# afb2001/path_planner

Measured on AMD Instinct MI355X. Metric: Dubins edges costed/sec on 2048x2048 grid, higher is better.
Workload: dtype f64; 1 GPU; cfg3_2048_10pct_65536_obst16; grid=2048x2048 @0.1m, 10% blocked, samples_per_iter_per_gpu=65536, samples_per_iter_total=65536, dynamic_obstacles=16, obstacle_placement=uniform in the map (SURVEY 8d), seed 3, ribbons=5, heuristic=TspPointRobotNoSplitKRibbons K=2, edges_per_iter_per_gpu=236140

## Files before the change

include/ppgpu.h:

```cpp
#ifndef PATH_PLANNER_AMD_PPGPU_H
#define PATH_PLANNER_AMD_PPGPU_H

#include <stdint.h>

#ifdef __cplusplus
extern "C" {
#endif

#define PPGPU_OK          0
#define PPGPU_EINVAL     (-1)
#define PPGPU_EHIP       (-2)
#define PPGPU_ENODEV     (-3)
#define PPGPU_ESTATE     (-4)
#define PPGPU_ECAPACITY  (-5)
#define PPGPU_ERCCL      (-6)

typedef struct ppgpu_ctx ppgpu_ctx;

enum {
    PPGPU_H_MAX_DISTANCE = 0,
    PPGPU_H_TSP_POINT_ALL = 1,
    PPGPU_H_TSP_POINT_K = 2,
    PPGPU_H_TSP_DUBINS_ALL = 3,
    PPGPU_H_TSP_DUBINS_K = 4
};

enum {
    PPGPU_OBST_NONE = 0,
    PPGPU_OBST_BINARY = 1,
    PPGPU_OBST_GAUSSIAN = 2
};

typedef struct ppgpu_config {
    double max_speed;
    double slow_speed;
    double turning_radius;
    double coverage_turning_radius;
    double time_horizon;
    double time_minimum;
    double collision_checking_increment;
    double start_state_time;
    double ribbon_width;
    double collision_penalty_factor;
    double time_penalty_factor;
    double heuristic_turning_radius;
    int32_t heuristic;
    int32_t tsp_k;
    int32_t branching_factor;
    int32_t reserved;
} ppgpu_config;

typedef struct ppgpu_vertex {
    double x, y, heading, speed, time;
    double g;
    double coverage_completed_time;
    int32_t ribbon_offset;
    int32_t ribbon_count;
} ppgpu_vertex;

#define PPGPU_F_INFEASIBLE   0x01u
#define PPGPU_F_THROWS       0x02u
#define PPGPU_F_RIBBON_OVF   0x04u
#define PPGPU_F_RIBBON_LOST  0x40u
#define PPGPU_F_DUBINS_ERR   0x08u
#define PPGPU_F_GOAL         0x10u
#define PPGPU_F_DONE         0x20u

typedef struct ppgpu_edge_result {
    uint32_t flags;
    uint32_t info;
    double true_cost;
    double collision_penalty;
    double approx_cost;
    double end_x, end_y, end_heading, end_speed, end_time;
    double g, h, f;
    double coverage_completed_time;
    double param[3];
} ppgpu_edge_result;

#define PPGPU_EDGE_COVERAGE 0x1u
#define PPGPU_EDGE_SLOW     0x2u
static inline uint64_t ppgpu_edge_pack(uint32_t vertex, uint32_t target, uint32_t cfg) {
    return ((uint64_t)(cfg & 0xffu) << 56) | ((uint64_t)(vertex & 0xffffffu) << 32) | (uint64_t)target;
}

typedef struct ppgpu_wrapper_edge {
    int32_t vertex;
    int32_t coverage_allowed;
    double qi[3];
    double param[3];
    double rho;
    int32_t type;
    int32_t reserved;
    double speed;
    double start_time;
    double end_time;
} ppgpu_wrapper_edge;


int ppgpu_create(int device, ppgpu_ctx** out);
int ppgpu_destroy(ppgpu_ctx* ctx);
const char* ppgpu_last_error(void);
int ppgpu_set_stream(ppgpu_ctx* ctx, void* hip_stream);
int ppgpu_synchronize(ppgpu_ctx* ctx);
int ppgpu_reserve_samples(ppgpu_ctx* ctx, int64_t max_samples, int32_t max_vertices);
int ppgpu_growth_stats(ppgpu_ctx* ctx, uint64_t* count, double* seconds);
int ppgpu_enable_timing(ppgpu_ctx* ctx, int32_t on);
int ppgpu_last_timing(ppgpu_ctx* ctx, double* ms_solve, double* ms_pose, double* ms_cover, double* ms_heuristic);
int ppgpu_past_timing(ppgpu_ctx* ctx, int32_t back, double* ms_solve, double* ms_pose, double* ms_cover, double* ms_heuristic);
int ppgpu_last_cover_edges(ppgpu_ctx* ctx, int64_t* n_edges);
int ppgpu_last_shared_edges(ppgpu_ctx* ctx, int64_t* n_edges);

int ppgpu_device_alloc(ppgpu_ctx* ctx, uint64_t bytes, void** d_out);
int ppgpu_device_free(ppgpu_ctx* ctx, void* d_ptr);
int ppgpu_device_read(ppgpu_ctx* ctx, void* h_dst, const void* d_src, uint64_t bytes);
int ppgpu_copy_engine_read(ppgpu_ctx* ctx, void* h_pinned_dst, const void* d_src, uint64_t bytes);
int ppgpu_copy_engine_wait(ppgpu_ctx* ctx);


int ppgpu_set_config(ppgpu_ctx* ctx, const ppgpu_config* cfg);

int ppgpu_set_grid(ppgpu_ctx* ctx, const uint8_t* h_cells, int32_t rows, int32_t cols, double resolution);
int ppgpu_get_grid_clearance(ppgpu_ctx* ctx, uint8_t* h_out, int64_t capacity);

int ppgpu_set_obstacles(ppgpu_ctx* ctx, int32_t model, int32_t n, const double* h_obstacles7);

int ppgpu_set_gaussian_obstacles(ppgpu_ctx* ctx, int32_t n, const double* h_obstacles, int32_t covariance_given);

int ppgpu_set_vertices(ppgpu_ctx* ctx, int32_t n, const ppgpu_vertex* h_vertices,
                       int32_t n_ribbons, const double* h_ribbons4);


int ppgpu_sampler_init(ppgpu_ctx* ctx, const double* bounds6, uint64_t seed,
                       int32_t n_ribbons, const double* h_ribbons4);

int ppgpu_sampler_add(ppgpu_ctx* ctx, int64_t n_attempts, int64_t* n_total_out);

int ppgpu_sampler_skip(ppgpu_ctx* ctx, int64_t n_attempts);

int ppgpu_set_samples(ppgpu_ctx* ctx, int64_t n, const double* h_x, const double* h_y, const double* h_heading);
int ppgpu_set_extra_targets(ppgpu_ctx* ctx, int32_t n, const double* h_x, const double* h_y, const double* h_heading,
                            int64_t* first_index);

int ppgpu_get_samples(ppgpu_ctx* ctx, int64_t first, int64_t n, double* h_states5);
int64_t ppgpu_num_samples(ppgpu_ctx* ctx);


int ppgpu_dubins_lengths(ppgpu_ctx* ctx, int32_t v0, int32_t nv, double* d_lengths);

int ppgpu_select_nearest(ppgpu_ctx* ctx, int32_t v0, int32_t nv, int32_t k,
                         int32_t* h_sample_index, double* h_length);

int ppgpu_expand_order(ppgpu_ctx* ctx, int32_t v0, int32_t nv, int32_t k, int32_t* h_sample_index, uint32_t* h_fallbacks);
uint64_t ppgpu_order_fallbacks(ppgpu_ctx* ctx);


int ppgpu_cost_edges_dense(ppgpu_ctx* ctx, int32_t v0, int32_t nv, int64_t s0, int64_t ns,
                           uint32_t cfg_mask, ppgpu_edge_result* d_results,
                           double* d_child_ribbons, int32_t ribbon_stride);

int ppgpu_cost_edges_list(ppgpu_ctx* ctx, int64_t n, const uint64_t* d_edges,
                          ppgpu_edge_result* d_results,
                          double* d_child_ribbons, int32_t ribbon_stride);

int64_t ppgpu_expand_capacity(int32_t nv, int32_t k);
int ppgpu_expand_host(ppgpu_ctx* ctx, int32_t nv, const ppgpu_vertex* h_vertices, int32_t n_ribbons, const double* h_ribbons,
                      const double* h_nearest, int32_t k, int64_t* n_edges, uint64_t* h_edges, ppgpu_edge_result* h_results,
                      double* h_child_ribbons, int32_t ribbon_stride);

int ppgpu_heuristic_host(ppgpu_ctx* ctx, int32_t n, const double* h_poses3, const int32_t* h_ribbon_counts, const double* h_ribbons,
                         double* h_out, uint32_t* h_flags);

#define PPGPU_TSP_TABLE_MAX 16
int ppgpu_set_tsp_table(ppgpu_ctx* ctx, int32_t min_ribbons, int32_t max_ribbons);
int ppgpu_set_dubins_tsp_table(ppgpu_ctx* ctx, int32_t min_ribbons, int32_t max_ribbons);
int ppgpu_tsp_table_stats(ppgpu_ctx* ctx, uint64_t* lists, uint64_t* refused);
int ppgpu_last_tsp_table_timing(ppgpu_ctx* ctx, double* ms);

int ppgpu_cost_edges_host(ppgpu_ctx* ctx, int64_t n, const uint64_t* h_edges,
                          ppgpu_edge_result* h_results,
                          double* h_child_ribbons, int32_t ribbon_stride);

int ppgpu_cost_wrapper_edges_host(ppgpu_ctx* ctx, int64_t n, const ppgpu_wrapper_edge* h_edges,
                                  ppgpu_edge_result* h_results,
                                  double* h_child_ribbons, int32_t ribbon_stride);


#define PPGPU_CHAIN_LEGS        1u
#define PPGPU_CHAIN_INFEASIBLE  2u
#define PPGPU_CHAIN_GOAL        3u
#define PPGPU_CHAIN_THROWS      4u
#define PPGPU_CHAIN_CAPACITY    5u

int ppgpu_cost_plans_host(ppgpu_ctx* ctx, int32_t n_plans, const int32_t* h_leg_offsets, const ppgpu_wrapper_edge* h_legs,
                          ppgpu_edge_result* h_results, double* h_child_ribbons, int32_t ribbon_stride,
                          int32_t* h_legs_costed, uint32_t* h_stop);


#define PPGPU_S_BLOCKED  0x1u
#define PPGPU_S_STRAIGHT 0x2u
typedef struct ppgpu_step_record {
    double x, y, heading, time;
    double collision;
    double penalty_before;
    uint32_t flags, step;
    double reserved;
} ppgpu_step_record;

int ppgpu_trace_edges_list(ppgpu_ctx* ctx, int64_t n, const uint64_t* d_edges, ppgpu_edge_result* d_results,
                           int32_t step_stride, int32_t* d_counts, ppgpu_step_record* d_steps);
int ppgpu_trace_edges_host(ppgpu_ctx* ctx, int64_t n, const uint64_t* h_edges, ppgpu_edge_result* h_results,
                           int32_t step_stride, int32_t* h_counts, ppgpu_step_record* h_steps);
int ppgpu_trace_wrapper_edges_host(ppgpu_ctx* ctx, int64_t n, const ppgpu_wrapper_edge* h_wedges, ppgpu_edge_result* h_results,
                                   int32_t step_stride, int32_t* h_counts, ppgpu_step_record* h_steps);
int ppgpu_last_trace_timing(ppgpu_ctx* ctx, double* ms_trace);


#define PPGPU_C_EVENT   0x1u
#define PPGPU_C_COVER   0x2u
#define PPGPU_C_CHANGED 0x4u
#define PPGPU_C_DONE    0x8u
typedef struct ppgpu_cover_record {
    double to_cover;
    double remaining;
    uint32_t flags, step;
    uint32_t ribbons;
    uint32_t reserved;
} ppgpu_cover_record;

#define PPGPU_CS_LAST_COVER   0x01u
#define PPGPU_CS_LAST_CHANGED 0x02u
#define PPGPU_CS_DONE         0x04u
#define PPGPU_CS_REFUSED      0x08u
#define PPGPU_CS_THROWS       0x10u
typedef struct ppgpu_cover_summary {
    int32_t events, changes;
    int32_t ribbons_final;
    uint32_t flags;
    double coverage_completed_time;
    double remaining_final;
} ppgpu_cover_summary;

int ppgpu_trace_cover_list(ppgpu_ctx* ctx, int64_t n, const uint64_t* d_edges, ppgpu_edge_result* d_results,
                           int32_t step_stride, int32_t* d_counts, ppgpu_cover_record* d_cover,
                           ppgpu_cover_summary* d_summaries, double* d_child_ribbons, int32_t ribbon_stride);
int ppgpu_trace_cover_host(ppgpu_ctx* ctx, int64_t n, const uint64_t* h_edges, ppgpu_edge_result* h_results,
                           int32_t step_stride, int32_t* h_counts, ppgpu_cover_record* h_cover,
                           ppgpu_cover_summary* h_summaries, double* h_child_ribbons, int32_t ribbon_stride);
int ppgpu_trace_cover_wrapper_edges_host(ppgpu_ctx* ctx, int64_t n, const ppgpu_wrapper_edge* h_wedges, ppgpu_edge_result* h_results,
                                         int32_t step_stride, int32_t* h_counts, ppgpu_cover_record* h_cover,
                                         ppgpu_cover_summary* h_summaries, double* h_child_ribbons, int32_t ribbon_stride);
int ppgpu_last_cover_trace_timing(ppgpu_ctx* ctx, double* ms_cover_trace);


typedef struct ppgpu_contact_record {
    double cpa_distance;
    double cpa_time;
    double first_hit_time, last_hit_time;
    double exposure;
    int32_t cpa_step, hit_steps, first_hit_step, last_hit_step;
    double peak;
} ppgpu_contact_record;

int ppgpu_obstacle_count(ppgpu_ctx* ctx, int32_t* n, int32_t* model);
// ... 98 lines not shown
```

path_planner_amd/api.py:

```python
import ctypes as C
import os

import numpy as np

from .types import PpgpuConfig, RESULT_DTYPE, VERTEX_DTYPE

_HERE = os.path.dirname(os.path.abspath(__file__))
LIB_PATH = os.environ.get("PPGPU_LIB_OVERRIDE") or os.path.join(_HERE, "csrc", "libppgpu.so")


class PpgpuError(RuntimeError):
    pass


def _load():
    try:
        import torch
    except Exception:
        pass
    if not os.path.exists(LIB_PATH):
        raise ImportError(
            f"{LIB_PATH} is missing: build it with `python -c 'import __graft_entry__ as g; g.build()'` "
            "(hipcc --offload-arch=gfx950). path_planner_amd has no CPU fallback.")
    lib = C.CDLL(LIB_PATH)
    vp, i32, i64, u32, u64, dbl = C.c_void_p, C.c_int32, C.c_int64, C.c_uint32, C.c_uint64, C.c_double
    sig = {
        "ppgpu_create": (C.c_int, [C.c_int, C.POINTER(vp)]),
        "ppgpu_destroy": (C.c_int, [vp]),
        "ppgpu_last_error": (C.c_char_p, []),
        "ppgpu_set_stream": (C.c_int, [vp, vp]),
        "ppgpu_synchronize": (C.c_int, [vp]),
        "ppgpu_reserve_samples": (C.c_int, [vp, i64, i32]),
        "ppgpu_growth_stats": (C.c_int, [vp, C.POINTER(u64), C.POINTER(dbl)]),
        "ppgpu_device_alloc": (C.c_int, [vp, u64, C.POINTER(vp)]),
        "ppgpu_device_free": (C.c_int, [vp, vp]),
        "ppgpu_device_read": (C.c_int, [vp, vp, vp, u64]),
        "ppgpu_copy_engine_read": (C.c_int, [vp, vp, vp, u64]),
        "ppgpu_copy_engine_wait": (C.c_int, [vp]),
        "ppgpu_heuristic_host": (C.c_int, [vp, i32, vp, vp, vp, vp, vp]),
        "ppgpu_set_tsp_table": (C.c_int, [vp, i32, i32]),
        "ppgpu_set_dubins_tsp_table": (C.c_int, [vp, i32, i32]),
        "ppgpu_tsp_table_stats": (C.c_int, [vp, C.POINTER(u64), C.POINTER(u64)]),
        "ppgpu_last_tsp_table_timing": (C.c_int, [vp, C.POINTER(dbl)]),
        "ppgpu_expand_capacity": (C.c_int64, [i32, i32]),
        "ppgpu_expand_host": (C.c_int, [vp, i32, vp, i32, vp, vp, i32, C.POINTER(C.c_int64), vp, vp, vp, i32]),
        "ppgpu_enable_timing": (C.c_int, [vp, i32]),
        "ppgpu_last_timing": (C.c_int, [vp, C.POINTER(dbl), C.POINTER(dbl), C.POINTER(dbl), C.POINTER(dbl)]),
        "ppgpu_past_timing": (C.c_int, [vp, i32, C.POINTER(dbl), C.POINTER(dbl), C.POINTER(dbl), C.POINTER(dbl)]),
        "ppgpu_last_cover_edges": (C.c_int, [vp, C.POINTER(i64)]),
        "ppgpu_last_shared_edges": (C.c_int, [vp, C.POINTER(i64)]),
        "ppgpu_set_config": (C.c_int, [vp, C.POINTER(PpgpuConfig)]),
        "ppgpu_set_grid": (C.c_int, [vp, vp, i32, i32, dbl]),
        "ppgpu_get_grid_clearance": (C.c_int, [vp, vp, i64]),
        "ppgpu_set_obstacles": (C.c_int, [vp, i32, i32, vp]),
        "ppgpu_set_gaussian_obstacles": (C.c_int, [vp, i32, vp, i32]),
        "ppgpu_set_vertices": (C.c_int, [vp, i32, vp, i32, vp]),
        "ppgpu_sampler_init": (C.c_int, [vp, vp, u64, i32, vp]),
        "ppgpu_sampler_add": (C.c_int, [vp, i64, C.POINTER(i64)]),
        "ppgpu_sampler_skip": (C.c_int, [vp, i64]),
        "ppgpu_set_samples": (C.c_int, [vp, i64, vp, vp, vp]),
        "ppgpu_set_extra_targets": (C.c_int, [vp, i32, vp, vp, vp, C.POINTER(i64)]),
        "ppgpu_get_samples": (C.c_int, [vp, i64, i64, vp]),
        "ppgpu_num_samples": (i64, [vp]),
        "ppgpu_dubins_lengths": (C.c_int, [vp, i32, i32, vp]),
        "ppgpu_select_nearest": (C.c_int, [vp, i32, i32, i32, vp, vp]),
        "ppgpu_expand_order": (C.c_int, [vp, i32, i32, i32, vp, C.POINTER(u32)]),
        "ppgpu_order_fallbacks": (u64, [vp]),
        "ppgpu_cost_edges_dense": (C.c_int, [vp, i32, i32, i64, i64, u32, vp, vp, i32]),
        "ppgpu_cost_edges_list": (C.c_int, [vp, i64, vp, vp, vp, i32]),
        "ppgpu_cost_edges_host": (C.c_int, [vp, i64, vp, vp, vp, i32]),
        "ppgpu_cost_wrapper_edges_host": (C.c_int, [vp, i64, vp, vp, vp, i32]),
        "ppgpu_cost_plans_host": (C.c_int, [vp, i32, vp, vp, vp, vp, i32, vp, vp]),
        "ppgpu_trace_edges_list": (C.c_int, [vp, i64, vp, vp, i32, vp, vp]),
        "ppgpu_trace_edges_host": (C.c_int, [vp, i64, vp, vp, i32, vp, vp]),
        "ppgpu_trace_wrapper_edges_host": (C.c_int, [vp, i64, vp, vp, i32, vp, vp]),
        "ppgpu_last_trace_timing": (C.c_int, [vp, C.POINTER(dbl)]),
        "ppgpu_trace_cover_list": (C.c_int, [vp, i64, vp, vp, i32, vp, vp, vp, vp, i32]),
        "ppgpu_trace_cover_host": (C.c_int, [vp, i64, vp, vp, i32, vp, vp, vp, vp, i32]),
        "ppgpu_trace_cover_wrapper_edges_host": (C.c_int, [vp, i64, vp, vp, i32, vp, vp, vp, vp, i32]),
        "ppgpu_last_cover_trace_timing": (C.c_int, [vp, C.POINTER(dbl)]),
        "ppgpu_obstacle_count": (C.c_int, [vp, C.POINTER(i32), C.POINTER(i32)]),
        "ppgpu_trace_contacts_list": (C.c_int, [vp, i64, vp, vp, vp, vp]),
        "ppgpu_trace_contacts_host": (C.c_int, [vp, i64, vp, vp, vp, vp]),
        "ppgpu_trace_contacts_wrapper_edges_host": (C.c_int, [vp, i64, vp, vp, vp, vp]),
        "ppgpu_last_contact_trace_timing": (C.c_int, [vp, C.POINTER(dbl)]),
        "ppgpu_get_grid_distance": (C.c_int, [vp, vp, i64]),
        "ppgpu_grid_clearance_at": (C.c_int, [vp, i64, vp, vp, vp]),
        "ppgpu_last_grid_distance_timing": (C.c_int, [vp, C.POINTER(dbl)]),
        "ppgpu_trace_clearance_list": (C.c_int, [vp, i64, vp, vp, vp, vp, dbl]),
        "ppgpu_trace_clearance_host": (C.c_int, [vp, i64, vp, vp, vp, vp, dbl]),
        "ppgpu_trace_clearance_wrapper_edges_host": (C.c_int, [vp, i64, vp, vp, vp, vp, dbl]),
        "ppgpu_last_clearance_trace_timing": (C.c_int, [vp, C.POINTER(dbl)]),
        "ppgpu_keepout_limit2": (C.c_int, [dbl, dbl, C.POINTER(u32)]),
        "ppgpu_set_keepout_limit2": (C.c_int, [vp, u32]),
        "ppgpu_get_keepout_limit2": (C.c_int, [vp, C.POINTER(u32)]),
        "ppgpu_get_grid_blocked": (C.c_int, [vp, vp, i64]),
        "ppgpu_last_keepout_timing": (C.c_int, [vp, C.POINTER(dbl)]),
        "ppgpu_get_grid_labels": (C.c_int, [vp, vp, i64]),
        "ppgpu_set_reach_seed": (C.c_int, [vp, dbl, dbl, vp]),
        "ppgpu_get_grid_reach_gap": (C.c_int, [vp, vp, i64]),
        "ppgpu_ribbon_reach_host": (C.c_int, [vp, i32, vp, dbl, vp]),
        "ppgpu_last_reach_timing": (C.c_int, [vp, C.POINTER(dbl), C.POINTER(dbl), C.POINTER(dbl)]),
        "ppgpu_dense_edge_count": (i64, [i32, i64, u32]),
        "ppgpu_best_edge": (C.c_int, [vp, i64, vp, i32, u64, vp]),
        "ppgpu_key_min": (C.c_int, [vp, i32, vp, vp]),
        "ppgpu_allreduce_best": (C.c_int, [vp, vp, vp]),
        "ppgpu_comm_unique_id": (C.c_int, [vp]),
        "ppgpu_comm_init_rank": (C.c_int, [vp, i32, i32, vp]),
        "ppgpu_comm_init_all": (C.c_int, [C.POINTER(vp), i32]),
        "ppgpu_comm_info": (C.c_int, [vp, C.POINTER(i32), C.POINTER(i32)]),
        "ppgpu_comm_destroy": (C.c_int, [vp]),
        "ppgpu_comm_abort": (C.c_int, [vp]),
    }
    for name, (res, args) in sig.items():
        fn = getattr(lib, name)
        fn.restype = res
        fn.argtypes = args
    return lib, list(sig)


LIB, EXPORTS = _load()


def keepout_limit2(res, margin):
    k = C.c_uint32()
    rc = LIB.ppgpu_keepout_limit2(float(res), float(margin), C.byref(k))
    if rc != 0:
        raise PpgpuError(f"ppgpu_keepout_limit2 failed ({rc}): {LIB.ppgpu_last_error().decode()}")
    return k.value


def _ptr(a):
    if a is None:
        return None
    if isinstance(a, np.ndarray):
        assert a.flags["C_CONTIGUOUS"]
        return a.ctypes.data
    return int(a)


class Context:

    def __init__(self, device=0):
        h = C.c_void_p()
        rc = LIB.ppgpu_create(device, C.byref(h))
        if rc != 0:
            raise PpgpuError(f"ppgpu_create: {LIB.ppgpu_last_error().decode()}")
        self._h = h

    def _ck(self, rc, what):
        if rc != 0:
            raise PpgpuError(f"{what} failed ({rc}): {LIB.ppgpu_last_error().decode()}")

    def close(self):
        if self._h:
            LIB.ppgpu_destroy(self._h)
            self._h = None

    def __del__(self):
        try:
            self.close()
        except Exception:
            pass

    def set_stream(self, stream_ptr):
        self._ck(LIB.ppgpu_set_stream(self._h, stream_ptr), "ppgpu_set_stream")

    def enable_timing(self, on=True):
        self._ck(LIB.ppgpu_enable_timing(self._h, 1 if on else 0), "ppgpu_enable_timing")

    def last_timing(self):
        t = [C.c_double() for _ in range(4)]
        self._ck(LIB.ppgpu_last_timing(self._h, *[C.byref(x) for x in t]), "ppgpu_last_timing")
        return tuple(x.value for x in t)

    def past_timing(self, back):
        t = [C.c_double() for _ in range(4)]
        self._ck(LIB.ppgpu_past_timing(self._h, back, *[C.byref(x) for x in t]), "ppgpu_past_timing")
        return tuple(x.value for x in t)

    def last_cover_edges(self):
        n = C.c_int64()
        self._ck(LIB.ppgpu_last_cover_edges(self._h, C.byref(n)), "ppgpu_last_cover_edges")
        return n.value

    def last_shared_edges(self):
        n = C.c_int64()
        self._ck(LIB.ppgpu_last_shared_edges(self._h, C.byref(n)), "ppgpu_last_shared_edges")
        return n.value

    def reserve_samples(self, max_samples, max_vertices=16):
        self._ck(LIB.ppgpu_reserve_samples(self._h, max_samples, max_vertices), "ppgpu_reserve_samples")

    def synchronize(self):
        self._ck(LIB.ppgpu_synchronize(self._h), "ppgpu_synchronize")

    def set_config(self, cfg):
        self.cfg = cfg
        self._ck(LIB.ppgpu_set_config(self._h, C.byref(cfg)), "ppgpu_set_config")

    def set_grid(self, cells, resolution):
        if cells is None:
            self._ck(LIB.ppgpu_set_grid(self._h, None, 0, 0, 0.0), "ppgpu_set_grid")
            return
        cells = np.ascontiguousarray(cells, dtype=np.uint8)
        self._ck(LIB.ppgpu_set_grid(self._h, _ptr(cells), cells.shape[0], cells.shape[1], float(resolution)), "ppgpu_set_grid")

    def get_grid_clearance(self, rows, cols):
        out = np.zeros((rows, cols), dtype=np.uint8)
        self._ck(LIB.ppgpu_get_grid_clearance(self._h, _ptr(out), out.size), "ppgpu_get_grid_clearance")
        return out

    def set_obstacles(self, obst7, model=1):
        if obst7 is None or len(obst7) == 0:
            self._ck(LIB.ppgpu_set_obstacles(self._h, 0, 0, None), "ppgpu_set_obstacles")
            return
        o = np.ascontiguousarray(obst7, dtype=np.float64).reshape(-1, 7)
        self._ck(LIB.ppgpu_set_obstacles(self._h, model, o.shape[0], _ptr(o)), "ppgpu_set_obstacles")

    def set_gaussian_obstacles(self, rows):
        o = np.ascontiguousarray(rows, dtype=np.float64)
        if o.size == 0:
            self._ck(LIB.ppgpu_set_gaussian_obstacles(self._h, 0, None, 0), "ppgpu_set_gaussian_obstacles")
            return
        assert o.ndim == 2 and o.shape[1] in (5, 9)
        self._ck(LIB.ppgpu_set_gaussian_obstacles(self._h, o.shape[0], _ptr(o), 1 if o.shape[1] == 9 else 0), "ppgpu_set_gaussian_obstacles")

    def set_vertices(self, vertices, ribbons4):
        v = np.ascontiguousarray(vertices, dtype=VERTEX_DTYPE)
        r = np.ascontiguousarray(ribbons4, dtype=np.float64).reshape(-1, 4)
        self._ck(LIB.ppgpu_set_vertices(self._h, v.shape[0], _ptr(v), r.shape[0], _ptr(r) if r.shape[0] else None),
                 "ppgpu_set_vertices")

    def sampler_init(self, bounds6, seed, ribbons4=None):
        b = np.ascontiguousarray(bounds6, dtype=np.float64)
        if ribbons4 is None:
            self._ck(LIB.ppgpu_sampler_init(self._h, _ptr(b), int(seed), -1, None), "ppgpu_sampler_init")
        else:
            r = np.ascontiguousarray(ribbons4, dtype=np.float64).reshape(-1, 4)
            self._ck(LIB.ppgpu_sampler_init(self._h, _ptr(b), int(seed), r.shape[0], _ptr(r) if r.shape[0] else None),
                     "ppgpu_sampler_init")

    def sampler_add(self, n_attempts):
        tot = C.c_int64()
        self._ck(LIB.ppgpu_sampler_add(self._h, int(n_attempts), C.byref(tot)), "ppgpu_sampler_add")
        return tot.value

    def copy_engine_read(self, h_pinned_ptr, d_ptr, nbytes):
        self._ck(LIB.ppgpu_copy_engine_read(self._h, int(h_pinned_ptr), int(d_ptr), int(nbytes)), "ppgpu_copy_engine_read")

    def copy_engine_wait(self):
        self._ck(LIB.ppgpu_copy_engine_wait(self._h), "ppgpu_copy_engine_wait")

    def growth_stats(self):
        n, sec = C.c_uint64(), C.c_double()
        self._ck(LIB.ppgpu_growth_stats(self._h, C.byref(n), C.byref(sec)), "ppgpu_growth_stats")
        return int(n.value), float(sec.value)

    def sampler_skip(self, n_attempts):
        self._ck(LIB.ppgpu_sampler_skip(self._h, int(n_attempts)), "ppgpu_sampler_skip")

    def set_samples(self, x, y, heading):
        x = np.ascontiguousarray(x, dtype=np.float64)
        y = np.ascontiguousarray(y, dtype=np.float64)
        h = np.ascontiguousarray(heading, dtype=np.float64)
        self._ck(LIB.ppgpu_set_samples(self._h, x.shape[0], _ptr(x), _ptr(y), _ptr(h)), "ppgpu_set_samples")

    def num_samples(self):
        return LIB.ppgpu_num_samples(self._h)

    def get_samples(self, first=0, n=None):
        if n is None:
            n = self.num_samples() - first
        out = np.zeros((n, 5), dtype=np.float64)
        self._ck(LIB.ppgpu_get_samples(self._h, first, n, _ptr(out)), "ppgpu_get_samples")
        return out

    def dubins_lengths(self, v0, nv, d_lengths):
        self._ck(LIB.ppgpu_dubins_lengths(self._h, v0, nv, _ptr(d_lengths)), "ppgpu_dubins_lengths")

    def set_extra_targets(self, x, y, heading):
        x, y, heading = [np.ascontiguousarray(a, dtype=np.float64) for a in (x, y, heading)]
        first = C.c_int64(0)
        self._ck(LIB.ppgpu_set_extra_targets(self._h, x.shape[0], _ptr(x) if x.shape[0] else None, _ptr(y) if x.shape[0] else None,
                                             _ptr(heading) if x.shape[0] else None, C.byref(first)), "ppgpu_set_extra_targets")
        return int(first.value)

    def select_nearest(self, v0, nv, k):
        idx = np.zeros((nv, 2, k), dtype=np.int32)
        ln = np.zeros((nv, 2, k), dtype=np.float64)
        self._ck(LIB.ppgpu_select_nearest(self._h, v0, nv, k, _ptr(idx), _ptr(ln)), "ppgpu_select_nearest")
        return idx, ln

    def expand_order(self, nv, k):
        idx = np.zeros((nv, 2, k), dtype=np.int32)
        fb = C.c_uint32(0)
        self._ck(LIB.ppgpu_expand_order(self._h, 0, nv, k, _ptr(idx), C.byref(fb)), "ppgpu_expand_order")
        return idx, int(fb.value)

    def order_fallbacks(self):
        return int(LIB.ppgpu_order_fallbacks(self._h))

    def cost_edges_dense(self, v0, nv, s0, ns, cfg_mask, d_results, d_child=None, stride=0):
        self._ck(LIB.ppgpu_cost_edges_dense(self._h, v0, nv, s0, ns, cfg_mask, _ptr(d_results), _ptr(d_child), stride),
                 "ppgpu_cost_edges_dense")

    def cost_edges_list(self, n, d_edges, d_results, d_child=None, stride=0):
        self._ck(LIB.ppgpu_cost_edges_list(self._h, n, _ptr(d_edges), _ptr(d_results), _ptr(d_child), stride),
                 "ppgpu_cost_edges_list")

    def heuristic_host(self, poses3, ribbon_lists):
        ps = np.ascontiguousarray(poses3, dtype=np.float64).reshape(-1, 3)
        counts = np.array([len(r) for r in ribbon_lists], dtype=np.int32)
        flat = np.ascontiguousarray(np.concatenate([np.asarray(r, dtype=np.float64).reshape(-1, 4) for r in ribbon_lists]) if counts.sum() else np.zeros((0, 4)))
        out = np.zeros(len(ps), dtype=np.float64)
        fl = np.zeros(len(ps), dtype=np.uint32)
        self._ck(LIB.ppgpu_heuristic_host(self._h, len(ps), _ptr(ps), _ptr(counts), _ptr(flat) if len(flat) else None, _ptr(out), _ptr(fl)), "ppgpu_heuristic_host")
        return out, fl

    def set_tsp_table(self, min_ribbons, max_ribbons):
        self._ck(LIB.ppgpu_set_tsp_table(self._h, int(min_ribbons), int(max_ribbons)), "ppgpu_set_tsp_table")

    def set_dubins_tsp_table(self, min_ribbons, max_ribbons):
        self._ck(LIB.ppgpu_set_dubins_tsp_table(self._h, int(min_ribbons), int(max_ribbons)), "ppgpu_set_dubins_tsp_table")

    def tsp_table_stats(self):
        lists, refused = C.c_uint64(), C.c_uint64()
        self._ck(LIB.ppgpu_tsp_table_stats(self._h, C.byref(lists), C.byref(refused)), "ppgpu_tsp_table_stats")
        return int(lists.value), int(refused.value)

    def last_tsp_table_timing(self):
        ms = C.c_double()
        self._ck(LIB.ppgpu_last_tsp_table_timing(self._h, C.byref(ms)), "ppgpu_last_tsp_table_timing")
        return float(ms.value)

    def expand_host(self, vertices, ribbons4, nearest3, k, stride=0):
        v = np.ascontiguousarray(vertices, dtype=VERTEX_DTYPE)
        r = np.ascontiguousarray(ribbons4, dtype=np.float64).reshape(-1, 4)
        nz = np.ascontiguousarray(nearest3, dtype=np.float64).reshape(-1, 3)
        cap = int(LIB.ppgpu_expand_capacity(v.shape[0], k))
        e = np.zeros(cap, dtype=np.uint64)
        res = np.zeros(cap, dtype=RESULT_DTYPE)
# ... 250 lines not shown
```

path_planner_amd/csrc/pp_k_common.h:

```cpp
#pragma once
#include "../../include/ppgpu.h"
#include "pp_device.h"

struct __attribute__((aligned(128))) PPLaunchWords {
    unsigned need_big;
    unsigned live_count;
    unsigned hw_count;
    unsigned defer_count[PP_HL_MAX_N + 1];
};
static_assert(sizeof(PPLaunchWords) == 128, "the launch counters share one 128-byte line");

struct PPParams {
    double max_speed, slow_speed, rho, rho_cov, horizon, tmin, inc_d, sst, ribw, cpf, tpf;
    double inv_inc_d;
    int heuristic, tsp_k;
    int fuse_h;
    int quiet_finish;
    int lane_split;
    int defer_h;
    double h_rho;
    PPGrid grid;
    const PPObst* obst; int n_obst; int obst_model;
    const ppgpu_vertex* verts; const double* ribbons; const double* tgrid; int ng; int nverts;
    const double* sx; const double* sy; const double* sh; long long n_samples;
    const unsigned long long* edges; long long n_edges;
    long long total_edges;
    const ppgpu_wrapper_edge* wedges;
    int v0, nv; long long s0, ns; unsigned cfg_mask; int per;
    ppgpu_edge_result* out; double* child; int stride;
    long long e_base, ws_base;
    struct PPEdgeSetup* setup;
    unsigned short* track_hits;
    unsigned long long* track_eq;
    unsigned* track_chunk_hits;
    double* track_pen;
    double* track_chunk_pen;
    struct PPTrackSummary* track_summary;
    unsigned char* track_skip;
    int2* track_far;
    unsigned long long* work;
    PPLaunchWords* words;
    int reset_words;
    unsigned* live_list;
    unsigned* defer_list;
    struct PPCoverState* cover_state;
    unsigned* hw_list;
    int ngp, nch;
    unsigned* share_head;
    unsigned* share_of;
};

#define PP_SETUP_MALFORMED 1u
#define PP_SETUP_COLOCATED 2u
#define PP_SETUP_SHARED 4u
#define PP_SETUP_NO_SWEEP (PP_SETUP_MALFORMED | PP_SETUP_COLOCATED | PP_SETUP_SHARED)
#define PP_SHARE_KEYS 8
#define PP_SHARE_NONE 0xffffffffu
struct PPEdgeSetupBody {
    PPSegBase seg[3];
    double p0, p1, p2, hi1;
    double qx, qy, rho, rho_inv, length;
    double wStart, wEnd, speed;
    double approx;
    unsigned long long omask;
    int type;
    unsigned vi, cbits, sflags;
    double srcH;
};
struct __attribute__((aligned(128))) PPEdgeSetup : PPEdgeSetupBody {};
static_assert(sizeof(PPEdgeSetup) == 256 && sizeof(PPEdgeSetupBody) == 256, "PPEdgeSetup is sized for two 128-byte lines");
template <bool TAB = false>
__device__ __forceinline__ void pp_setup_seg_pose(const PPEdgeSetupBody* S, int i, double tprime, double p0, double p1, int word, double& ux, double& uy, double& uth) {
    const PPSegBase* g = &S->seg[i];
    pp_curve_seg<TAB>(pp_word_seg_type(word, i), (tprime - pp_seg_o1(i, p0)) - pp_seg_o2(i, p1), g->bx, g->by, g->bth, g->sb, g->cb, ux, uy, uth);
}
template <bool TAB = false>
__device__ __forceinline__ void pp_setup_seg_pose(const PPEdgeSetupBody* S, int i, double tprime, double& ux, double& uy, double& uth) {
    pp_setup_seg_pose<TAB>(S, i, tprime, S->p0, S->p1, S->type, ux, uy, uth);
}
#define PP_SETUP_GLOBAL_WORDS 32
#define PP_SETUP_WORDS 32
#define PP_SETUP_LDS_STRIDE 33
static_assert(sizeof(PPEdgeSetup) == 8 * PP_SETUP_GLOBAL_WORDS && sizeof(PPEdgeSetupBody) == 8 * PP_SETUP_WORDS, "the LDS staging of the skip planner copies whole records");

__global__ __launch_bounds__(256) void pp_k_grid_row_clear(const uint32_t* bits, int rows, int cols, int wpr, unsigned char* rowclear) {
    const long long i = (long long)blockIdx.x * 256 + threadIdx.x;
    if (i >= (long long)rows * cols) return;
    const int r = (int)(i / cols), c = (int)(i - (long long)r * cols);
    const uint32_t* row = bits + (size_t)r * wpr;
    int d = 0;
    for (; d < PP_CLEAR_CAP; d++) {
        const int a = c - d, b = c + d;
        if (a < 0 || b >= cols) break;
        if (((row[a >> 5] >> (a & 31)) | (row[b >> 5] >> (b & 31))) & 1u) break;
    }
    rowclear[i] = (unsigned char)d;
}
__global__ __launch_bounds__(256) void pp_k_grid_clear(const unsigned char* rowclear, int rows, int cols, unsigned char* clearance) {
    const long long i = (long long)blockIdx.x * 256 + threadIdx.x;
    if (i >= (long long)rows * cols) return;
    const int r = (int)(i / cols), c = (int)(i - (long long)r * cols);
    int best = rowclear[i];
    for (int dy = 1; dy < best; dy++) {
        const int up = r + dy, dn = r - dy;
        int m = dy;
        if (up < rows && dn >= 0) {
            const int ru = rowclear[(size_t)up * cols + c], rd = rowclear[(size_t)dn * cols + c];
            m = max(dy, min(ru, rd));
        }
        best = min(best, m);
    }
    clearance[i] = (unsigned char)best;
}

#define PP_TG_SEG 2048
__global__ __launch_bounds__(64) void pp_k_time_grid(const ppgpu_vertex* verts, int nverts, double sst, double inc_d, double max_speed,
                                                    int ng, double* tgrid) {
    __shared__ double seg[PP_TG_SEG];
    const int v = blockIdx.x;
    if (v >= nverts) return;
    const int lane = threadIdx.x;
    double timeIncrement = inc_d / max_speed;
    double t = verts[v].time;
    double timeSinceStart = t - sst;
    double timeNudge = fmod(timeSinceStart, timeIncrement);
    t += timeNudge;
    double* row = tgrid + (size_t)v * ng;
    int s = 0;
    for (int tries = 0; s < ng && tries < 8; tries++) {
        const double c = (t + timeIncrement) - t;
        int firstBad = ng;
        for (int k0 = s; k0 < ng; k0 += 64) {
            const int k = k0 + lane;
            const double val = t + (double)(k - s) * c;
            const double nxt = t + (double)(k + 1 - s) * c;
            if (k < ng) row[k] = val;
            const bool bad = (k < ng - 1) && !(val + timeIncrement == nxt);
            const unsigned long long m = __ballot(bad);
            if (m != 0ull) { firstBad = k0 + (int)__builtin_ctzll(m); break; }
        }
        if (firstBad == ng) { s = ng; break; }
        const double tf = t + (double)(firstBad - s) * c;
        t = tf + timeIncrement;
        s = firstBad + 1;
    }
    for (int k0 = s; k0 < ng; k0 += PP_TG_SEG) {
        const int m = (ng - k0) < PP_TG_SEG ? (ng - k0) : PP_TG_SEG;
        if (lane == 0) {
            for (int k = 0; k < m; k++) {
                seg[k] = t;
                t += timeIncrement;
            }
        }
        __syncthreads();
        for (int k = lane; k < m; k += 64) row[k0 + k] = seg[k];
        __syncthreads();
        t = __shfl(t, 0, 64);
    }
}

__device__ __forceinline__ long long pp_edge_position(const PPParams& p, long long w) {
    if (p.wedges || p.edges) return w;
    const long long Q = p.total_edges / p.per;
    const long long r = w / Q;
    return (w - r * Q) * p.per + (p.per - 1 - r);
}

__device__ __forceinline__ void pp_edge_decode(const PPParams& p, long long e, unsigned& vi, unsigned& target, unsigned& cbits) {
    if (p.wedges) {
        vi = (unsigned)p.wedges[e].vertex;
        target = 0;
        cbits = p.wedges[e].coverage_allowed ? PPGPU_EDGE_COVERAGE : 0u;
    } else if (p.edges) {
        unsigned long long d = p.edges[e];
        target = (unsigned)(d & 0xffffffffull);
        vi = (unsigned)((d >> 32) & 0xffffffull);
        cbits = (unsigned)(d >> 56);
    } else {
        long long q = e / p.per;
        int rank = (int)(e - q * p.per);
        long long vv = q / p.ns;
        target = (unsigned)(p.s0 + (q - vv * p.ns));
        vi = (unsigned)(p.v0 + vv);
        unsigned m = p.cfg_mask;
        for (int i = 0; i < rank; i++) m &= m - 1;
        cbits = (unsigned)(__ffs((int)m) - 1);
    }
}

template <int WPB>
__device__ __forceinline__ long long pp_wave_edge(int& wave) {
    wave = __builtin_amdgcn_readfirstlane((int)(threadIdx.x >> 6));
    return (long long)blockIdx.x * WPB + wave;
}
#define PP_NQ 32
#define PP_QSTRIDE 544
#define PP_WORK_WORDS (PP_NQ * PP_QSTRIDE)
struct PPQueue { int q, dry; };
__device__ __forceinline__ PPQueue pp_queue_init() {
    PPQueue s; s.q = (int)(blockIdx.x % PP_NQ); s.dry = 0; return s;
}
__device__ __forceinline__ long long pp_next_edge(const PPParams& p, PPQueue& s, long long n) {
    while (s.dry < PP_NQ) {
        unsigned long long* head = p.work + (size_t)s.q * PP_QSTRIDE;
        unsigned long long k = 0;
        if (pp_lane() == 0) {
            k = (s.dry > 0) ? __hip_atomic_load(head, __ATOMIC_RELAXED, __HIP_MEMORY_SCOPE_AGENT) : 0ull;
            if ((long long)(k * PP_NQ) + s.q < n) k = atomicAdd(head, 1ull);
        }
        const unsigned lo = (unsigned)__builtin_amdgcn_readfirstlane((int)(unsigned)k);
        const unsigned hi = (unsigned)__builtin_amdgcn_readfirstlane((int)(unsigned)(k >> 32));
        const int q = __builtin_amdgcn_readfirstlane(s.q);
        const unsigned long long kk = ((unsigned long long)hi << 32) | lo;
        const long long idx = (long long)(kk * PP_NQ) + q;
        if (idx < n) { s.dry = 0; return idx; }
        s.q = (s.q + 1 == PP_NQ) ? 0 : s.q + 1;
        s.dry++;
    }
    return n;
}
__device__ __forceinline__ void pp_launch_reset(const PPParams& p, long long e) {
    if (!p.reset_words) return;
    if (e < PP_NQ) p.work[(size_t)e * PP_QSTRIDE] = 0ull;
    if (e == 0) { if (p.e_base == 0) *p.words = PPLaunchWords{}; else p.words->live_count = 0u; }
}
```

path_planner_amd/csrc/pp_k_cover.h:

```cpp
#pragma once
__device__ __forceinline__ int pp_event_stride(double D, double inc_d, double inv_inc_d, int ng) {
    int m = 0;
    if (D > inc_d) {
        const double qd = D * inv_inc_d;
        if (qd > (double)(ng + 2)) {
            m = ng + 1;
        } else {
            const int m0 = (int)ceil(qd - 1.0);
            const double r = fma(-(double)m0, inc_d, D);
            const double margin = (double)m0 * D * 5e-16 + 1e-12;
            if (m0 >= 1 && r > margin && r < inc_d - margin) {
                m = m0;
            } else {
                double tc = D;
                while (tc > inc_d && m <= ng) { tc -= inc_d; m++; }
            }
        }
    }
    return m;
}

#define PP_FAR_DONE (-2)
#define PP_FAR_SHARED (-3)
#define PP_FAR_LAST_MASK 0xfffff
#define PP_FAR_SPLIT (1 << 30)
#define PP_FAR_MOVE_END (1 << 29)
#define PP_FAR_PIECE_SHIFT 21
#define PP_REC_STRIDE 17
template <class RP>
__device__ __forceinline__ bool pp_any_tiny_ribbon(RP r, int n, double thr) {
    bool tiny = false;
    for (int i = 0; i < n; i++) tiny |= pp_sq_len(r[4 * i], r[4 * i + 1], r[4 * i + 2], r[4 * i + 3]) < thr;
    return tiny;
}
struct PPBoxScan { bool inBox; int boxCount, boxIdx; double q; };
template <class RP>
__device__ __forceinline__ PPBoxScan pp_box_scan(RP r, int n, double x, double y, double grow) {
    PPBoxScan s = {false, 0, 0, PP_DBL_MAX};
    for (int i = 0; i < n; i++) {
        const double sx = r[4 * i], sy = r[4 * i + 1], ex = r[4 * i + 2], ey = r[4 * i + 3];
        const bool in = pp_in_grown_box(sx, sy, ex, ey, x, y, grow);
        s.inBox |= in; s.boxCount += in ? 1 : 0; s.boxIdx = in ? i : s.boxIdx;
        const double qS = (sx - x) * (sx - x) + (sy - y) * (sy - y);
        const double qE = (ex - x) * (ex - x) + (ey - y) * (ey - y);
        s.q = fmin(s.q, fmin(qE, qS));
    }
    return s;
}
#ifndef PP_APPROACH_MIN_WAVES
#define PP_APPROACH_MIN_WAVES 4
#endif
#ifndef PP_APPROACH_THREADS
#define PP_APPROACH_THREADS 256
#endif
#ifndef PP_LANE_NEAR_MAX
#define PP_LANE_NEAR_MAX 8
#endif
__global__ __launch_bounds__(PP_APPROACH_THREADS, PP_APPROACH_MIN_WAVES) void pp_k_approach_events(PPParams p) {
    __shared__ double s_rec[PP_APPROACH_THREADS * PP_REC_STRIDE];
    const long long e0 = (long long)blockIdx.x * PP_APPROACH_THREADS;
    const long long e = e0 + threadIdx.x;
    const bool valid = e < p.n_edges;
    const PPEdgeSetupBody* S = p.setup + p.ws_base + (valid ? e : 0);
    int2 out; out.x = 0; out.y = 0;
    int splitInfo = 0;
#ifdef PP_DBG_PHASES
    const long long apT0 = (long long)__builtin_readcyclecounter();
    long long apT1 = apT0, apT2 = apT0;
    int apEvents = 0;
#endif
    const unsigned sflags = S->sflags;
    const int dubType = S->type;
    const unsigned viMine = S->vi;
    const unsigned viFirst = (unsigned)__builtin_amdgcn_readfirstlane((int)viMine);
    const bool oneVertex = viFirst < (unsigned)p.nverts && __ballot(valid && viMine != viFirst) == 0ull;
    const double* rpU = p.ribbons + 4 * (size_t)pp_const_i32(&p.verts[oneVertex ? viFirst : 0].ribbon_offset)[0];
    const int nribU = pp_const_i32(&p.verts[oneVertex ? viFirst : 0].ribbon_count)[0];
    if (valid && !(sflags & PP_SETUP_NO_SWEEP) && dubType >= 0) {
        const ppgpu_vertex* V = p.verts + S->vi;
        const int nrib = V->ribbon_count;
        const int limit = p.track_summary[p.ws_base + e].limit;
        if (nrib > 0 && nrib <= PP_WAVE && limit > 0) {
            const double* rp = p.ribbons + 4 * (size_t)V->ribbon_offset;
            const double* tg = p.tgrid + (size_t)S->vi * p.ng;
            const PPLaneCurve cv = pp_lane_curve(S);
            const double endTime0 = fmin(p.horizon + 1e-12 + p.sst, S->wEnd);
            const double w = p.ribw, grow = w + 1e-3, minLength0 = 2 * w;
            const PPLaneRibbons ribs = {rp, nrib, rpU, nribU, oneVertex};
            const bool tiny = pp_with_ribbons(ribs, [&](auto r, int n) { return pp_any_tiny_ribbon(r, n, minLength0 * minLength0 / (2.0 * 2.0)); });
            int k = 0, lastEv = -1;
            bool handOver = tiny;
            int nearBudget = PP_LANE_NEAR_MAX;
            const bool covEdge = (S->cbits & PPGPU_EDGE_COVERAGE) != 0;
#ifdef PP_DBG_PHASES
            apT1 = (long long)__builtin_readcyclecounter();
#endif
            while (!tiny) {
                if (k >= limit) break;
                const double t = tg[k];
                if (!(t < endTime0)) break;
#ifdef PP_DBG_PHASES
                apEvents++;
#endif
                double x, y, uth;
                bool perr = false;
                pp_lane_pose(S, cv, t, x, y, uth, perr);
                if (perr) { handOver = true; break; }
                const PPBoxScan scan = pp_with_ribbons(ribs, [&](auto r, int n) { return pp_box_scan(r, n, x, y, grow); });
                const int boxIdx = scan.boxIdx;
#ifdef PP_DBG_TRACE
                if (pp_edge_position(p, p.e_base + e) == (long long)(PP_DBG_TRACE)) printf("[lane] event %d: inBox %d q %.17g x %.17g y %.17g\n", k, (int)scan.inBox, scan.q, x, y);
#endif
                double D = fmin(PP_DBL_MAX, sqrt(scan.q));
                if (scan.inBox) {
                    if (scan.boxCount == 1 && nearBudget-- > 0) {
                        bool inside, strict;
                        double px, py;
                        const double bsx = rp[4 * boxIdx], bsy = rp[4 * boxIdx + 1], bex = rp[4 * boxIdx + 2], bey = rp[4 * boxIdx + 3];
                        pp_lane_ribbon_contains(bsx, bsy, bex, bey, x, y, w, inside, strict, px, py);
                        const bool coverOn = covEdge || (((p.track_eq[(size_t)(p.ws_base + e) * p.nch + (k >> 6)] >> (k & 63)) & 1ull) != 0ull);
                        if (!(strict && coverOn)) {
                            if (inside) D = 0;
                            lastEv = k;
                            k = k + pp_event_stride(D, p.inc_d, p.inv_inc_d, p.ng) + 1;
                            continue;
                        }
                        const double thr = minLength0 * minLength0 / (2.0 * 2.0);
                        const bool keepF = !(pp_sq_len(bsx, bsy, px, py) < thr), keepR = !(pp_sq_len(px, py, bex, bey) < thr);
                        if (keepF && keepR && p.lane_split && nrib + 1 <= p.stride && nrib + 1 <= PP_WAVE) {
                            double* c = p.child + (size_t)pp_edge_position(p, p.e_base + e) * p.stride * 4;
                            for (int i = 0; i < boxIdx; i++) { c[4 * i] = rp[4 * i]; c[4 * i + 1] = rp[4 * i + 1]; c[4 * i + 2] = rp[4 * i + 2]; c[4 * i + 3] = rp[4 * i + 3]; }
                            c[4 * boxIdx] = bsx; c[4 * boxIdx + 1] = bsy; c[4 * boxIdx + 2] = px; c[4 * boxIdx + 3] = py;
                            c[4 * boxIdx + 4] = px; c[4 * boxIdx + 5] = py; c[4 * boxIdx + 6] = bex; c[4 * boxIdx + 7] = bey;
                            for (int i = boxIdx + 1; i < nrib; i++) { c[4 * i + 4] = rp[4 * i]; c[4 * i + 5] = rp[4 * i + 1]; c[4 * i + 6] = rp[4 * i + 2]; c[4 * i + 7] = rp[4 * i + 3]; }
                            double sn, cs;
                            pp_sincos_bounded(uth, &sn, &cs);
                            const bool towardsEnd = (cs * (bex - bsx) + sn * (bey - bsy)) > 0.0;
                            splitInfo = PP_FAR_SPLIT | (towardsEnd ? 0 : PP_FAR_MOVE_END) | ((towardsEnd ? boxIdx + 1 : boxIdx) << PP_FAR_PIECE_SHIFT);
                            lastEv = k;
                            k = k + 1;
                            handOver = true; break;
                        }
                    }
                    handOver = true; break;
                }
                lastEv = k;
                k = k + pp_event_stride(D, p.inc_d, p.inv_inc_d, p.ng) + 1;
            }
            out.x = k; out.y = (lastEv + 1) | splitInfo;
#ifdef PP_DBG_PHASES
            apT2 = (long long)__builtin_readcyclecounter();
#endif
            if (!handOver && k >= limit && p.quiet_finish &&
                pp_finish_quiet_edge(p, S, cv, V, p.ws_base + e, pp_edge_position(p, p.e_base + e), limit, lastEv, ribs, tg, s_rec + (size_t)threadIdx.x * PP_REC_STRIDE))
                out.x = PP_FAR_DONE;
        }
    }
    asm volatile("" ::: "memory");
    if (valid && (S->sflags & PP_SETUP_SHARED) != 0u) out.x = PP_FAR_SHARED;
    if (valid) p.track_far[p.ws_base + e] = make_int2(max(out.x, PP_FAR_DONE), out.y);
#ifdef PP_DBG_PHASES
    {
        const long long apT3 = (long long)__builtin_readcyclecounter();
        const double wPro = pp_wave_max((double)(apT1 - apT0)), wLoop = pp_wave_max((double)(apT2 - apT1)), wFin = pp_wave_max((double)(apT3 - apT2));
        const double wEv = pp_wave_max((double)apEvents);
        if (valid && out.x == PP_FAR_DONE) {
            double* st = s_rec + (size_t)threadIdx.x * PP_REC_STRIDE;
            st[12] = wPro; st[13] = wLoop * 4294967296.0 + (double)(apT2 - apT1); st[14] = -1.0 - wFin; st[15] = wEv * 1e6 + (double)apEvents;
        }
    }
#endif
    {
        const int lane = threadIdx.x & 63, wbase = (int)threadIdx.x - lane;
        const unsigned long long doneMask = __ballot(valid && out.x == PP_FAR_DONE);
        if (doneMask) {
            pp_wave_lds_fence();
            const long long myEg = valid ? pp_edge_position(p, p.e_base + e) : 0;
            const int g = lane >> 4, slot = lane & 15;
            for (int it = 0; it < 16; it++) {
                const int src = 4 * it + g;
                const long long egs = __shfl(myEg, src, PP_WAVE);
                if ((doneMask >> src) & 1ull) reinterpret_cast<double*>(p.out + egs)[slot] = s_rec[(size_t)(wbase + src) * PP_REC_STRIDE + slot];
            }
        }
    }
    if (p.live_list) {
        __shared__ unsigned s_cnt[PP_APPROACH_THREADS / 64];
        __shared__ unsigned s_base;
        const int lane = threadIdx.x & 63, wave = threadIdx.x >> 6;
        const bool live = valid && out.x >= 0;
        const unsigned long long m = __ballot(live);
        if (lane == 0) s_cnt[wave] = (unsigned)__popcll(m);
        __syncthreads();
        if (threadIdx.x == 0) {
            unsigned tot = 0;
            for (int w = 0; w < PP_APPROACH_THREADS / 64; w++) tot += s_cnt[w];
            s_base = tot ? atomicAdd(&p.words->live_count, tot) : 0u;
        }
        __syncthreads();
        if (live) {
            unsigned at = s_base + (unsigned)__popcll(m & ((1ull << lane) - 1ull));
            for (int w = 0; w < wave; w++) at += s_cnt[w];
            p.live_list[2 * at] = (unsigned)e;
            p.live_list[2 * at + 1] = (unsigned)pp_edge_position(p, p.e_base + e);
        }
    }
}

#ifndef PP_FUSE_HEUR
#define PP_FUSE_HEUR 1
#endif
template <bool GAUSSIAN>
__device__ __forceinline__ void pp_cover_sweep_edge(const PPParams& p, const long long e, const long long eg, double* lds) {
    const int lane = pp_lane();

    if (p.track_far && pp_const_i32(&p.track_far[e].x)[0] == PP_FAR_DONE) return;
    const PPEdgeSetup* S = p.setup + e;
    unsigned flags = 0;
    ppgpu_edge_result* rec = p.out + eg;
    const unsigned sflags = (unsigned)PP_SI32(sflags);
#if !defined(PP_DBG_COUNTS)
    const bool laneFinish = !GAUSSIAN && p.cover_state != nullptr;
#else
    const bool laneFinish = false;
#endif
    if (laneFinish && lane == 0) p.cover_state[e].nrib = -1;
    if (sflags & PP_SETUP_MALFORMED) {
        if (lane == 0) { rec->flags = PPGPU_F_INFEASIBLE | PPGPU_F_THROWS | PPGPU_F_DUBINS_ERR; rec->info = 0; }
        return;
    }
    const unsigned vi = (unsigned)PP_SI32(vi), cbits = (unsigned)PP_SI32(cbits);
    const ppgpu_vertex* V = p.verts + vi;
    const double srcX = pp_sgpr(V->x), srcY = pp_sgpr(V->y), srcT = pp_sgpr(V->time), srcG = pp_sgpr(V->g);
    double cct = pp_sgpr(V->coverage_completed_time);
    int nrib = __builtin_amdgcn_readfirstlane(V->ribbon_count);
    const bool cov = (cbits & PPGPU_EDGE_COVERAGE) != 0;

    PPRibbon rib = {0, 0, 0, 0};
    if (nrib > PP_WAVE) { nrib = PP_WAVE; flags |= PPGPU_F_RIBBON_OVF | PPGPU_F_RIBBON_LOST; }
    if (lane < nrib) {
        const double* rp = p.ribbons + 4 * ((size_t)V->ribbon_offset + lane);
        rib.sx = rp[0]; rib.sy = rp[1]; rib.ex = rp[2]; rib.ey = rp[3];
    }
    const bool startedDone = (nrib == 0);

    const int dubType = PP_SI32(type);
    const double wEnd = PP_SF64(wEnd), wStart = PP_SF64(wStart), speed = PP_SF64(speed);
    const double endTime0 = fmin(p.horizon + 1e-12 + p.sst, wEnd);
    double endTime = endTime0;
    bool infeasible = (srcT >= endTime);
    bool throwsRef = ((sflags & PP_SETUP_COLOCATED) != 0) || (dubType < 0);
    if (dubType < 0) flags |= PPGPU_F_DUBINS_ERR;

    const PPTrackSummary* sum = p.track_summary + e;
    const int limit = pp_const_i32(&sum->limit)[0];
    const int stopKind = pp_const_i32(&sum->blocked)[0];
    const bool blockedAtLimit = stopKind == 1;
    if (pp_const_i32(&sum->dub_err)[0]) flags |= PPGPU_F_DUBINS_ERR;
    const unsigned long long* teq = p.track_eq + (size_t)e * p.nch;
    const double* tg = p.tgrid + (size_t)vi * p.ng;

#ifdef PP_DBG_COUNTS
    int dbgWindows = 0, dbgCorr = 0, dbgQuiet = 0, dbgGeneric = 0, dbgCorrLen = 0, dbgQuietLen = 0, dbgFar = 0, dbgNoChange = 0, dbgInPlace = 0, dbgRestFar = 0;
#define PP_CNT(x) x
#else
#define PP_CNT(x)
#endif
#ifdef PP_DBG_PHASES
    long long phWin = 0, phCont = 0, phGen = 0, phRun = 0, phLoop = 0, phT = 0;
#define PP_PH_START() (phT = (long long)__builtin_readcyclecounter())
#define PP_PH_END(acc) (acc += (long long)__builtin_readcyclecounter() - phT)
#else
#define PP_PH_START()
#define PP_PH_END(acc)
#endif
#ifdef PP_DBG_TRACE
#define PP_TRACE(...) do { if (eg == (long long)(PP_DBG_TRACE) && lane == 0) printf(__VA_ARGS__); } while (0)
#else
#define PP_TRACE(...)
#endif
    int rdt = -1;
    int nextEvent = 0;
    int lastEv = -1;
    int handCont = 0, handPiece = 0, handCount = 0;
    bool handMoveEnd = false;
    if (p.track_far) {
        nextEvent = pp_const_i32(&p.track_far[e].x)[0];
        const int fy = pp_const_i32(&p.track_far[e].y)[0];
        lastEv = (fy & PP_FAR_LAST_MASK) - 1;
        if (fy & PP_FAR_SPLIT) {
            nrib = nrib + 1;
            rib = PPRibbon{0, 0, 0, 0};
            if (lane < nrib) {
                const double* rp = p.child + ((size_t)eg * p.stride + lane) * 4;
                rib.sx = rp[0]; rib.sy = rp[1]; rib.ex = rp[2]; rib.ey = rp[3];
            }
            handCont = 1 | 4; handPiece = (fy >> PP_FAR_PIECE_SHIFT) & 0x3f; handMoveEnd = (fy & PP_FAR_MOVE_END) != 0;
            handCount = nrib;
        }
    }
    const double w = p.ribw;
    const double inc_d = p.inc_d;
    const double runSpan = 64.0 * (p.inc_d / p.max_speed) * speed * (1.0 + 1e-9) + 1e-6;

#ifndef PP_LONG_REACH
#define PP_LONG_REACH 0.05
#endif
#ifndef PP_LONG_MAX_STRIDE
#define PP_LONG_MAX_STRIDE 16
#endif
#define PP_STEP_LEN() ((p.inc_d / p.max_speed) * speed * (1.0 + 1e-9) + 1e-9)
    int longStride = 1;
    {
        const double stepLen = PP_STEP_LEN();
        const double sd = PP_LONG_REACH / stepLen;
        longStride = sd >= (double)PP_LONG_MAX_STRIDE ? PP_LONG_MAX_STRIDE : (sd > 1.0 ? (int)sd : 1);
        if (!((double)longStride * stepLen + 1e-6 < 0.5 * w) || !(((double)longStride * stepLen + 1e-6) / PP_SF64(rho) < 0.5)) longStride = 1;
    }

    if (!throwsRef) {
#ifdef PP_DBG_PHASES
        const long long phLoop0 = (long long)__builtin_readcyclecounter();
#endif
        bool ended = false;
        int cont = handCont, contPiece = handPiece;
        bool contMoveEnd = handMoveEnd;
        while (!ended) {
            if (nextEvent >= limit) break;
            const int base = nextEvent;
            const int stride = ((cont & 4) != 0 && longStride > 1 && base + 2 * longStride < limit) ? longStride : 1;
            PP_TRACE("[wave] window at %d stride %d (limit %d, lastEv %d, nrib %d)\n", base, stride, limit, lastEv, nrib);
            PP_CNT(dbgWindows++);
            PP_PH_START();
            const int k = base + lane * stride;
            const double t = (k < p.ng) ? tg[k] : INFINITY;
            double2 q;
            {
                PP_WINDOW_POSE(S, t, pp_readlane(t, 0), k < limit, q.x, q.y);
                if (k >= limit) { q.x = 0.0; q.y = 0.0; }
            }
            unsigned long long coverMask = ~0ull, coverAny = ~0ull;
            if (!cov) {
                if (stride == 1) {
                    const int c0 = base >> 6, sh = base & 63;
                    const unsigned long long lo = pp_const_u64(teq + c0)[0];
                    const unsigned long long hi = (sh != 0 && c0 + 1 < p.nch) ? pp_const_u64(teq + c0 + 1)[0] : 0ull;
                    coverMask = sh ? ((lo >> sh) | (hi << (64 - sh))) : lo;
                    coverAny = coverMask;
                } else {
                    const int lo = (lane == 0) ? base : (k - stride + 1);
                    const int cnt = (lane == 0) ? 1 : stride;
                    unsigned long long bits = 0ull;
                    if (k < limit) {
                        const int w0 = lo >> 6, sh = lo & 63;
                        bits = teq[w0] >> sh;
                        if (sh + cnt > 64 && w0 + 1 < p.nch) bits |= teq[w0 + 1] << (64 - sh);
                    }
                    const unsigned long long mask = (1ull << cnt) - 1ull;
                    bits &= mask;
                    coverMask = __ballot(bits == mask);
// ... 323 lines not shown
```

path_planner_amd/csrc/pp_k_solve.h:

```cpp
#pragma once
#ifndef PP_CR_SOLVE
#define PP_CR_SOLVE true
#endif
#ifndef PP_SOLVE_MIN_WAVES
#define PP_SOLVE_MIN_WAVES 1
#endif
__device__ __forceinline__ bool pp_edge_shareable(const PPParams& p, const PPCurve& cv, int type, unsigned sflags, unsigned cbits,
                                                  double wStart, double wEnd, double speed) {
    if (type < 0 || (sflags & (PP_SETUP_MALFORMED | PP_SETUP_COLOCATED)) || cbits >= 4u) return false;
    const double bound = p.horizon + 1e-12 + p.sst;
    if (wEnd < bound) return false;
    const double dist = (bound - wStart) * speed;
    if (!(dist <= cv.length)) return false;
    const double tprime = (cv.rho_inv != 0.0) ? dist * cv.rho_inv : dist / cv.rho;
    return tprime < cv.p0;
}
__device__ __forceinline__ unsigned pp_share_key(unsigned vi, unsigned cbits, int type) {
    return vi * PP_SHARE_KEYS + (cbits & 3u) * 2u + (pp_word_seg_type(type, 0) == 0 ? 0u : 1u);
}
__device__ __forceinline__ void pp_share_elect(const PPParams& p, bool member, unsigned key, unsigned pos) {
    bool pend = false;
    if (member) pend = pos < __hip_atomic_load(p.share_head + key, __ATOMIC_RELAXED, __HIP_MEMORY_SCOPE_AGENT);
    unsigned long long m;
    while ((m = __ballot(pend)) != 0ull) {
        const int leader = __ffsll((long long)m) - 1;
        const unsigned k0 = (unsigned)__builtin_amdgcn_readlane((int)key, leader);
        if (pp_lane() == leader) atomicMin(p.share_head + k0, pos);
        if (key == k0) pend = false;
    }
}

template <bool ALL_WORDS>
__device__ __forceinline__ void pp_solve_edges_body(const PPParams& p) {
    const long long e = (long long)blockIdx.x * 256 + threadIdx.x;
    pp_launch_reset(p, e);
    if (e >= p.n_edges) return;
    long long e2 = -1;
    if (!p.wedges && !p.edges) {
        const long long Q = p.total_edges / p.per;
        const int r = (int)((p.e_base + e) / Q);
        unsigned m = p.cfg_mask;
        for (int i = 0; i < p.per - 1 - r; i++) m &= m - 1;
        const unsigned c = (unsigned)(__ffs((int)m) - 1), c2 = c ^ PPGPU_EDGE_SLOW;
        if ((p.cfg_mask >> c2) & 1u) {
            const int r2 = (int)__popc(p.cfg_mask >> (c2 + 1));
            const long long ep = e + (long long)(r2 - r) * Q;
            if (ep >= 0 && ep < p.n_edges) {
                if (!(c & PPGPU_EDGE_SLOW)) return;
                e2 = ep;
            }
        }
    }
    unsigned vi, target, cbits;
    const long long eg = pp_edge_position(p, p.e_base + e);
    pp_edge_decode(p, eg, vi, target, cbits);
    PPCurve cv;
    bool valid = false;
    unsigned sflags = 0;
    double srcT = 0, wSpeed = 1, wStart = 0, wEnd = 0;
    double srcHeading = 0;
    PPDubins dub;
    dub.p0 = dub.p1 = dub.p2 = 0; dub.type = -1;
    if (vi >= (unsigned)p.nverts || (!p.wedges && (long long)target >= p.n_samples)) {
        sflags = PP_SETUP_MALFORMED;
        pp_curve_init<false>(cv, 0, 0, 0, 1.0, dub);
    } else {
        const ppgpu_vertex* V = p.verts + vi;
        const double srcX = V->x, srcY = V->y, srcH = V->heading;
        srcT = V->time;
        srcHeading = srcH;
        valid = true;
        double rho = (cbits & PPGPU_EDGE_COVERAGE) ? p.rho_cov : p.rho;
        if (p.wedges) {
            const ppgpu_wrapper_edge* W = p.wedges + eg;
            dub.p0 = W->param[0]; dub.p1 = W->param[1]; dub.p2 = W->param[2]; dub.type = W->type;
            if (dub.type < 0 || dub.type > 5) dub.type = -1;
            rho = W->rho; wSpeed = W->speed;
            pp_curve_init<PP_CR_SOLVE, PP_CR_SOLVE && !ALL_WORDS>(cv, W->qi[0], W->qi[1], W->qi[2], rho, dub);
            wStart = W->start_time; wEnd = W->end_time;
        } else {
            const double tgtX = p.sx[target], tgtY = p.sy[target], tgtH = p.sh[target];
            if ((srcX == tgtX) && (srcY == tgtY) && (srcH == tgtH)) sflags |= PP_SETUP_COLOCATED;
            if constexpr (ALL_WORDS || !PP_CR_SOLVE) {
                pp_dubins_shortest<PP_CR_SOLVE>(srcX, srcY, pp_yaw(srcH), tgtX, tgtY, pp_yaw(tgtH), rho, dub);
                pp_curve_init<PP_CR_SOLVE>(cv, srcX, srcY, pp_yaw(srcH), rho, dub);
            } else {
                pp_dubins_shortest_ranked(srcX, srcY, pp_yaw(srcH), tgtX, tgtY, pp_yaw(tgtH), rho, dub);
                pp_curve_init<PP_CR_SOLVE, true>(cv, srcX, srcY, pp_yaw(srcH), rho, dub);
            }
        }
        {
            const double bound = fabs(cv.qth) + cv.p0 + (cv.t1 == 1 ? 0.0 : cv.p1) + cv.p2;
            if (!(bound < 9.0e4)) dub.type = -1;
        }
    }
    bool member[2] = {false, false};
    unsigned key[2] = {0u, 0u}, pos[2] = {0u, 0u};
    for (int k = 0; k < (e2 >= 0 ? 2 : 1); k++) {
        PPEdgeSetup* __restrict__ O = p.setup + p.ws_base + (k ? e2 : e);
        struct { double approx, wStart, wEnd, speed; int type; unsigned vi, cbits, sflags; } S;
        S.vi = vi; S.cbits = k ? (cbits ^ PPGPU_EDGE_SLOW) : cbits; S.sflags = sflags; S.type = -1;
        S.approx = S.wStart = S.wEnd = 0; S.speed = 1;
        if (valid) {
            if (p.wedges) {
                S.speed = wSpeed;
                S.wStart = wStart; S.wEnd = wEnd;
                S.approx = (S.wEnd - srcT) * 1.0;
            } else {
                S.speed = (S.cbits & PPGPU_EDGE_SLOW) ? p.slow_speed : p.max_speed;
                S.approx = cv.length / S.speed * 1.0;
                S.wStart = srcT;
                S.wEnd = srcT + cv.length / S.speed;
            }
            S.type = dub.type;
        }
        if (p.share_head) {
            const long long egk = k ? pp_edge_position(p, p.e_base + e2) : eg;
            member[k] = pp_edge_shareable(p, cv, S.type, S.sflags, S.cbits, S.wStart, S.wEnd, S.speed);
            key[k] = member[k] ? pp_share_key(S.vi, S.cbits, S.type) : PP_SHARE_NONE;
            pos[k] = (unsigned)egk;
            p.share_of[egk] = key[k];
        }
        pp_curve_segments(cv, O->seg);
        O->qx = cv.qx; O->qy = cv.qy; O->rho = cv.rho; O->rho_inv = cv.rho_inv; O->length = cv.length;
        O->p0 = cv.p0; O->p1 = cv.p1; O->p2 = cv.p2; O->hi1 = cv.p0 + cv.p1;
        O->approx = S.approx; O->wStart = S.wStart; O->wEnd = S.wEnd; O->speed = S.speed;
        O->type = S.type; O->vi = S.vi; O->cbits = S.cbits; O->sflags = S.sflags;
        O->srcH = srcHeading;
        unsigned long long omask = 0ull;
        if (p.n_obst > PP_WAVE) omask = ~0ull;
        else if (p.n_obst > 0 && S.type >= 0 && !(S.sflags & PP_SETUP_MALFORMED) && p.ng > 0) {
            const double t0 = p.tgrid[(size_t)vi * p.ng];
            const double endTime = fmin(p.horizon + 1e-12 + p.sst, S.wEnd);
            const double chunkTime = 64.0 * (p.inc_d / p.max_speed);
            const double duration = fmax(endTime - t0, 0.0) + chunkTime;
            const double travel = fmin(cv.length, fmax(endTime - S.wStart, 0.0) * S.speed) + 1e-3;
            for (int j = 0; j < p.n_obst; j++) {
                const PPObst& o = p.obst[j];
                const double dt = t0 - o.Time;
                const double X = o.X + o.Speed * dt * o.cosYaw, Y = o.Y + o.Speed * dt * o.sinYaw;
                const double R = o.reach + travel + fabs(o.Speed) * duration + 1e-3;
                const double dx = cv.qx - X, dy = cv.qy - Y;
                if (!(dx * dx + dy * dy > R * R)) omask |= 1ull << j;
            }
        }
        O->omask = omask;
    }
    if (p.share_head) {
        pp_share_elect(p, member[0], key[0], pos[0]);
        if (__ballot(e2 >= 0) != 0ull) pp_share_elect(p, member[1], key[1], pos[1]);
    }
}
__global__ __launch_bounds__(256) void pp_k_share_mark(PPParams p) {
    const long long e = (long long)blockIdx.x * 256 + threadIdx.x;
    if (e >= p.n_edges) return;
    const long long eg = pp_edge_position(p, p.e_base + e);
    const unsigned key = p.share_of[eg];
    if (key == PP_SHARE_NONE) return;
    const unsigned head = p.share_head[key];
    if (head == (unsigned)eg) { p.share_of[eg] = PP_SHARE_NONE; return; }
    p.share_of[eg] = head;
    PPEdgeSetup* S = p.setup + p.ws_base + e;
    S->sflags |= PP_SETUP_SHARED;
    double* r = reinterpret_cast<double*>(p.out + eg);
    const unsigned info = (unsigned)(S->type & 0xff);
    r[0] = __hiloint2double((int)info, 0);
    r[1] = 0.0; r[2] = 0.0; r[3] = S->approx;
    for (int i = 4; i < 13; i++) r[i] = 0.0;
    r[13] = S->p0; r[14] = S->p1; r[15] = S->p2;
}
__global__ __launch_bounds__(256) void pp_k_share_fanout(PPParams p, int copy_child) {
    const long long eg = (long long)blockIdx.x * 16 + (threadIdx.x >> 4);
    const int sub = (int)(threadIdx.x & 15);
    if (eg >= p.n_edges) return;
    const unsigned h = p.share_of[eg];
    if (h == PP_SHARE_NONE) return;
    const unsigned long long* src = reinterpret_cast<const unsigned long long*>(p.out + h);
    unsigned long long* dst = reinterpret_cast<unsigned long long*>(p.out + eg);
    unsigned long long v = src[sub];
    if (sub == 0) v = (v & ~(0xffull << 32)) | (dst[0] & (0xffull << 32));
    if (sub != 3 && sub < 13) dst[sub] = v;
    if (copy_child) {
        const double* cs = p.child + (size_t)h * p.stride * 4;
        double* cd = p.child + (size_t)eg * p.stride * 4;
        for (int i = sub; i < p.stride * 4; i += 16) cd[i] = cs[i];
    }
}
__global__ __launch_bounds__(256, PP_SOLVE_MIN_WAVES) void pp_k_solve_edges(PPParams p) { pp_solve_edges_body<false>(p); }
__global__ __launch_bounds__(256, PP_SOLVE_MIN_WAVES) void pp_k_solve_edges_all_words(PPParams p) { pp_solve_edges_body<true>(p); }
```

path_planner_amd/csrc/pp_k_sweep.h:

```cpp
#pragma once
#ifndef PP_WPB
#define PP_WPB 4
#endif
#ifndef PP_MIN_WAVES
#define PP_MIN_WAVES 4
#endif
#define PP_SF64(field) (pp_const_f64(&S->field)[0])
#define PP_SI32(field) (pp_const_i32(&S->field)[0])

struct PPTrackSummary {
    int limit;
    int blocked;
    int dub_err;
    int pad;
};

#define PP_FINISH_MAX 8
struct PPCoverState {
    double cct, endTime;
    int nrib, lastEv, rdt;
    unsigned flags;
};
struct PPCurveHot { double wStart, speed, length, rho, rho_inv, qx, qy; };
__device__ __forceinline__ PPCurveHot pp_curve_hot(const PPEdgeSetup* S) {
    PPCurveHot h;
    h.wStart = PP_SF64(wStart); h.speed = PP_SF64(speed); h.length = PP_SF64(length); h.rho = PP_SF64(rho); h.rho_inv = PP_SF64(rho_inv);
    h.qx = PP_SF64(qx); h.qy = PP_SF64(qy);
    return h;
}
template <bool TAB = false>
__device__ __forceinline__ void pp_window_pose(const PPEdgeSetup* S, const PPCurveHot& c, int& cur, PPSeg& cs, double t, double tFirst, bool valid,
                                               double& x, double& y, double& uth, bool& dubErr) {
    const double tl = valid ? t : tFirst;
    double dist = (tl - c.wStart) * c.speed;
    if (__ballot((dist < 0) | (dist > c.length)) != 0ull) {
        if (dist < 0 || dist > c.length) dist = dist - 1e-5;
        if (dist < 0 || dist > c.length) { dubErr = true; dist = fmin(fmax(dist, 0.0), c.length); }
    }
    const double tprime = (c.rho_inv != 0.0) ? dist * c.rho_inv : dist / c.rho;
    double ux, uy;
    bool uniformSeg = __ballot(!((tprime >= cs.lo) & (tprime < cs.hi))) == 0ull;
    if (!uniformSeg) {
        const double hi0 = PP_SF64(p0), hi1 = PP_SF64(hi1);
        const int mine = pp_seg_of(tprime, hi0, hi1);
        const int firstSeg = __builtin_amdgcn_readfirstlane(mine);
        const int lastSeg = __builtin_amdgcn_readlane(mine, 63 - __clzll((long long)__ballot(valid)));
        if (__ballot(mine != firstSeg) != 0ull) {
            pp_setup_seg_pose<TAB>(S, mine, tprime, ux, uy, uth);
        } else {
            uniformSeg = true;
            if (cur != firstSeg) { cur = firstSeg; cs = pp_seg_load_uniform(&S->seg[cur], cur, hi0, PP_SF64(p1), hi1, PP_SI32(type)); }
        }
        if (cur != lastSeg && !uniformSeg) { cur = lastSeg; cs = pp_seg_load_uniform(&S->seg[cur], cur, hi0, PP_SF64(p1), hi1, PP_SI32(type)); }
    }
    if (uniformSeg) pp_curve_seg<TAB>(cs.type, (tprime - cs.o1) - cs.o2, cs.bx, cs.by, cs.bth, cs.sb, cs.cb, ux, uy, uth);
    x = ux * c.rho + c.qx;
    y = uy * c.rho + c.qy;
}

#ifndef PP_COVER_SINCOS_TAB
#define PP_COVER_SINCOS_TAB true
#endif
#define PP_WINDOW_POSE(S, t, t0, valid, x, y) do {                                                         \
        const PPEdgeSetup* _S = (S);                                                                       \
        asm volatile("" : "+s"(_S));                                                                       \
        const PPCurveHot _hot = pp_curve_hot(_S);                                                          \
        int _cur = -1;                                                                                     \
        PPSeg _cs = PPSeg{0, 0, 0, 0, 0, INFINITY, -INFINITY, 0, 0, 1};    \
        double _u; bool _e = false;                                                                        \
        pp_window_pose<PP_COVER_SINCOS_TAB>(_S, _hot, _cur, _cs, t, t0, valid, x, y, _u, _e);              \
    } while (0)
template <bool GAUSSIAN>
__device__ __forceinline__ bool pp_chunk_clear_of(const PPObst& o, double x, double y, double tM, double rad, double ht) {
    const double dt = tM - o.Time;
    const double X = o.X + o.Speed * dt * o.cosYaw, Y = o.Y + o.Speed * dt * o.sinYaw;
    const double slack = rad + fabs(o.Speed) * ht + 1e-3;
    const double dx = x - X, dy = y - Y;
    if (GAUSSIAN) {
        const double R = o.reach + slack;
        return dx * dx + dy * dy > R * R;
    }
    const double rx = dx * o.cosYaw - dy * o.sinYaw, ry = dx * o.sinYaw + dy * o.cosYaw;
    return (fabs(rx) > o.halfL + slack) | (fabs(ry) > o.halfW + slack);
}
#define PP_SKIP_ALL 1
#define PP_SKIP_GRID 2
#define PP_SKIP_OBST 4
#define PP_SKIP_HITS 8
#define PP_PLAN_EDGES_MAX 32
__device__ __forceinline__ void pp_plan_unit_pose(const PPEdgeSetupBody* S, double d, double& ux, double& uy) {
    const double rho = S->rho, rho_inv = S->rho_inv;
    const double tp = (rho_inv != 0.0) ? d * rho_inv : d / rho;
    double uth;
    pp_setup_seg_pose(S, pp_seg_of(tp, S->p0, S->hi1), tp, ux, uy, uth);
}
__device__ __forceinline__ void pp_plan_place(const PPEdgeSetupBody* S, double ux, double uy, double& x, double& y) {
    x = ux * S->rho + S->qx; y = uy * S->rho + S->qy;
}
__device__ __forceinline__ void pp_plan_pose(const PPEdgeSetupBody* S, double d, double& x, double& y) {
    double ux, uy;
    pp_plan_unit_pose(S, d, ux, uy);
    pp_plan_place(S, ux, uy, x, y);
}
template <bool GAUSSIAN, typename Ends, typename Each>
__device__ __forceinline__ void pp_plan_chunk(const PPParams& p, const PPEdgeSetupBody* S, const long long e, const int chunk, const double* tg,
                                              const double endTime, const double tF, Ends ends, Each each) {
    const int k0 = chunk * PP_WAVE;
    unsigned char* skipb = p.track_skip + (size_t)e * p.nch + chunk;
    if (!(tF < endTime)) { *skipb = 0; return; }
    const bool whole = k0 + PP_WAVE - 1 < p.ng;
    const bool cov = (S->cbits & PPGPU_EDGE_COVERAGE) != 0;
    const double wStart = S->wStart, speed = S->speed, length = S->length, rho = S->rho, rho_inv = S->rho_inv;
    const double tM = whole ? tg[k0 + PP_WAVE / 2] : tF, tL = whole ? tg[k0 + PP_WAVE - 1] : tF;
    const double tP = (k0 > 0) ? tg[k0 - 1] : 0.0;
    const double dP = (tP - wStart) * speed, dF = (tF - wStart) * speed, dL = (tL - wStart) * speed;
    const bool okGeom = whole && tL < endTime && (dF >= 0.0) && (dL <= length);
    const double hi0 = S->p0, hi1 = S->hi1;
    unsigned long long eqWord = ~0ull;
    double tpP = 0.0;
    int segP = 0;
    bool okHead = true;
    if (!cov) {
        tpP = (rho_inv != 0.0) ? dP * rho_inv : dP / rho;
        const double tpL = (rho_inv != 0.0) ? dL * rho_inv : dL / rho;
        segP = pp_seg_of(tpP, hi0, hi1);
        const int segL = pp_seg_of(tpL, hi0, hi1);
        const bool straight = pp_word_seg_type(S->type, segL) == 1;
        eqWord = straight ? ~0ull : 0ull;
        if (k0 > 0) {
            okHead = (dP >= 0.0) && (segP == segL) && (straight || (tpL - tpP) > 65.0 * 1e-9);
        } else {
            const double tpF = (rho_inv != 0.0) ? dF * rho_inv : dF / rho;
            const int segF = pp_seg_of(tpF, hi0, hi1);
            okHead = (dF >= 0.0) && (segF == segL) && (straight || (tpL - tpF) > 64.0 * 1e-9);
            const PPSegBase* g = &S->seg[segF];
            const int gtype = pp_word_seg_type(S->type, segF);
            const double tt = (tpF - pp_seg_o1(segF, S->p0)) - pp_seg_o2(segF, S->p1);
            const double uth0 = (gtype == 1) ? (0.0 + g->bth) : ((gtype == 0) ? (tt + g->bth) : (-tt + g->bth));
            const bool same0 = pp_heading_from_yaw(pp_mod2pi(uth0)) == S->srcH;
            eqWord = (eqWord & ~1ull) | (same0 ? 1ull : 0ull);
        }
    }
    bool gridClear = false, obstClear = false;
    int nInside = 0;
    bool decided = false;
    if (okGeom) {
        double xF, yF, xE, yE, tE = tL, dE = dL;
        ends(dF, dL, xF, yF, xE, yE, tE, dE);
        const double ht = fmax(tE - tM, tM - tF);
        const double Lc = dE - dF;
        const double dev = ((rho_inv != 0.0) ? Lc * Lc * (0.125 * rho_inv) : Lc * Lc / (8.0 * rho)) * (1.0 + 1e-9) + 1e-3;
        gridClear = true;
        if (p.grid.rows != 0) {
            const int need = (int)((0.25 * Lc + dev) * p.grid.inv_res) + 2;
            for (int h = 0; h < 2; h++) {
                const double f = h ? 0.75 : 0.25;
                const double x = xF + f * (xE - xF), y = yF + f * (yE - yF);
                const double cx = x * p.grid.inv_res, cy = y * p.grid.inv_res;
                const bool inside = (x >= 0.0) & (y >= 0.0) & (cx < (double)p.grid.cols) & (cy < (double)p.grid.rows);
                int clear = 0;
                if (inside) clear = (int)p.grid.clearance[(size_t)(unsigned)cy * p.grid.cols + (unsigned)cx];
                gridClear = gridClear && inside && (need < PP_CLEAR_CAP) && (clear > need);
            }
        }
        decided = true;
        auto against = [&](const PPObst& o) {
            if (GAUSSIAN) {
                if (!pp_chunk_clear_of<true>(o, 0.5 * (xF + xE), 0.5 * (yF + yE), tM, 0.5 * Lc + dev, ht)) decided = false;
                return;
            }
            {
                const double dtM = tM - o.Time;
                const double ddx = 0.5 * (xF + xE) - (o.X + o.Speed * dtM * o.cosYaw), ddy = 0.5 * (yF + yE) - (o.Y + o.Speed * dtM * o.sinYaw);
                const double R = o.reach + 0.5 * Lc + dev + fabs(o.Speed) * ht + 1e-3;
                if (ddx * ddx + ddy * ddy > R * R) return;
            }
            const double dtF = tF - o.Time, dtE = tE - o.Time;
            const double txF = xF - (o.X + o.Speed * dtF * o.cosYaw), tyF = yF - (o.Y + o.Speed * dtF * o.sinYaw);
            const double txE = xE - (o.X + o.Speed * dtE * o.cosYaw), tyE = yE - (o.Y + o.Speed * dtE * o.sinYaw);
            const double rxF = txF * o.cosYaw - tyF * o.sinYaw, ryF = txF * o.sinYaw + tyF * o.cosYaw;
            const double rxE = txE * o.cosYaw - tyE * o.sinYaw, ryE = txE * o.sinYaw + tyE * o.cosYaw;
            const bool out = (fmin(rxF, rxE) > o.halfL + dev) | (fmax(rxF, rxE) < -o.halfL - dev) | (fmin(ryF, ryE) > o.halfW + dev) | (fmax(ryF, ryE) < -o.halfW - dev);
            const bool in = (fmax(fabs(rxF), fabs(rxE)) < o.halfL - dev) & (fmax(fabs(ryF), fabs(ryE)) < o.halfW - dev);
            if (in) nInside++;
            else if (!out) decided = false;
        };
        each(against, decided);
        obstClear = decided && nInside == 0;
    }
    const bool ok = okGeom && okHead && gridClear && decided;
    *skipb = ok ? (unsigned char)(PP_SKIP_ALL | (nInside > 0 ? PP_SKIP_HITS : 0)) : (unsigned char)((gridClear ? PP_SKIP_GRID : 0) | (obstClear ? PP_SKIP_OBST : 0));
    if (ok) {
        p.track_chunk_hits[(size_t)e * p.nch + chunk] = (unsigned)(PP_WAVE * nInside);
        if (!cov) p.track_eq[(size_t)e * p.nch + chunk] = eqWord;
        if (GAUSSIAN) p.track_chunk_pen[(size_t)e * p.nch + chunk] = 0.0;
    } else if (!cov && k0 > 0 && dP >= 0.0 && dP <= length) {
        double ux, uy, uth;
        pp_setup_seg_pose(S, segP, tpP, ux, uy, uth);
        p.track_eq[(size_t)e * p.nch + chunk] = (unsigned long long)__double_as_longlong(pp_heading_from_yaw(pp_mod2pi(uth)));
    }
}
template <bool GAUSSIAN>
__device__ __forceinline__ void pp_plan_skips_chunk(const PPParams& p, const PPEdgeSetupBody* S, const PPObst* OB, const long long e, const int chunk) {
    const bool sane = !(S->sflags & PP_SETUP_NO_SWEEP) && S->type >= 0;
    const double endTime = fmin(p.horizon + 1e-12 + p.sst, S->wEnd);
    const double* tg = p.tgrid + (size_t)(sane ? S->vi : 0) * p.ng;
    const double tF = (sane && chunk * PP_WAVE < p.ng) ? tg[chunk * PP_WAVE] : INFINITY;
    pp_plan_chunk<GAUSSIAN>(p, S, e, chunk, tg, endTime, tF,
        [&](double dF, double dL, double& xF, double& yF, double& xE, double& yE, double&, double&) {
            double uxF, uyF, uxE, uyE;
            pp_plan_unit_pose(S, dF, uxF, uyF);
            pp_plan_unit_pose(S, dL, uxE, uyE);
            pp_plan_place(S, uxF, uyF, xF, yF);
            pp_plan_place(S, uxE, uyE, xE, yE);
        },
        [&](auto& against, const bool& decided) {
            unsigned long long m = S->omask;
            if (p.n_obst > PP_WAVE) m = 0ull;
            while (decided && m) {
                const int j = __ffsll((long long)m) - 1;
                m &= m - 1;
                against(OB[j]);
            }
            if (p.n_obst > PP_WAVE)
                for (int j = 0; j < p.n_obst && decided; j++) against(OB[j]);
        });
}
template <bool OBST_LDS>
__device__ __forceinline__ void pp_plan_stage(const PPParams& p, const long long el0, const int ne, double* s_setup, PPObst* s_obst) {
    const int tid = (int)threadIdx.x;
    const double* src = reinterpret_cast<const double*>(p.setup + p.ws_base + el0);
    for (int i = tid; i < ne * PP_SETUP_GLOBAL_WORDS; i += 256) {
        const int ed = i / PP_SETUP_GLOBAL_WORDS, w = i - ed * PP_SETUP_GLOBAL_WORDS;
        if (w < PP_SETUP_WORDS) s_setup[ed * PP_SETUP_LDS_STRIDE + w] = src[i];
    }
    if (OBST_LDS) {
        const double* os = reinterpret_cast<const double*>(p.obst);
        double* od = reinterpret_cast<double*>(s_obst);
        for (int i = tid; i < p.n_obst * (int)(sizeof(PPObst) / sizeof(double)); i += 256) od[i] = os[i];
    }
}
template <bool GAUSSIAN, bool OBST_LDS>
__device__ __forceinline__ void pp_plan_skips_thread(const PPParams& p, int epw) {
    __shared__ double s_setup[PP_PLAN_EDGES_MAX * PP_SETUP_LDS_STRIDE];
    __shared__ PPObst s_obst[OBST_LDS ? PP_WAVE : 1];
    const int tid = (int)threadIdx.x;
    const long long el0 = (long long)blockIdx.x * epw;
    const int ne = (int)((p.n_edges - el0 < (long long)epw) ? (p.n_edges - el0) : (long long)epw);
    pp_plan_stage<OBST_LDS>(p, el0, ne, s_setup, s_obst);
    __syncthreads();
    const int t = (int)blockIdx.y * 256 + tid;
    if (t >= ne * p.nch) return;
    const int el = (int)((unsigned)t / (unsigned)p.nch);
    const int chunk = t - el * p.nch;
    const PPEdgeSetupBody* S = reinterpret_cast<const PPEdgeSetupBody*>(&s_setup[el * PP_SETUP_LDS_STRIDE]);
    pp_plan_skips_chunk<GAUSSIAN>(p, S, OBST_LDS ? s_obst : p.obst, p.ws_base + el0 + el, chunk);
}
#ifndef PP_PLAN_MIN_WAVES
#define PP_PLAN_MIN_WAVES 8
#endif
__global__ __launch_bounds__(256, PP_PLAN_MIN_WAVES) void pp_k_plan_skips_chunkwise(PPParams p, int epw) { pp_plan_skips_thread<false, true>(p, epw); }
__global__ __launch_bounds__(256) void pp_k_plan_skips_many(PPParams p, int epw) { pp_plan_skips_thread<false, false>(p, epw); }
__global__ __launch_bounds__(256) void pp_k_plan_skips_gaussian_chunkwise(PPParams p, int epw) { pp_plan_skips_thread<true, true>(p, epw); }
__global__ __launch_bounds__(256) void pp_k_plan_skips_gaussian_many(PPParams p, int epw) { pp_plan_skips_thread<true, false>(p, epw); }

#ifndef PP_PLAN_SPAN
#define PP_PLAN_SPAN 4
#endif
static_assert(PP_PLAN_SPAN >= 2 && PP_PLAN_SPAN <= 32 && 256 % PP_PLAN_SPAN == 0, "a span may not straddle a 256-chunk tile of a long edge (and 256 threads clear the span words)");
#define PP_PLAN_SPANS_MAX (256 / PP_PLAN_SPAN + PP_PLAN_EDGES_MAX)
template <bool GAUSSIAN>
__device__ __forceinline__ void pp_plan_skips_spans(const PPParams& p, int epw) {
    constexpr int LOG = __builtin_ctz(PP_PLAN_SPAN);
    __shared__ double s_setup[PP_PLAN_EDGES_MAX * PP_SETUP_LDS_STRIDE];
    __shared__ PPObst s_obst[PP_WAVE];
    __shared__ double s_bx[256], s_by[256];
    __shared__ unsigned long long s_span[PP_PLAN_SPANS_MAX];
    const int tid = (int)threadIdx.x;
    const long long el0 = (long long)blockIdx.x * epw;
    const int ne = (int)((p.n_edges - el0 < (long long)epw) ? (p.n_edges - el0) : (long long)epw);
    pp_plan_stage<true>(p, el0, ne, s_setup, s_obst);
    if (tid < PP_PLAN_SPANS_MAX) s_span[tid] = 0ull;
    __syncthreads();
    const int t = (int)blockIdx.y * 256 + tid;
    const bool live = t < ne * p.nch;
    const int el = live ? (int)((unsigned)t / (unsigned)p.nch) : 0;
    const int chunk = live ? t - el * p.nch : 0;
    const PPEdgeSetupBody* S = reinterpret_cast<const PPEdgeSetupBody*>(&s_setup[el * PP_SETUP_LDS_STRIDE]);
    const int k0 = chunk * PP_WAVE;
    const bool sane = !(S->sflags & PP_SETUP_NO_SWEEP) && S->type >= 0;
    const double endTime = fmin(p.horizon + 1e-12 + p.sst, S->wEnd);
    const double* tg = p.tgrid + (size_t)(sane ? S->vi : 0) * p.ng;
    const double tF = (live && sane && k0 < p.ng) ? tg[k0] : INFINITY;
    const double wStart = S->wStart, speed = S->speed;
    {
        const double dF = (tF - wStart) * speed;
        double x = NAN, y = 0.0;
        if (tF < endTime && dF >= 0.0 && dF <= S->length) pp_plan_pose(S, dF, x, y);
        s_bx[tid] = x; s_by[tid] = y;
    }
    __syncthreads();
    const int sp = live ? el * ((p.nch + PP_PLAN_SPAN - 1) >> LOG) + ((chunk - (int)blockIdx.y * 256) >> LOG) : 0;
    {
        const int r = chunk & (PP_PLAN_SPAN - 1), cA = chunk - r, tidA = tid - r;
        const int nT = (p.nch - cA < PP_PLAN_SPAN) ? p.nch - cA : PP_PLAN_SPAN;
        unsigned long long mine = 0ull;
        for (int q = r; q < PP_PLAN_SPAN; q += nT) mine |= (~0ull / ((1ull << PP_PLAN_SPAN) - 1ull)) << q;
        unsigned long long m = live ? (S->omask & mine) : 0ull;
        unsigned long long keep = m;
        const double xA = s_bx[tidA], yA = s_by[tidA];
        if (m != 0ull && xA == xA) {
            const double tA = tg[cA * PP_WAVE], dA = (tA - wStart) * speed;
            const int cB = cA + PP_PLAN_SPAN, tidB = tidA + PP_PLAN_SPAN;
            const bool inTile = cB < p.nch && tidB < 256;
            const double xB = inTile ? s_bx[tidB] : NAN, yB = inTile ? s_by[tidB] : 0.0;
            double cx, cy, rad, tc, th;
            if (xB == xB) {
                const double tB = tg[cB * PP_WAVE], dB = (tB - wStart) * speed;
                cx = 0.5 * (xA + xB); cy = 0.5 * (yA + yB); rad = 0.5 * (dB - dA); tc = 0.5 * (tA + tB); th = 0.5 * (tB - tA);
            } else {
                const int kE = (cB * PP_WAVE < p.ng) ? cB * PP_WAVE : p.ng - 1;
                const double tE = fmin(tg[kE], endTime), dE = fmin((tE - wStart) * speed, S->length);
                cx = xA; cy = yA; rad = dE - dA; tc = tA; th = tE - tA;
            }
            if (rad >= 0.0 && th >= 0.0) {
                rad = rad * (1.0 + 1e-9) + 1e-3; th = th * (1.0 + 1e-9);
                while (m) {
                    const int j = __ffsll((long long)m) - 1;
                    m &= m - 1;
                    const PPObst& o = s_obst[j];
                    const double dt = tc - o.Time;
                    const double ddx = cx - (o.X + o.Speed * dt * o.cosYaw), ddy = cy - (o.Y + o.Speed * dt * o.sinYaw);
                    const double R = o.reach + rad + fabs(o.Speed) * th + 1e-3;
                    if (ddx * ddx + ddy * ddy > R * R) keep &= ~(1ull << j);
                }
            }
        }
        if (keep != 0ull) atomicOr(&s_span[sp], keep);
    }
    __syncthreads();
    if (!live) return;
    pp_plan_chunk<GAUSSIAN>(p, S, p.ws_base + el0 + el, chunk, tg, endTime, tF,
        [&](double, double dL, double& xF, double& yF, double& xE, double& yE, double& tE, double& dE) {
            xF = s_bx[tid]; yF = s_by[tid];
            xE = NAN; yE = 0.0;
            if (tid + 1 < 256 && chunk + 1 < p.nch) { xE = s_bx[tid + 1]; yE = s_by[tid + 1]; }
            if (xE == xE) {
                tE = tg[chunk * PP_WAVE + PP_WAVE]; dE = (tE - S->wStart) * S->speed;
            } else {
                pp_plan_pose(S, dL, xE, yE);
            }
        },
        [&](auto& against, const bool& decided) {
            unsigned long long m = s_span[sp];
            while (decided && m) {
                const int j = __ffsll((long long)m) - 1;
                m &= m - 1;
                against(s_obst[j]);
            }
        });
}
__global__ __launch_bounds__(256, PP_PLAN_MIN_WAVES) void pp_k_plan_skips(PPParams p, int epw) { pp_plan_skips_spans<false>(p, epw); }
__global__ __launch_bounds__(256, PP_PLAN_MIN_WAVES) void pp_k_plan_skips_gaussian(PPParams p, int epw) { pp_plan_skips_spans<true>(p, epw); }

template <bool GAUSSIAN>
__device__ __forceinline__ void pp_pose_sweep_edge(const PPParams& p, const long long e) {
    const int lane = pp_lane();
    const PPEdgeSetup* S = p.setup + e;
    PPTrackSummary* sum = p.track_summary + e;
    const unsigned char* skipb = p.track_skip ? p.track_skip + (size_t)e * p.nch : nullptr;
    unsigned sbits = (skipb && lane < p.nch) ? (unsigned)skipb[lane] : 0u;
    const bool laneCull = p.n_obst <= PP_WAVE;
    PPObst ol;
    if (laneCull && p.ng > 0 && p.n_obst > 0) {
        const PPObst* o = p.obst + (lane < p.n_obst ? lane : p.n_obst - 1);
        ol.X = o->X; ol.Y = o->Y; ol.cosYaw = o->cosYaw; ol.sinYaw = o->sinYaw; ol.Speed = o->Speed; ol.Time = o->Time; ol.reach = o->reach;
    }
    const unsigned sflags = (unsigned)PP_SI32(sflags);
    const int dubType = PP_SI32(type);
    const unsigned vi = (unsigned)PP_SI32(vi);
    const unsigned cbitsW = (unsigned)PP_SI32(cbits);
    const double srcH = PP_SF64(srcH);
    const PPCurveHot hot = pp_curve_hot(S);
    const double wEnd = PP_SF64(wEnd), wStart = hot.wStart, speed = hot.speed;
    const unsigned long long omask = pp_const_u64(&S->omask)[0];
    int cur = 0;
    PPSeg cs = pp_seg_load_uniform(&S->seg[0], 0, PP_SF64(p0), PP_SF64(p1), PP_SF64(hi1), dubType);
    asm volatile("" :: "s"(sflags), "s"(dubType), "s"(vi), "s"(cbitsW), "s"(srcH), "s"(hot.wStart), "s"(hot.speed), "s"(hot.length), "s"(hot.rho),
                 "s"(hot.rho_inv), "s"(hot.qx), "s"(hot.qy), "s"(wEnd), "s"(omask), "s"(cs.bx), "s"(cs.by), "s"(cs.bth), "s"(cs.sb), "s"(cs.cb),
                 "s"(cs.hi));
    const bool cov = (cbitsW & PPGPU_EDGE_COVERAGE) != 0;
    if ((sflags & PP_SETUP_NO_SWEEP) || dubType < 0) {
        if (lane == 0) { sum->limit = 0; sum->blocked = 0; sum->dub_err = 0; sum->pad = 0; }
        return;
    }
    const double endTime = fmin(p.horizon + 1e-12 + p.sst, wEnd);
    const double* tg = p.tgrid + (size_t)vi * p.ng;
    if (p.wedges && p.ng > 0) {
        const double t0 = pp_const_f64(tg)[0];
        if (t0 < endTime && t0 < wStart) {
            if (lane == 0) { sum->limit = 0; sum->blocked = 2; sum->dub_err = 0; sum->pad = 0; }
            return;
        }
    }
    unsigned short* thits = p.track_hits + (size_t)e * p.ngp;
    unsigned long long* teq = p.track_eq + (size_t)e * p.nch;
    unsigned* tch = p.track_chunk_hits + (size_t)e * p.nch;
    const bool gaussian = GAUSSIAN;
    const double chunkTime = 64.0 * (p.inc_d / p.max_speed);
    const double chunkSpan = 64.0 * (p.inc_d / p.max_speed) * speed;
    double carryHeading = srcH;
    int anyErr = 0;
    int limit = 0, blocked = 0;
    const bool anyObstacle = (p.n_obst > 0 && p.ng > 0) ? (omask != 0ull) : false;
    const double* carry = reinterpret_cast<const double*>(p.track_eq + (size_t)e * p.nch);
    int g0 = -PP_WAVE;
    unsigned long long skips = 0ull, todo = 0ull, gclear = 0ull, oclear = 0ull;
    bool lastSkipped = false;
    int ci;
    double t, carryW;
    bool after;
    auto next_chunk = [&]() {
        while (todo == 0ull) {
            lastSkipped = (g0 >= 0) && ((skips >> 63) & 1ull) != 0ull;
            g0 += PP_WAVE;
            if (g0 > 0) sbits = (skipb && g0 + lane < p.nch) ? (unsigned)skipb[g0 + lane] : 0u;
            skips = __ballot((sbits & PP_SKIP_ALL) != 0u);
            gclear = __ballot((sbits & PP_SKIP_GRID) != 0u);
            oclear = anyObstacle ? __ballot((sbits & PP_SKIP_OBST) != 0u) : ~0ull;
            todo = ~skips;
        }
        ci = __ffsll((long long)todo) - 1;
        todo &= todo - 1ull;
        after = ci > 0 ? (((skips >> (ci - 1)) & 1ull) != 0ull) : lastSkipped;
        const int k = (g0 + ci) * PP_WAVE + lane;
        t = (k < p.ng) ? tg[k] : INFINITY;
        carryW = 0.0;
        if (!cov && after && g0 + ci < p.nch) carryW = pp_const_f64(carry + (g0 + ci))[0];
    };
    next_chunk();
    __shared__ double s_cull[PP_WPB * 5 * PP_WAVE];
    double* cullL = s_cull + (size_t)__builtin_amdgcn_readfirstlane((int)(threadIdx.x >> 6)) * (5 * PP_WAVE) + lane;
    double cullT0 = 0;
    if (anyObstacle && laneCull) {
        const double t0 = pp_const_f64(tg)[0];
        cullT0 = t0;
        double oX0 = 0, oY0 = 0, oVx = 0, oVy = 0, oR2 = -1.0;
        if (lane < p.n_obst) {
            const PPObst& o = ol;
            const double dt = t0 - o.Time;
            oX0 = o.X + o.Speed * dt * o.cosYaw; oY0 = o.Y + o.Speed * dt * o.sinYaw;
            oVx = o.Speed * o.cosYaw; oVy = o.Speed * o.sinYaw;
            const double Rc = o.reach + chunkSpan + fabs(o.Speed) * chunkTime + 2e-3;
            oR2 = Rc * Rc;
        }
        cullL[0 * PP_WAVE] = oX0; cullL[1 * PP_WAVE] = oY0; cullL[2 * PP_WAVE] = oVx; cullL[3 * PP_WAVE] = oVy; cullL[4 * PP_WAVE] = oR2;
        pp_wave_lds_fence();
    }
    for (;;) {
        const double tFirst = pp_readlane(t, 0);
        const bool live = tFirst < endTime;
        double x, y, heading;
        bool dubErr = false;
        PPCellRef cell;
        uint32_t word;
        unsigned long long near = 0ull;
        if (live) {
            const bool gridClear = ((gclear >> ci) & 1ull) != 0ull, obstClear = ((oclear >> ci) & 1ull) != 0ull;
            const bool valid = t < endTime;
            double uth;
            pp_window_pose(S, hot, cur, cs, t, tFirst, valid, x, y, uth, dubErr);
            heading = cov ? 0.0 : pp_heading_from_yaw(pp_mod2pi(uth));
            if (!gridClear && p.grid.rows != 0) {
                cell = pp_blocked_cell(p.grid, x, y);
                word = p.grid.bits[cell.word];
            }
            if (!obstClear && laneCull) {
                const double dtc = tFirst - cullT0;
                const double oX0 = cullL[0 * PP_WAVE], oY0 = cullL[1 * PP_WAVE], oVx = cullL[2 * PP_WAVE], oVy = cullL[3 * PP_WAVE], oR2 = cullL[4 * PP_WAVE];
                const double ddx = pp_readlane(x, 0) - (oX0 + oVx * dtc), ddy = pp_readlane(y, 0) - (oY0 + oVy * dtc);
                near = __ballot(!(ddx * ddx + ddy * ddy > oR2));
            }
        }
        const int base = (g0 + ci) * PP_WAVE;
        const int k = base + lane;
        {
#ifdef PP_DBG_TRACE
            if (pp_edge_position(p, p.e_base + (e - p.ws_base)) == (long long)(PP_DBG_TRACE) && lane == 0 && base < 400)
                printf("[pose] chunk at %d: sampled after skip %d (eq word %llx)\n", base, (int)after, (unsigned long long)teq[base >> 6]);
#endif
            if (!live) { limit = base; break; }
            if (!cov && after) carryHeading = carryW;
            const bool obstClear = ((oclear >> ci) & 1ull) != 0ull;
            const bool valid = t < endTime;
            const bool gridTested = !(((gclear >> ci) & 1ull) != 0ull) && p.grid.rows != 0;
            const bool blk = gridTested ? (valid & pp_blocked_test(cell, word)) : false;
            int hits = 0;
            double dens = 0;
            if (obstClear) {
            } else if (laneCull) {
                unsigned long long m = near;
                while (m) {
                    const int j = __ffsll((long long)m) - 1;
                    m &= m - 1;
                    if (!gaussian) { if (valid) hits += pp_obstacle_hit(pp_obst_load_uniform(p.obst + j), x, y, t); }
                    else dens += pp_obstacle_pdf(reinterpret_cast<const PPGauss*>(p.obst)[j], x, y, t);
                }
                if (gaussian) { if (dens < 1e-5) dens = 0; if (!valid) dens = 0; }
            } else {
                if (!gaussian)
                    hits = pp_obstacle_hits_chunk(p.obst, p.n_obst, x, y, t, valid, pp_readlane(x, 0), pp_readlane(y, 0), tFirst, chunkSpan, chunkTime);
                else
                    dens = pp_obstacle_density_chunk(reinterpret_cast<const PPGauss*>(p.obst), p.n_obst, x, y, t, valid, pp_readlane(x, 0),
                                                     pp_readlane(y, 0), tFirst, chunkSpan, chunkTime);
            }
            unsigned long long eqMask = ~0ull;
            if (!cov) {
                double prevHeading = __shfl_up(heading, 1, PP_WAVE);
                if (lane == 0) prevHeading = carryHeading;
                eqMask = __ballot(prevHeading == heading);
#ifdef PP_DBG_TRACE
                if (pp_edge_position(p, p.e_base + (e - p.ws_base)) == (long long)(PP_DBG_TRACE) && lane == 0 && base < 400)
                    printf("[pose] chunk at %d sampled: carry %.17g heading0 %.17g heading1 %.17g eq %llx\n", base, prevHeading, heading, pp_readlane(heading, 1), (unsigned long long)eqMask);
#endif
                carryHeading = pp_readlane(heading, 63);
            }
            if (__ballot(dubErr) != 0ull) anyErr = 1;

            const unsigned long long bm = __ballot(blk);
            const int fb = bm ? (__ffsll((long long)bm) - 1) : PP_WAVE;
            const int nvalid = __popcll(__ballot(valid));
            const int nlim = fb < nvalid ? fb : nvalid;

            int chunkHits = 0;
            if (__ballot(hits != 0) != 0ull) {
                chunkHits = pp_wave_sum_i(lane < nlim ? hits : 0);
                thits[k] = (unsigned short)(hits > 65535 ? 65535 : hits);
            }
            if (gaussian) {
                double chunkPen = 0;
                if (__ballot(dens != 0.0) != 0ull) {
                    chunkPen = pp_wave_sum_d(lane < nlim ? dens * p.cpf : 0.0);
                    p.track_pen[(size_t)e * p.ngp + k] = dens;
                }
                if (lane == 0) p.track_chunk_pen[(size_t)e * p.nch + (base >> 6)] = chunkPen;
            }
            if (lane == 0) {
                tch[base >> 6] = (unsigned)chunkHits;
                if (!cov) teq[base >> 6] = eqMask;
            }

            if (fb < nvalid) { limit = base + fb; blocked = 1; break; }
            if (nvalid < PP_WAVE) { limit = base + nvalid; break; }
            limit = base + PP_WAVE;
        }
        next_chunk();
    }
    if (lane == 0) { sum->limit = limit; sum->blocked = blocked; sum->dub_err = anyErr; sum->pad = 0; }
}

#ifndef PP_POSE_MIN_WAVES
#define PP_POSE_MIN_WAVES 6
#endif
__global__ __launch_bounds__(PP_WPB * 64, PP_POSE_MIN_WAVES) void pp_k_pose_sweep(PPParams p) {
    int wave;
    const long long idx = pp_wave_edge<PP_WPB>(wave);
    if (idx < p.n_edges) pp_pose_sweep_edge<false>(p, p.ws_base + idx);
}
__global__ __launch_bounds__(PP_WPB * 64, 4) void pp_k_pose_sweep_gaussian(PPParams p) {
    int wave;
    const long long idx = pp_wave_edge<PP_WPB>(wave);
    if (idx < p.n_edges) pp_pose_sweep_edge<true>(p, p.ws_base + idx);
}
```

path_planner_amd/csrc/ppgpu.hip:

```cpp
#include <hip/hip_runtime.h>

#include <algorithm>
#include <cfloat>
#include <cmath>
#include <cstdio>
#include <cstdlib>
#include <cstring>
#include <memory>
#include <mutex>
#include <string>
#include <vector>

#include "../../include/ppgpu.h"
#include "pp_kernels.h"
#include "pp_sampler.h"

static thread_local std::string g_err = "";
static int fail(int code, const std::string& msg) { g_err = msg; return code; }

#define HIP_TRY(call)                                                                              \
    do {                                                                                           \
        hipError_t _e = (call);                                                                    \
        if (_e != hipSuccess)                                                                      \
            return fail(PPGPU_EHIP, std::string(#call) + ": " + hipGetErrorString(_e));            \
    } while (0)

#ifndef PP_PREPASS_MIN_EDGES
#define PP_PREPASS_MIN_EDGES 8192
#endif
#ifndef PP_SLICE_BYTES
#define PP_SLICE_BYTES (32ull << 30)
#endif
#include <atomic>
#include <chrono>
static std::atomic<unsigned long long> g_growth_count{0}, g_growth_ns{0};
struct GrowthTimer {
    std::chrono::steady_clock::time_point t0 = std::chrono::steady_clock::now();
    ~GrowthTimer() {
        g_growth_count.fetch_add(1, std::memory_order_relaxed);
        g_growth_ns.fetch_add((unsigned long long)std::chrono::duration_cast<std::chrono::nanoseconds>(std::chrono::steady_clock::now() - t0).count(), std::memory_order_relaxed);
    }
};
template <typename T>
struct DevBuf {
    T* p = nullptr;
    size_t cap = 0;
    DevBuf() = default;
    DevBuf(const DevBuf&) = delete;
    DevBuf& operator=(const DevBuf&) = delete;
    ~DevBuf() { if (p) (void)hipFree(p); }
    int reserve(size_t n, bool keep, hipStream_t s) {
        if (n <= cap) return PPGPU_OK;
        GrowthTimer growth;
        size_t ncap = cap ? cap : 64;
        while (ncap < n) ncap *= 2;
        T* np = nullptr;
        HIP_TRY(hipMalloc((void**)&np, ncap * sizeof(T)));
        hipError_t e = hipSuccess;
        if (keep && p && cap) {
            e = hipMemcpyAsync(np, p, cap * sizeof(T), hipMemcpyDeviceToDevice, s);
            if (e == hipSuccess) e = hipStreamSynchronize(s);
        }
        if (e == hipSuccess && p) e = hipFree(p);
        if (e != hipSuccess) {
            (void)hipFree(np);
            return fail(PPGPU_EHIP, std::string("DevBuf::reserve: ") + hipGetErrorString(e));
        }
        p = np; cap = ncap;
        return PPGPU_OK;
    }
};

struct ExpandWork {
    DevBuf<double> lengths;
    DevBuf<double> probe_min, groupmin, bound, key, len;
    DevBuf<int> near_idx, near_count, groupcnt, count, val, idx;
    DevBuf<unsigned> fallbacks;
    static long long list_cap(long long ns) {
        long long cap = 64;
        while (cap < ns && cap < 65536) cap <<= 1;
        return cap;
    }
    static size_t groups_row(long long ns) { return (size_t)((ns + 255) / 256) * (256 / PP_NEAR_GROUP); }
    int reserve(size_t nv, long long ns, int k, hipStream_t st) {
        const size_t lists = nv * 2 * (size_t)list_cap(ns), groups = nv * groups_row(ns);
        int rc;
        if ((rc = lengths.reserve(nv * (size_t)ns * 2, false, st)) || (rc = probe_min.reserve(nv * 2 * PP_PROBE_GROUPS, false, st)) ||
            (rc = near_idx.reserve(nv * (size_t)ns, false, st)) || (rc = near_count.reserve(nv, false, st)) ||
            (rc = groupmin.reserve(groups * 2, false, st)) || (rc = groupcnt.reserve(groups, false, st)) ||
            (rc = bound.reserve(nv * 2, false, st)) || (rc = count.reserve(nv * 2, false, st)) ||
            (rc = key.reserve(lists, false, st)) || (rc = val.reserve(lists, false, st)) || (rc = len.reserve(lists, false, st)) ||
            (rc = idx.reserve(nv * 2 * (size_t)k, false, st)) || (rc = fallbacks.reserve(1, false, st)))
            return rc;
        return PPGPU_OK;
    }
};

#define PP_TIMING_RING 8
struct TraceTimer {
    hipEvent_t ev[2] = {nullptr, nullptr};
    double ms_earlier = 0;
    bool timed = false;
};
enum { EV_BEGIN, EV_SOLVED, EV_POSED, EV_COVERED, EV_END, EV_APPROACHED, EV_COUNT };
struct ppgpu_ctx {
    int device = 0;
    hipStream_t own_stream = nullptr, stream = nullptr;
    hipStream_t side_stream = nullptr;
    hipEvent_t ev_fork = nullptr, ev_join = nullptr;
    bool have_cfg = false;
    ppgpu_config cfg{};
    DevBuf<uint32_t> grid;
    DevBuf<unsigned char> grid_clear, grid_rowclear;
    int rows = 0, cols = 0, wpr = 0;
    double res = 0;
    DevBuf<uint16_t> grid_dist;
    bool grid_dist_built = false;
    uint32_t keepout_limit2 = 0;
    DevBuf<uint32_t> grid_keepout;
    DevBuf<uint32_t> reach_labels;
    bool reach_labels_built = false;
    DevBuf<unsigned long long> reach_words;
    unsigned long long reach_free = 0, reach_components = 0, reach_cells = 0;
    bool reach_have_seed = false;
    double reach_seed_x = 0, reach_seed_y = 0;
    uint32_t reach_seed_label = PPGPU_REACH_NONE;
    bool reach_seed_fresh = false;
    DevBuf<uint32_t> reach_bits;
    DevBuf<uint16_t> reach_gap;
    bool reach_set_built = false;
    uint32_t reach_set_label = PPGPU_REACH_NONE;
    DevBuf<double> reach_ribbons;
    DevBuf<ppgpu_ribbon_reach_record> reach_records;
    TraceTimer t_reach_labels, t_reach_gap, t_reach_ribbons;
    DevBuf<PPObst> obst;
    int n_obst = 0;
    int obst_model = PPGPU_OBST_NONE;
    DevBuf<ppgpu_vertex> verts;
    DevBuf<double> ribbons, tgrid;
    int nverts = 0, nribbons = 0, ng = 0;
    DevBuf<double> sx, sy, sh;
    long long n_samples = 0;
    long long n_extra = 0;
    PPSamplerState sampler{};
    DevBuf<double> samp_ribbons;
    DevBuf<unsigned long long> samp_pos;
    int samp_group = -1;
    unsigned long long* pinned_counts = nullptr;
    std::vector<double> samp_ribbons_host;
    DevBuf<unsigned char> s_bytes;
    DevBuf<unsigned long long> s_u64;
    DevBuf<unsigned> s_u32a, s_u32b;
    DevBuf<double> s_cand;
    DevBuf<unsigned long long> tmp_edges, partial;
    DevBuf<ppgpu_wrapper_edge> tmp_wedges;
    DevBuf<ppgpu_edge_result> tmp_results;
    DevBuf<double> tmp_child, tmp_lengths, tmp_len_out, int_child;
    DevBuf<unsigned char> tmp_trace;
    DevBuf<ppgpu_cover_summary> tmp_summaries;
    DevBuf<double> tmp_cover_child;
    DevBuf<int> tmp_counts;
    TraceTimer t_steps, t_cover, t_contacts, t_clearance;
    TraceTimer t_tsp;
    TraceTimer t_dist;
    TraceTimer t_keepout;
    bool quiet_finish = true;
    bool solve_all_words = false;
    bool lane_split = true;
    bool lane_finish = true;
    bool plan_spans = true;
    bool lane_heuristic = true;
    long long prepass_min_edges = PP_PREPASS_MIN_EDGES;
    bool share_sweeps = true;
    size_t slice_bytes = PP_SLICE_BYTES;
    DevBuf<PPEdgeSetup> setup;
    DevBuf<unsigned short> track_hits;
    DevBuf<unsigned long long> track_eq;
    DevBuf<unsigned> track_chunk_hits;
    DevBuf<PPTrackSummary> track_summary;
    DevBuf<int2> track_far;
    DevBuf<unsigned char> track_skip;
    DevBuf<PPLaunchWords> words;
    DevBuf<unsigned> defer_list, live_list, hw_list;
    DevBuf<unsigned> share_head, share_of;
    bool last_launch_shared = false;
    DevBuf<PPCoverState> cover_state;
    DevBuf<unsigned long long> work;
    int n_cu = 0;
    int resident[2] = {0, 0};
    DevBuf<double> track_pen, track_chunk_pen;
    bool timing = false;
    hipEvent_t ev_ring[PP_TIMING_RING][EV_COUNT] = {};
    double ms_ring[PP_TIMING_RING][4] = {};
    int ev_slot = 0;
    long long last_launch_edges = 0;
    bool last_launch_packed = false;
    long long live_earlier_slices = 0;
    long long ev_launches = 0;
    int max_vertex_ribbons = 0;
    DevBuf<int> tmp_idx;
    ExpandWork expand;
    unsigned long long order_fallbacks = 0;
    DevBuf<unsigned char> dstage_in, dstage_out;
    void* stage_in = nullptr; size_t stage_in_cap = 0;
    void* stage_out = nullptr; size_t stage_out_cap = 0;
    DevBuf<unsigned long long> gather;
    void* comm = nullptr;
    unsigned long long hsa_gpu = 0, hsa_cpu = 0, hsa_signal = 0;
    bool copy_pending = false;
    int tsp_table_min = 0, tsp_table_max = 0;
    int tsp_dubins_min = 0, tsp_dubins_max = 0;
    int tsp_table_cap = 0;
    DevBuf<unsigned char> tsp_slots;
    DevBuf<unsigned> tsp_list;
    DevBuf<double> tsp_T;
    DevBuf<unsigned long long> tsp_words;

    __attribute__((visibility("hidden"))) ~ppgpu_ctx() {
        for (void* pinned : {(void*)pinned_counts, stage_in, stage_out}) if (pinned) (void)hipHostFree(pinned);
        for (auto& set : ev_ring) for (hipEvent_t e : set) if (e) (void)hipEventDestroy(e);
        for (hipEvent_t e : {t_steps.ev[0], t_steps.ev[1], t_cover.ev[0], t_cover.ev[1], t_contacts.ev[0], t_contacts.ev[1], t_clearance.ev[0], t_clearance.ev[1], t_tsp.ev[0], t_tsp.ev[1], t_dist.ev[0], t_dist.ev[1], t_keepout.ev[0], t_keepout.ev[1],
                             t_reach_labels.ev[0], t_reach_labels.ev[1], t_reach_gap.ev[0], t_reach_gap.ev[1], t_reach_ribbons.ev[0], t_reach_ribbons.ev[1], ev_fork, ev_join}) if (e) (void)hipEventDestroy(e);
        for (hipStream_t s : {side_stream, own_stream}) if (s) (void)hipStreamDestroy(s);
    }
};

static int require_cfg(ppgpu_ctx* c) {
    if (!c) return fail(PPGPU_EINVAL, "null context");
    if (!c->have_cfg) return fail(PPGPU_ESTATE, "ppgpu_set_config must be called first");
    return PPGPU_OK;
}

static int require_vertices(ppgpu_ctx* c) {
    int rc = require_cfg(c);
    if (rc) return rc;
    if (c->nverts <= 0) return fail(PPGPU_ESTATE, "ppgpu_set_vertices must be called (after ppgpu_set_config)");
    return PPGPU_OK;
}

static int require_world(ppgpu_ctx* c) {
    int rc = require_vertices(c);
    if (rc) return rc;
    if (c->n_samples + c->n_extra <= 0) return fail(PPGPU_ESTATE, "no targets: call ppgpu_sampler_add, ppgpu_set_samples or ppgpu_set_extra_targets");
    return PPGPU_OK;
}

static int check_open_vertices(const ppgpu_ctx* c, const char* who, int n, const ppgpu_vertex* hv, int n_ribbons, int* max_ribbons) {
    *max_ribbons = 0;
    for (int i = 0; i < n; i++) {
        if (hv[i].ribbon_count < 0 || hv[i].ribbon_offset < 0 || hv[i].ribbon_offset + hv[i].ribbon_count > n_ribbons)
            return fail(PPGPU_EINVAL, std::string(who) + ": ribbon range outside the pool");
        if (hv[i].ribbon_count > PP_WAVE) return fail(PPGPU_ECAPACITY, std::string(who) + ": more than 64 ribbons on one vertex");
        if (hv[i].time < c->cfg.start_state_time) return fail(PPGPU_EINVAL, std::string(who) + ": vertex time before start_state_time");
        if (hv[i].ribbon_count > *max_ribbons) *max_ribbons = hv[i].ribbon_count;
    }
    return PPGPU_OK;
}

static int check_wrapper_edges(const ppgpu_ctx* c, const char* who, int64_t n, const ppgpu_wrapper_edge* w) {
    for (int64_t i = 0; i < n; i++) {
        if (!(w[i].rho > 0) || !(w[i].speed > 0)) return fail(PPGPU_EINVAL, std::string(who) + ": rho and speed must be positive");
        if (w[i].vertex < 0 || w[i].vertex >= c->nverts) return fail(PPGPU_EINVAL, std::string(who) + ": vertex out of range");
    }
    return PPGPU_OK;
}

namespace { struct CtxDelete { void operator()(ppgpu_ctx* c) const { delete c; } }; }
static void ppgpu_copy_engine_release(ppgpu_ctx* c);
extern "C" int ppgpu_copy_engine_wait(ppgpu_ctx* c);

extern "C" {

const char* ppgpu_last_error(void) { return g_err.c_str(); }

int ppgpu_create(int device, ppgpu_ctx** out) {
    if (!out) return fail(PPGPU_EINVAL, "out is null");
    *out = nullptr;
    int n = 0;
    if (hipGetDeviceCount(&n) != hipSuccess || n <= 0) return fail(PPGPU_ENODEV, "no HIP device visible");
    if (device < 0 || device >= n) return fail(PPGPU_ENODEV, "device index out of range");
    HIP_TRY(hipSetDevice(device));
    hipDeviceProp_t prop;
    HIP_TRY(hipGetDeviceProperties(&prop, device));
    if (std::strncmp(prop.gcnArchName, "gfx950", 6) != 0)
        return fail(PPGPU_ENODEV, std::string("device is ") + prop.gcnArchName + ", this library carries gfx950 code only");
    std::unique_ptr<ppgpu_ctx, CtxDelete> c(new ppgpu_ctx());
    c->device = device;
    c->n_cu = prop.multiProcessorCount;
    HIP_TRY(hipStreamCreateWithFlags(&c->own_stream, hipStreamNonBlocking));
    c->stream = c->own_stream;
    HIP_TRY(hipStreamCreateWithFlags(&c->side_stream, hipStreamNonBlocking));
    HIP_TRY(hipEventCreateWithFlags(&c->ev_fork, hipEventDisableTiming));
    HIP_TRY(hipEventCreateWithFlags(&c->ev_join, hipEventDisableTiming));
    HIP_TRY(hipHostMalloc((void**)&c->pinned_counts, 64, hipHostMallocDefault));
    if (const char* pm = std::getenv("PPGPU_PREPASS_MIN_EDGES")) c->prepass_min_edges = std::atoll(pm);
    if (const char* lh = std::getenv("PPGPU_LANE_HEURISTIC")) c->lane_heuristic = std::atoi(lh) != 0;
    if (const char* qf = std::getenv("PPGPU_QUIET_FINISH")) c->quiet_finish = std::atoi(qf) != 0;
    if (const char* lf = std::getenv("PPGPU_LANE_FINISH")) c->lane_finish = std::atoi(lf) != 0;
    if (const char* ls = std::getenv("PPGPU_LANE_SPLIT")) c->lane_split = std::atoi(ls) != 0;
    if (const char* aw = std::getenv("PPGPU_SOLVE_ALL_WORDS")) c->solve_all_words = std::atoi(aw) != 0;
    if (const char* ps = std::getenv("PPGPU_PLAN_SPANS")) c->plan_spans = std::atoi(ps) != 0;
    if (const char* ss = std::getenv("PPGPU_SHARE_SWEEPS")) c->share_sweeps = std::atoi(ss) != 0;
    if (const char* sb = std::getenv("PPGPU_SLICE_BYTES")) {
        const long long v = std::atoll(sb);
        if (v > 0) c->slice_bytes = (size_t)v;
    }
    *out = c.release();
    return PPGPU_OK;
}

int ppgpu_destroy(ppgpu_ctx* c) {
    if (!c) return PPGPU_OK;
    (void)hipSetDevice(c->device);
    (void)hipStreamSynchronize(c->stream);
    if (c->comm) (void)ppgpu_comm_destroy(c);
    if (c->copy_pending) (void)ppgpu_copy_engine_wait(c);
    ppgpu_copy_engine_release(c);
    delete c;
    return PPGPU_OK;
}

int ppgpu_set_stream(ppgpu_ctx* c, void* s) {
    if (!c) return fail(PPGPU_EINVAL, "null context");
    c->stream = s ? (hipStream_t)s : c->own_stream;
    return PPGPU_OK;
}

int ppgpu_enable_timing(ppgpu_ctx* c, int32_t on) {
    if (!c) return fail(PPGPU_EINVAL, "null context");
    HIP_TRY(hipSetDevice(c->device));
    if (on && !c->ev_ring[0][0])
        for (int r = 0; r < PP_TIMING_RING; r++) for (int i = 0; i < EV_COUNT; i++) HIP_TRY(hipEventCreate(&c->ev_ring[r][i]));
    for (TraceTimer* tm : {&c->t_steps, &c->t_cover, &c->t_contacts, &c->t_clearance, &c->t_tsp, &c->t_dist}) {
        if (on && !tm->ev[0])
            for (int i = 0; i < 2; i++) HIP_TRY(hipEventCreate(&tm->ev[i]));
        tm->timed = false;
    }
    c->t_keepout.timed = false;
    c->t_reach_labels.timed = c->t_reach_gap.timed = c->t_reach_ribbons.timed = false;
    c->timing = on != 0;
    c->ev_launches = 0;
    return PPGPU_OK;
}

static int slice_durations(hipEvent_t* ev, float ms[4]) {
    HIP_TRY(hipEventElapsedTime(&ms[0], ev[EV_BEGIN], ev[EV_SOLVED]));
    HIP_TRY(hipEventElapsedTime(&ms[1], ev[EV_SOLVED], ev[EV_POSED]));
    HIP_TRY(hipEventElapsedTime(&ms[2], ev[EV_APPROACHED], ev[EV_COVERED]));
    HIP_TRY(hipEventElapsedTime(&ms[3], ev[EV_POSED], ev[EV_APPROACHED]));
    return PPGPU_OK;
}

int ppgpu_past_timing(ppgpu_ctx* c, int32_t back, double* ms_solve, double* ms_pose, double* ms_cover, double* ms_heuristic) {
    if (!c || !ms_solve || !ms_pose || !ms_cover || !ms_heuristic) return fail(PPGPU_EINVAL, "null argument");
    if (!c->timing || c->ev_launches == 0) return fail(PPGPU_ESTATE, "no timed costing launch (ppgpu_enable_timing, then cost edges)");
    if (back < 0 || back >= PP_TIMING_RING || back >= c->ev_launches) return fail(PPGPU_EINVAL, "past_timing: that launch is no longer (or not yet) in the ring");
    HIP_TRY(hipSetDevice(c->device));
    const int slot = (c->ev_slot - back + PP_TIMING_RING) % PP_TIMING_RING;
    hipEvent_t* ev = c->ev_ring[slot];
    HIP_TRY(hipEventSynchronize(ev[EV_END]));
    float t[4] = {0, 0, 0, 0}, tail = 0;
    int rc = slice_durations(ev, t);
    if (rc) return rc;
    HIP_TRY(hipEventElapsedTime(&tail, ev[EV_COVERED], ev[EV_END]));
    *ms_solve = t[0] + c->ms_ring[slot][0]; *ms_pose = t[1] + c->ms_ring[slot][1]; *ms_cover = t[2] + c->ms_ring[slot][2];
    *ms_heuristic = tail + t[3] + c->ms_ring[slot][3];
    return PPGPU_OK;
}
int ppgpu_last_timing(ppgpu_ctx* c, double* ms_solve, double* ms_pose, double* ms_cover, double* ms_heuristic) {
    return ppgpu_past_timing(c, 0, ms_solve, ms_pose, ms_cover, ms_heuristic);
}

int ppgpu_last_cover_edges(ppgpu_ctx* c, int64_t* n_edges) {
    if (!c || !n_edges) return fail(PPGPU_EINVAL, "null argument");
    HIP_TRY(hipSetDevice(c->device));
    *n_edges = c->last_launch_edges;
    if (c->last_launch_packed) {
        unsigned live = 0;
        HIP_TRY(hipStreamSynchronize(c->stream));
        HIP_TRY(hipMemcpy(&live, &c->words.p->live_count, sizeof(unsigned), hipMemcpyDeviceToHost));
        *n_edges = (int64_t)live + c->live_earlier_slices;
    }
    return PPGPU_OK;
}

int ppgpu_last_shared_edges(ppgpu_ctx* c, int64_t* n_edges) {
    if (!c || !n_edges) return fail(PPGPU_EINVAL, "null argument");
    HIP_TRY(hipSetDevice(c->device));
    *n_edges = 0;
    if (!c->last_launch_shared || c->last_launch_edges <= 0) return PPGPU_OK;
    std::vector<unsigned> of((size_t)c->last_launch_edges);
    HIP_TRY(hipStreamSynchronize(c->stream));
    HIP_TRY(hipMemcpy(of.data(), c->share_of.p, of.size() * sizeof(unsigned), hipMemcpyDeviceToHost));
    int64_t n = 0;
    for (unsigned h : of) n += (h != PP_SHARE_NONE);
    *n_edges = n;
    return PPGPU_OK;
}

int ppgpu_reserve_samples(ppgpu_ctx* c, int64_t max_samples, int32_t max_vertices) {
    if (!c) return fail(PPGPU_EINVAL, "null context");
    if (max_samples <= 0 || max_vertices <= 0) return fail(PPGPU_EINVAL, "reserve_samples: sizes must be positive");
    HIP_TRY(hipSetDevice(c->device));
    hipStream_t st = c->stream;
    const size_t ns = (size_t)max_samples, nv = (size_t)max_vertices;
    const size_t nq = 6 * (size_t)524288 + 8;
    int rc;
    if ((rc = c->sx.reserve(ns + nv, true, st)) || (rc = c->sy.reserve(ns + nv, true, st)) || (rc = c->sh.reserve(ns + nv, true, st)) ||
        (rc = c->s_cand.reserve((size_t)524288 * 3, false, st)) || (rc = c->s_bytes.reserve(nq + 64, false, st)) || (rc = c->s_u32a.reserve(nq + 64, false, st)) ||
        (rc = c->expand.reserve(nv, max_samples, 0, st)))
        return rc;
    return PPGPU_OK;
}

int ppgpu_growth_stats(ppgpu_ctx* c, uint64_t* count, double* seconds) {
    if (!c) return fail(PPGPU_EINVAL, "null context");
    if (count) *count = g_growth_count.load(std::memory_order_relaxed);
    if (seconds) *seconds = 1e-9 * (double)g_growth_ns.load(std::memory_order_relaxed);
    return PPGPU_OK;
}

static int set_table_range(ppgpu_ctx* c, int32_t min_ribbons, int32_t max_ribbons, int& range_min, int& range_max, bool dubins) {
    if (!c) return fail(PPGPU_EINVAL, "null context");
    if (min_ribbons < 0 || max_ribbons < 0 || max_ribbons > PP_TSP_TABLE_MAX || (max_ribbons > 0 && min_ribbons > max_ribbons))
        return fail(PPGPU_EINVAL, "set_tsp_table: 0 <= min_ribbons <= max_ribbons <= 16 (max_ribbons = 0: off)");
    HIP_TRY(hipSetDevice(c->device));
    HIP_TRY(hipStreamSynchronize(c->stream));
    if (max_ribbons > 0) {
        int rc = c->tsp_words.p ? PPGPU_OK : c->tsp_words.reserve(4, false, c->stream);
        if (rc) return rc;
        if (c->tsp_table_cap == 0) HIP_TRY(hipMemsetAsync(c->tsp_words.p, 0, 4 * sizeof(unsigned long long), c->stream));
        const int cap = max_ribbons > c->tsp_table_cap ? max_ribbons : c->tsp_table_cap;
        size_t slots = (size_t)PP_TSP_TABLE_BYTES / pp_tt_slot_bytes(cap);
        if (slots > PP_TT_GRID) slots = PP_TT_GRID;
        if (slots < 1) return fail(PPGPU_ECAPACITY, "set_tsp_table: PP_TSP_TABLE_BYTES holds no slot");
        if (cap != c->tsp_table_cap) {
            if (c->tsp_slots.p) { HIP_TRY(hipFree(c->tsp_slots.p)); c->tsp_slots.p = nullptr; c->tsp_slots.cap = 0; }
            GrowthTimer growth;
            HIP_TRY(hipMalloc((void**)&c->tsp_slots.p, slots * pp_tt_slot_bytes(cap)));
            c->tsp_slots.cap = slots * pp_tt_slot_bytes(cap);
            c->tsp_table_cap = cap;
        }
        if ((rc = c->tsp_list.reserve(1u << 20, false, c->stream))) return rc;
        if (dubins && (rc = c->tsp_T.reserve((size_t)PP_TT_TCAP * PP_TT_TSTRIDE, false, c->stream))) return rc;
        HIP_TRY(hipStreamSynchronize(c->stream));
    }
    range_min = min_ribbons; range_max = max_ribbons;
    return PPGPU_OK;
}

int ppgpu_set_tsp_table(ppgpu_ctx* c, int32_t min_ribbons, int32_t max_ribbons) {
    return c ? set_table_range(c, min_ribbons, max_ribbons, c->tsp_table_min, c->tsp_table_max, false) : fail(PPGPU_EINVAL, "null context");
}

int ppgpu_set_dubins_tsp_table(ppgpu_ctx* c, int32_t min_ribbons, int32_t max_ribbons) {
    return c ? set_table_range(c, min_ribbons, max_ribbons, c->tsp_dubins_min, c->tsp_dubins_max, true) : fail(PPGPU_EINVAL, "null context");
}

int ppgpu_tsp_table_stats(ppgpu_ctx* c, uint64_t* lists, uint64_t* refused) {
    if (!c || !lists || !refused) return fail(PPGPU_EINVAL, "null argument");
    unsigned long long w[2] = {0, 0};
    if (c->tsp_words.p) {
        HIP_TRY(hipSetDevice(c->device));
        HIP_TRY(hipMemcpyAsync(w, c->tsp_words.p, sizeof(w), hipMemcpyDeviceToHost, c->stream));
        HIP_TRY(hipStreamSynchronize(c->stream));
    }
    *lists = w[0]; *refused = w[1];
    return PPGPU_OK;
}

int ppgpu_synchronize(ppgpu_ctx* c) {
    if (!c) return fail(PPGPU_EINVAL, "null context");
    HIP_TRY(hipStreamSynchronize(c->stream));
    return PPGPU_OK;
}

int ppgpu_device_alloc(ppgpu_ctx* c, uint64_t bytes, void** d_out) {
    if (!c || !d_out || bytes == 0) return fail(PPGPU_EINVAL, "device_alloc: bad arguments");
    HIP_TRY(hipSetDevice(c->device));
    HIP_TRY(hipMalloc(d_out, (size_t)bytes));
    return PPGPU_OK;
}
int ppgpu_device_free(ppgpu_ctx* c, void* d_ptr) {
    if (!c) return fail(PPGPU_EINVAL, "null context");
    if (!d_ptr) return PPGPU_OK;
    HIP_TRY(hipSetDevice(c->device));
    HIP_TRY(hipStreamSynchronize(c->stream));
    HIP_TRY(hipFree(d_ptr));
    return PPGPU_OK;
}
int ppgpu_device_read(ppgpu_ctx* c, void* h_dst, const void* d_src, uint64_t bytes) {
    if (!c || !h_dst || !d_src) return fail(PPGPU_EINVAL, "device_read: null argument");
    HIP_TRY(hipSetDevice(c->device));
    HIP_TRY(hipMemcpyAsync(h_dst, d_src, (size_t)bytes, hipMemcpyDeviceToHost, c->stream));
    HIP_TRY(hipStreamSynchronize(c->stream));
    return PPGPU_OK;
}

int ppgpu_set_config(ppgpu_ctx* c, const ppgpu_config* cfg) {
    if (!c || !cfg) return fail(PPGPU_EINVAL, "null argument");
    if (!(cfg->max_speed > 0) || !(cfg->collision_checking_increment > 0) || !(cfg->turning_radius > 0) ||
        !(cfg->coverage_turning_radius > 0) || !(cfg->time_horizon > 0))
        return fail(PPGPU_EINVAL, "config: speeds, radii, increment and horizon must be positive");
    if (cfg->heuristic < PPGPU_H_MAX_DISTANCE || cfg->heuristic > PPGPU_H_TSP_DUBINS_K)
        return fail(PPGPU_EINVAL, "config: unknown heuristic");
    if ((cfg->heuristic == PPGPU_H_TSP_DUBINS_ALL || cfg->heuristic == PPGPU_H_TSP_DUBINS_K) && !(cfg->heuristic_turning_radius > 0))
        return fail(PPGPU_EINVAL, "config: the Dubins-TSP heuristics need heuristic_turning_radius > 0 "
                                  "(RibbonManager throws \"Cannot compute ribbon dubins distance with unset turning radius\")");
    double steps = cfg->time_horizon / (cfg->collision_checking_increment / cfg->max_speed);
    if (!(steps < 60000.0)) return fail(PPGPU_ECAPACITY, "config: more than 60000 collision-check steps per edge");
    c->cfg = *cfg;
    c->have_cfg = true;
    c->ng = (int)steps + 8;
    c->nverts = 0;
    return PPGPU_OK;
}

static const uint32_t* grid_bits(const ppgpu_ctx* c) { return c->keepout_limit2 ? c->grid_keepout.p : c->grid.p; }
static void launch_grid_clear(ppgpu_ctx* c, const uint32_t* bits, int rows, int cols, int wpr) {
    const long long ncell = (long long)rows * cols;
    hipLaunchKernelGGL(pp_k_grid_row_clear, dim3((unsigned)((ncell + 255) / 256)), dim3(256), 0, c->stream, bits, rows, cols, wpr, c->grid_rowclear.p);
    hipLaunchKernelGGL(pp_k_grid_clear, dim3((unsigned)((ncell + 255) / 256)), dim3(256), 0, c->stream, c->grid_rowclear.p, rows, cols, c->grid_clear.p);
}
static int apply_keepout(ppgpu_ctx* c);

int ppgpu_set_grid(ppgpu_ctx* c, const uint8_t* cells, int32_t rows, int32_t cols, double res) {
    if (!c) return fail(PPGPU_EINVAL, "null context");
    HIP_TRY(hipSetDevice(c->device));
    c->grid_dist_built = false;
    c->reach_labels_built = false;
    if (rows == 0) { c->rows = c->cols = c->wpr = 0; c->res = 0; return PPGPU_OK; }
    if (!cells || rows < 0 || cols <= 0 || !(res > 0)) return fail(PPGPU_EINVAL, "grid: bad shape or resolution");
    int wpr = (cols + 31) / 32;
    std::vector<uint32_t> bits((size_t)rows * wpr, 0u);
    for (int r = 0; r < rows; r++) {
        const uint8_t* row = cells + (size_t)r * cols;
        uint32_t* brow = bits.data() + (size_t)r * wpr;
        for (int x = 0; x < cols; x++)
            if (row[x]) brow[x >> 5] |= 1u << (x & 31);
    }
    int rc = c->grid.reserve(bits.size(), false, c->stream);
    if (rc) return rc;
    HIP_TRY(hipMemcpyAsync(c->grid.p, bits.data(), bits.size() * sizeof(uint32_t), hipMemcpyHostToDevice, c->stream));
    if ((rc = c->grid_clear.reserve((size_t)rows * cols, false, c->stream)) || (rc = c->grid_rowclear.reserve((size_t)rows * cols, false, c->stream)))
        return rc;
    if (c->keepout_limit2) {
        c->rows = rows; c->cols = cols; c->wpr = wpr; c->res = res;
        return apply_keepout(c);
    }
// ... 515 lines not shown
    HIP_TRY(hipMemcpyAsync(y.data(), c->sy.p + first, (size_t)n * sizeof(double), hipMemcpyDeviceToHost, c->stream));
    HIP_TRY(hipMemcpyAsync(h.data(), c->sh.p + first, (size_t)n * sizeof(double), hipMemcpyDeviceToHost, c->stream));
    HIP_TRY(hipStreamSynchronize(c->stream));
    for (int64_t i = 0; i < n; i++) {
        out5[5 * i] = x[(size_t)i]; out5[5 * i + 1] = y[(size_t)i]; out5[5 * i + 2] = h[(size_t)i];
        out5[5 * i + 3] = c->cfg.max_speed;
        out5[5 * i + 4] = 0;
    }
    return PPGPU_OK;
}

int64_t ppgpu_num_samples(ppgpu_ctx* c) { return c ? c->n_samples : 0; }

int ppgpu_sampler_init(ppgpu_ctx* c, const double* b6, uint64_t seed, int32_t n_ribbons, const double* hr) {
    int rc = require_cfg(c);
    if (rc) return rc;
    HIP_TRY(hipSetDevice(c->device));
    if (!b6) return fail(PPGPU_EINVAL, "sampler: bounds are null");
    if (n_ribbons > 0 && !hr) return fail(PPGPU_EINVAL, "sampler: ribbons are null");
    if (n_ribbons > 1024) return fail(PPGPU_ECAPACITY, "sampler: more than 1024 ribbons");
    PPSamplerState& s = c->sampler;
    for (int i = 0; i < 6; i++) s.b[i] = b6[i];
    unsigned long long x = seed % 2147483647ull;
    s.seed = (unsigned)(x == 0 ? 1 : x);
    s.on_ribbons = n_ribbons >= 0 ? 1 : 0;
    s.n_ribbons = n_ribbons > 0 ? n_ribbons : 0;
    const int kPosGroups = 1024;
    if (!c->samp_pos.p) c->samp_group = -1;
    if ((rc = c->samp_pos.reserve((size_t)8 * kPosGroups, false, c->stream))) return rc;
    c->samp_group = (c->samp_group + 1) % kPosGroups;
    if (c->samp_group == 0)
        HIP_TRY(hipMemsetAsync(c->samp_pos.p, 0, (size_t)8 * kPosGroups * sizeof(unsigned long long), c->stream));
    s.d_pos = c->samp_pos.p + (size_t)8 * c->samp_group;
    s.initialised = 1;
    if (n_ribbons > 0) {
        const size_t nd = (size_t)n_ribbons * 4;
        if (c->samp_ribbons_host.size() != nd || std::memcmp(c->samp_ribbons_host.data(), hr, nd * sizeof(double)) != 0) {
            if ((rc = c->samp_ribbons.reserve(nd, false, c->stream))) return rc;
            c->samp_ribbons_host.clear();
            HIP_TRY(hipMemcpyAsync(c->samp_ribbons.p, hr, nd * sizeof(double), hipMemcpyHostToDevice, c->stream));
            HIP_TRY(hipStreamSynchronize(c->stream));
            c->samp_ribbons_host.assign(hr, hr + nd);
        }
    }
    c->n_samples = 0;
    c->n_extra = 0;
    return PPGPU_OK;
}

static int sampler_chain(ppgpu_ctx* c, long long n, long long& nq, int& nblk_q, unsigned long long** d_end, bool skip = false) {
    PPSamplerState& s = c->sampler;
    hipStream_t st = c->stream;
    int rc;
    nq = s.on_ribbons ? (6 * n + 8) : n;
    nblk_q = (int)((nq + PP_SCAN_TILE - 1) / PP_SCAN_TILE);
    if (nblk_q > PP_SCAN_TILE) return fail(PPGPU_ECAPACITY, "sampler: batch too large for the two-level scan (max ~690k samples per call)");
    if ((rc = c->s_bytes.reserve((size_t)nq + 64 + (size_t)n + 64, false, st))) return rc;
    if ((rc = c->s_u64.reserve((size_t)nblk_q + 64, false, st))) return rc;
    if ((rc = c->s_u32a.reserve((size_t)nq + 64, false, st))) return rc;
    {
        const size_t nblk_n = (size_t)((n + 255) / 256);
        if ((rc = c->s_u32b.reserve(((size_t)nblk_q > nblk_n ? (size_t)nblk_q : nblk_n) + 64, false, st))) return rc;
    }
    *d_end = c->s_u64.p + nblk_q + 8;
    if (!s.on_ribbons) { HIP_TRY(hipMemsetAsync(c->s_u64.p + nblk_q + 8, 0, 16 * sizeof(unsigned long long), st)); return PPGPU_OK; }
    unsigned char* proj = c->s_bytes.p;
    unsigned* tilefn = reinterpret_cast<unsigned*>(c->s_u64.p);
    hipLaunchKernelGGL(pp_k_proj_reduce, dim3(nblk_q), dim3(256), 0, st, s.seed, s.d_pos, nq, proj, tilefn, c->s_u64.p + nblk_q + 8);
    hipLaunchKernelGGL(pp_k_chain_apply_count, dim3(nblk_q), dim3(256), 0, st, proj, nq, tilefn, c->s_u32b.p);
    hipLaunchKernelGGL(pp_k_chain_positions_scan, dim3(nblk_q), dim3(256), 0, st, proj, nq, c->s_u32b.p, n, c->s_u32a.p, *d_end,
                       skip ? const_cast<unsigned long long*>(s.d_pos) : (unsigned long long*)nullptr);
    HIP_TRY(hipGetLastError());
    return PPGPU_OK;
}

int ppgpu_sampler_skip(ppgpu_ctx* c, int64_t n_attempts) {
    int rc = require_cfg(c);
    if (rc) return rc;
    HIP_TRY(hipSetDevice(c->device));
    if (!c->sampler.initialised) return fail(PPGPU_ESTATE, "ppgpu_sampler_init must be called first");
    if (n_attempts < 0) return fail(PPGPU_EINVAL, "sampler: negative count");
    PPSamplerState& s = c->sampler;
    long long left = n_attempts;
    while (left > 0) {
        long long n = left < 524288 ? left : 524288;
        long long nq = 0; int nblk_q = 0; unsigned long long* d_end = nullptr;
        if (s.on_ribbons) {
            if ((rc = sampler_chain(c, n, nq, nblk_q, &d_end, true))) return rc;
        } else {
            hipLaunchKernelGGL(pp_k_sampler_advance, dim3(1), dim3(1), 0, c->stream, const_cast<unsigned long long*>(s.d_pos), d_end, (const unsigned long long*)nullptr,
                               4ull * (unsigned long long)n, 0);
            HIP_TRY(hipGetLastError());
        }
        left -= n;
    }
    return PPGPU_OK;
}

int ppgpu_sampler_add(ppgpu_ctx* c, int64_t n_attempts, int64_t* n_total_out) {
    int rc = require_cfg(c);
    if (rc) return rc;
    HIP_TRY(hipSetDevice(c->device));
    if (!c->sampler.initialised) return fail(PPGPU_ESTATE, "ppgpu_sampler_init must be called first");
    if (n_attempts < 0) return fail(PPGPU_EINVAL, "sampler: negative count");
    if (n_attempts == 0) { if (n_total_out) *n_total_out = c->n_samples; return PPGPU_OK; }
    if (n_attempts > 524288) return fail(PPGPU_ECAPACITY, "sampler: at most 524288 attempts per call");
    const long long n = n_attempts;
    PPSamplerState& s = c->sampler;
    hipStream_t st = c->stream;
    size_t need_samples = (size_t)(c->n_samples + n);
    if ((rc = c->sx.reserve(need_samples, true, st)) || (rc = c->sy.reserve(need_samples, true, st)) ||
        (rc = c->sh.reserve(need_samples, true, st)))
        return rc;
    if ((rc = c->s_cand.reserve((size_t)n * 3, false, st))) return rc;
    long long nq; int nblk_q; unsigned long long* d_end;
    if ((rc = sampler_chain(c, n, nq, nblk_q, &d_end))) return rc;
    const int nblk_n = (int)((n + 255) / 256);
    unsigned char* proj = c->s_bytes.p;
    unsigned* qpos = c->s_u32a.p;
    unsigned* blk32 = c->s_u32b.p;
    PPGrid g{grid_bits(c), c->rows, c->cols, c->wpr, c->res, c->res > 0 ? 1.0 / c->res : 0.0, nullptr};
    unsigned char* keep = c->s_bytes.p + (size_t)nq + 64;
    hipLaunchKernelGGL(pp_k_generate_keep, dim3((unsigned)nblk_n), dim3(256), 0, st, s, s.on_ribbons ? qpos : nullptr, s.on_ribbons ? proj : nullptr,
                       c->samp_ribbons.p, n, c->s_cand.p, g, keep, blk32);
    unsigned long long* d_total = d_end + 8;
    hipLaunchKernelGGL(pp_k_compact_scan, dim3((unsigned)nblk_n), dim3(256), 0, st, keep, n, blk32, c->s_cand.p, c->sx.p, c->sy.p,
                       c->sh.p, c->n_samples, d_total);
    HIP_TRY(hipGetLastError());
    hipLaunchKernelGGL(pp_k_sampler_advance, dim3(1), dim3(1), 0, st, const_cast<unsigned long long*>(s.d_pos), d_end, d_total, 4ull * (unsigned long long)n, s.on_ribbons);
    HIP_TRY(hipGetLastError());
    volatile unsigned long long* h2 = c->pinned_counts;
    h2[0] = 0; h2[1] = 0; h2[2] = 0;
    HIP_TRY(hipMemcpyAsync((void*)&h2[0], s.d_pos + 1, 3 * sizeof(unsigned long long), hipMemcpyDeviceToHost, st));
    HIP_TRY(hipStreamSynchronize(st));
    if (h2[0] != 0) return fail(PPGPU_EHIP, "sampler: chain scan did not reach the end of the batch (this call or a ppgpu_sampler_skip before it)");
    c->n_samples += (long long)h2[1];
    c->n_extra = 0;
    if (n_total_out) *n_total_out = c->n_samples;
    return PPGPU_OK;
}

static void fill_params(ppgpu_ctx* c, PPParams& p) {
    const ppgpu_config& g = c->cfg;
    p.max_speed = g.max_speed;
    p.slow_speed = g.slow_speed <= 0 ? g.max_speed : g.slow_speed;
    p.rho = g.turning_radius; p.rho_cov = g.coverage_turning_radius;
    p.horizon = g.time_horizon; p.tmin = g.time_minimum; p.inc_d = g.collision_checking_increment;
    p.sst = g.start_state_time; p.ribw = g.ribbon_width;
    p.inv_inc_d = 1.0 / p.inc_d;
    p.cpf = g.collision_penalty_factor; p.tpf = g.time_penalty_factor;
    p.heuristic = g.heuristic; p.tsp_k = g.tsp_k; p.h_rho = g.heuristic_turning_radius;
    p.fuse_h = 0;
    p.lane_split = 0; p.defer_h = 0; p.defer_list = nullptr; p.quiet_finish = 0; p.live_list = nullptr; p.cover_state = nullptr; p.hw_list = nullptr; p.words = nullptr; p.reset_words = 0;
    p.share_head = nullptr; p.share_of = nullptr;
    p.grid = PPGrid{grid_bits(c), c->rows, c->cols, c->wpr, c->res, c->res > 0 ? 1.0 / c->res : 0.0, c->rows > 0 ? c->grid_clear.p : nullptr};
    p.obst = c->obst.p; p.n_obst = c->n_obst; p.obst_model = c->obst_model;
    p.verts = c->verts.p; p.ribbons = c->ribbons.p; p.tgrid = c->tgrid.p; p.ng = c->ng; p.nverts = c->nverts;
    p.sx = c->sx.p; p.sy = c->sy.p; p.sh = c->sh.p; p.n_samples = c->n_samples + c->n_extra;
}

int ppgpu_dubins_lengths(ppgpu_ctx* c, int32_t v0, int32_t nv, double* d_lengths) {
    int rc = require_world(c);
    if (rc) return rc;
    HIP_TRY(hipSetDevice(c->device));
    if (v0 < 0 || nv <= 0 || v0 + nv > c->nverts || !d_lengths) return fail(PPGPU_EINVAL, "dubins_lengths: vertex range");
    if (nv > 65535) return fail(PPGPU_ECAPACITY, "dubins_lengths: at most 65535 vertices per call");
    const long long ns = c->n_samples;
    if (ns <= 0) return fail(PPGPU_ESTATE, "dubins_lengths: the sample store is empty");
    hipLaunchKernelGGL(pp_k_dubins_lengths, dim3((unsigned)((ns + 255) / 256), (unsigned)nv), dim3(256), 0, c->stream, c->verts.p,
                       v0, c->sx.p, c->sy.p, c->sh.p, ns, c->cfg.turning_radius, c->cfg.coverage_turning_radius,
                       c->cfg.collision_checking_increment, d_lengths);
    HIP_TRY(hipGetLastError());
    return PPGPU_OK;
}

int ppgpu_select_nearest(ppgpu_ctx* c, int32_t v0, int32_t nv, int32_t k, int32_t* h_idx, double* h_len) {
    int rc = require_world(c);
    if (rc) return rc;
    HIP_TRY(hipSetDevice(c->device));
    if (k <= 0 || !h_idx || !h_len) return fail(PPGPU_EINVAL, "select_nearest: bad arguments");
    const long long ns = c->n_samples;
    if ((rc = c->expand.lengths.reserve((size_t)nv * ns * 2, false, c->stream))) return rc;
    if ((rc = ppgpu_dubins_lengths(c, v0, nv, c->expand.lengths.p))) return rc;
    size_t nout = (size_t)nv * 2 * k;
    if ((rc = c->tmp_idx.reserve(nout, false, c->stream)) || (rc = c->tmp_len_out.reserve(nout, false, c->stream))) return rc;
    hipLaunchKernelGGL(pp_k_select_nearest, dim3((unsigned)(nv * 2)), dim3(256), 0, c->stream, c->expand.lengths.p, ns, k,
                       c->tmp_idx.p, c->tmp_len_out.p);
    HIP_TRY(hipGetLastError());
    HIP_TRY(hipMemcpyAsync(h_idx, c->tmp_idx.p, nout * sizeof(int), hipMemcpyDeviceToHost, c->stream));
    HIP_TRY(hipMemcpyAsync(h_len, c->tmp_len_out.p, nout * sizeof(double), hipMemcpyDeviceToHost, c->stream));
    HIP_TRY(hipStreamSynchronize(c->stream));
    return PPGPU_OK;
}

struct ExpandLoops { int two_speeds, two_radii; };
static ExpandLoops expand_loops(const ppgpu_config& g) {
    const double slow = g.slow_speed <= 0 ? g.max_speed : g.slow_speed;
    return {slow != g.max_speed ? 1 : 0, g.coverage_turning_radius != g.turning_radius ? 1 : 0};
}

static int launch_expand_order(ppgpu_ctx* c, int nv, int k, bool zero_fallbacks = true) {
    const long long ns = c->n_samples;
    ExpandWork& w = c->expand;
    hipStream_t st = c->stream;
    int rc;
    if ((rc = w.reserve((size_t)nv, ns, k, st))) return rc;
    if (zero_fallbacks) HIP_TRY(hipMemsetAsync(w.fallbacks.p, 0, sizeof(unsigned), st));
    const ppgpu_config& g = c->cfg;
    PPExpandArgs a{};
    a.verts = c->verts.p; a.sx = c->sx.p; a.sy = c->sy.p; a.sh = c->sh.p; a.ns = ns;
    a.k = k; a.two_radii = expand_loops(g).two_radii;
    a.rho = g.turning_radius; a.rho_cov = g.coverage_turning_radius; a.inc_d = g.collision_checking_increment;
    a.max_speed = g.max_speed; a.tpf = g.time_penalty_factor;
    a.probe_min = w.probe_min.p; a.near_idx = w.near_idx.p; a.near_count = w.near_count.p; a.lengths = w.lengths.p;
    a.groupmin = w.groupmin.p; a.groupcnt = w.groupcnt.p; a.groups_row = (int)ExpandWork::groups_row(ns);
    a.bound = w.bound.p; a.cand_count = w.count.p;
    a.g_key = w.key.p; a.g_val = w.val.p; a.g_len = w.len.p; a.g_cap = ExpandWork::list_cap(ns);
    a.out_idx = w.idx.p; a.fallbacks = w.fallbacks.p;
    const dim3 per_sample((unsigned)((ns + 255) / 256), (unsigned)nv), per_list((unsigned)(nv * 2));
    hipLaunchKernelGGL(pp_k_expand_probe, dim3((unsigned)(PP_PROBE / 256), (unsigned)nv), dim3(256), 0, st, a);
    hipLaunchKernelGGL(pp_k_expand_near, dim3((unsigned)((ns + 256 * PP_NEAR_PER - 1) / (256 * PP_NEAR_PER)), (unsigned)nv), dim3(256), 0, st, a);
    hipLaunchKernelGGL(pp_k_near_lengths, per_sample, dim3(256), 0, st, a);
    hipLaunchKernelGGL(pp_k_expand_bound, per_list, dim3(256), 0, st, a);
    hipLaunchKernelGGL(pp_k_expand_candidates, per_sample, dim3(256), 0, st, a);
    hipLaunchKernelGGL(pp_k_expand_order, per_list, dim3(256), 0, st, a);
    HIP_TRY(hipGetLastError());
    return PPGPU_OK;
}

int ppgpu_expand_order(ppgpu_ctx* c, int32_t v0, int32_t nv, int32_t k, int32_t* h_idx, uint32_t* h_fallbacks) {
    int rc = require_world(c);
    if (rc) return rc;
    HIP_TRY(hipSetDevice(c->device));
    if (k <= 0 || !h_idx || v0 != 0 || nv <= 0 || nv > c->nverts) return fail(PPGPU_EINVAL, "expand_order: bad arguments (v0 must be 0)");
    if (nv > 65535) return fail(PPGPU_ECAPACITY, "expand_order: at most 65535 vertices per call");
    if (c->n_samples <= 0) return fail(PPGPU_ESTATE, "expand_order: the sample store is empty");
    const size_t nout = (size_t)nv * 2 * k;
    if ((rc = launch_expand_order(c, nv, k))) return rc;
    unsigned fb = 0;
    HIP_TRY(hipMemcpyAsync(h_idx, c->expand.idx.p, nout * sizeof(int), hipMemcpyDeviceToHost, c->stream));
    HIP_TRY(hipMemcpyAsync(&fb, c->expand.fallbacks.p, sizeof(unsigned), hipMemcpyDeviceToHost, c->stream));
    HIP_TRY(hipStreamSynchronize(c->stream));
    c->order_fallbacks += fb;
    if (h_fallbacks) *h_fallbacks = fb;
    return PPGPU_OK;
}

uint64_t ppgpu_order_fallbacks(ppgpu_ctx* c) { return c ? c->order_fallbacks : 0; }

int64_t ppgpu_dense_edge_count(int32_t nv, int64_t ns, uint32_t cfg_mask) {
    return (int64_t)nv * ns * (int64_t)__builtin_popcount(cfg_mask & 0xFu);
}

static unsigned resident_grid(ppgpu_ctx* c, bool gaussian, long long n_edges) {
    int& resident = c->resident[gaussian ? 1 : 0];
    if (resident == 0) {
        const void* kernel = gaussian ? (const void*)pp_k_cover_sweep_gaussian : (const void*)pp_k_cover_sweep;
        int per_cu = 0;
        if (hipOccupancyMaxActiveBlocksPerMultiprocessor(&per_cu, kernel, PP_WPB * 64, 0) != hipSuccess || per_cu <= 0) per_cu = 2;
        resident = per_cu * (c->n_cu > 0 ? c->n_cu : 256);
    }
    const long long need = (n_edges + PP_WPB - 1) / PP_WPB;
    return (unsigned)(need < resident ? need : resident);
}

static PPParams list_params(ppgpu_ctx* c, long long n, const unsigned long long* d_edges, const ppgpu_wrapper_edge* d_wedges,
                            ppgpu_edge_result* d_out, double* d_child, int stride) {
    PPParams p;
    fill_params(c, p);
    p.edges = d_edges; p.wedges = d_wedges;
    p.v0 = 0; p.nv = 0; p.s0 = 0; p.ns = 1; p.cfg_mask = 0; p.per = 1;
    p.n_edges = n;
    p.out = d_out; p.child = d_child; p.stride = stride;
    return p;
}

struct CostLaunch {
    PPParams p;
    bool gaussian;
    bool prepasses;
    bool skip_chunks;
    bool packed;
    bool lane_finish;
    bool fuse_h;
    bool defer_h;
    bool quiet_finish, lane_split;
    bool forked;
    bool share;
    bool share_child;
    int nch, ngp;
    long long slice;
};

static void cost_modes(const ppgpu_ctx* c, CostLaunch& m) {
    const PPParams& p = m.p;
    const long long total = p.n_edges;
    m.gaussian = p.n_obst > 0 && p.obst_model == PPGPU_OBST_GAUSSIAN;
    m.nch = (p.ng + PP_WAVE - 1) / PP_WAVE;
    if (m.nch < 1) m.nch = 1;
    m.ngp = m.nch * PP_WAVE;
    const size_t per_edge = sizeof(PPEdgeSetup) + (size_t)m.ngp * sizeof(unsigned short) +
                            (size_t)m.nch * (sizeof(unsigned long long) + sizeof(unsigned)) + sizeof(PPTrackSummary) +
                            (m.gaussian ? (size_t)(m.ngp + m.nch) * sizeof(double) : 0);
    m.slice = (long long)(c->slice_bytes / per_edge);
    if (m.slice < PP_WPB) m.slice = PP_WPB;
    if (m.slice > total) m.slice = total;
    m.prepasses = total >= c->prepass_min_edges;
    m.skip_chunks = m.prepasses && !p.wedges && (c->rows == 0 || c->grid_clear.p) && p.ng >= PP_WAVE;
    const bool dubinsH = p.heuristic == PPGPU_H_TSP_DUBINS_ALL || p.heuristic == PPGPU_H_TSP_DUBINS_K;
    m.fuse_h = PP_FUSE_HEUR && !dubinsH && !m.gaussian;
    m.defer_h = m.fuse_h && m.prepasses && c->lane_heuristic && total < (1ll << 32) &&
                (p.heuristic == PPGPU_H_TSP_POINT_ALL || p.heuristic == PPGPU_H_TSP_POINT_K);
    m.quiet_finish = m.prepasses && c->quiet_finish;
    m.lane_split = m.prepasses && c->lane_split && !m.gaussian;
    m.packed = m.prepasses && total < (1ll << 32);
#if defined(PP_DBG_COUNTS)
    const bool laneFinishBuilt = false;
#else
    const bool laneFinishBuilt = true;
#endif
    m.lane_finish = laneFinishBuilt && m.packed && c->lane_finish && !m.gaussian;
    m.forked = m.lane_finish && m.fuse_h && p.heuristic != PPGPU_H_MAX_DISTANCE;
    m.share = m.prepasses && m.packed && !p.wedges && c->share_sweeps && (long long)p.nverts * PP_SHARE_KEYS < (1ll << 32);
    m.share_child = m.share && p.child != nullptr;
}

static int cost_workspace(ppgpu_ctx* c, CostLaunch& m) {
    PPParams& p = m.p;
    const size_t total = (size_t)p.n_edges, ws = (size_t)m.slice;
    hipStream_t st = c->stream;
    int rc;
    if (!p.child) {
        int stride = c->max_vertex_ribbons + 8;
        if (stride > PP_WAVE) stride = PP_WAVE;
        if ((rc = c->int_child.reserve(total * stride * 4, false, st))) return rc;
        p.child = c->int_child.p;
        p.stride = stride;
    }
    p.nch = m.nch; p.ngp = m.ngp;
    if ((rc = c->setup.reserve(ws, false, st)) || (rc = c->track_hits.reserve(ws * p.ngp, false, st)) ||
        (rc = c->track_eq.reserve(ws * p.nch, false, st)) || (rc = c->track_chunk_hits.reserve(ws * p.nch, false, st)) ||
        (rc = c->track_summary.reserve(ws, false, st)) || (rc = c->track_far.reserve(ws, false, st)) ||
        (rc = c->track_skip.reserve(ws * p.nch, false, st)))
        return rc;
    if (m.gaussian && ((rc = c->track_pen.reserve(ws * p.ngp, false, st)) || (rc = c->track_chunk_pen.reserve(ws * p.nch, false, st))))
        return rc;
    if ((rc = c->words.reserve(1, false, st)) || (rc = c->work.reserve(PP_WORK_WORDS, false, st))) return rc;
    p.setup = c->setup.p; p.track_hits = c->track_hits.p; p.track_eq = c->track_eq.p;
    p.track_chunk_hits = c->track_chunk_hits.p; p.track_summary = c->track_summary.p;
    p.track_far = m.prepasses ? c->track_far.p : nullptr;
    p.track_skip = m.skip_chunks ? c->track_skip.p : nullptr;
    p.track_pen = c->track_pen.p; p.track_chunk_pen = c->track_chunk_pen.p;
    p.words = c->words.p; p.reset_words = 1;
    p.work = c->work.p;
    p.fuse_h = m.fuse_h; p.defer_h = m.defer_h; p.quiet_finish = m.quiet_finish; p.lane_split = m.lane_split;
    if (m.packed) {
        if ((rc = c->live_list.reserve(ws * 2, false, st))) return rc;
        p.live_list = c->live_list.p;
    }
    if (m.lane_finish) {
        if ((rc = c->cover_state.reserve(ws, false, st)) || (rc = c->hw_list.reserve(total, false, st))) return rc;
        p.cover_state = c->cover_state.p; p.hw_list = c->hw_list.p;
    }
    if (m.defer_h) {
        if ((rc = c->defer_list.reserve(total * PP_HL_MAX_N, false, st))) return rc;
        p.defer_list = c->defer_list.p;
    }
    if (m.share) {
        if ((rc = c->share_head.reserve((size_t)p.nverts * PP_SHARE_KEYS, false, st)) || (rc = c->share_of.reserve(total, false, st))) return rc;
        p.share_head = c->share_head.p; p.share_of = c->share_of.p;
    }
    return PPGPU_OK;
}

static int bank_slice_timing(ppgpu_ctx* c, bool packed) {
    hipEvent_t* ev = c->ev_ring[c->ev_slot];
    HIP_TRY(hipEventSynchronize(ev[EV_COVERED]));
    float ms[4] = {0, 0, 0, 0};
    int rc = slice_durations(ev, ms);
    if (rc) return rc;
    for (int i = 0; i < 4; i++) c->ms_ring[c->ev_slot][i] += ms[i];
    if (packed) { unsigned live = 0; HIP_TRY(hipMemcpy(&live, &c->words.p->live_count, sizeof(unsigned), hipMemcpyDeviceToHost)); c->live_earlier_slices += live; }
    return PPGPU_OK;
}

static int cost_slice(ppgpu_ctx* c, const CostLaunch& m) {
    const PPParams& p = m.p;
    hipStream_t st = c->stream;
    hipEvent_t* ev = c->ev_ring[c->ev_slot];
    if (c->timing) HIP_TRY(hipEventRecord(ev[EV_BEGIN], st));
    hipLaunchKernelGGL(c->solve_all_words ? pp_k_solve_edges_all_words : pp_k_solve_edges, dim3((unsigned)((p.n_edges + 255) / 256)), dim3(256), 0, st, p);
    if (m.share) hipLaunchKernelGGL(pp_k_share_mark, dim3((unsigned)((p.n_edges + 255) / 256)), dim3(256), 0, st, p);
    if (c->timing) HIP_TRY(hipEventRecord(ev[EV_SOLVED], st));
    if (m.skip_chunks) {
        int epw = 256 / p.nch;
        if (epw < 1) epw = 1;
        if (epw > PP_PLAN_EDGES_MAX) epw = PP_PLAN_EDGES_MAX;
        const unsigned blocks = (unsigned)((p.n_edges + epw - 1) / epw);
        const bool many = p.n_obst > PP_WAVE;
        void (*planner)(PPParams, int) = m.gaussian ? (many ? pp_k_plan_skips_gaussian_many : (c->plan_spans ? pp_k_plan_skips_gaussian : pp_k_plan_skips_gaussian_chunkwise))
                                                    : (many ? pp_k_plan_skips_many : (c->plan_spans ? pp_k_plan_skips : pp_k_plan_skips_chunkwise));
        hipLaunchKernelGGL(planner, dim3(blocks, (unsigned)((epw * p.nch + 255) / 256)), dim3(256), 0, st, p, epw);
    }
    hipLaunchKernelGGL(m.gaussian ? pp_k_pose_sweep_gaussian : pp_k_pose_sweep, dim3((unsigned)((p.n_edges + PP_WPB - 1) / PP_WPB)), dim3(PP_WPB * 64), 0, st, p);
    if (c->timing) HIP_TRY(hipEventRecord(ev[EV_POSED], st));
    if (m.prepasses) hipLaunchKernelGGL(pp_k_approach_events, dim3((unsigned)((p.n_edges + PP_APPROACH_THREADS - 1) / PP_APPROACH_THREADS)), dim3(PP_APPROACH_THREADS), 0, st, p);
    if (c->timing) HIP_TRY(hipEventRecord(ev[EV_APPROACHED], st));
    hipLaunchKernelGGL(m.gaussian ? pp_k_cover_sweep_gaussian : pp_k_cover_sweep, dim3(resident_grid(c, m.gaussian, p.n_edges)), dim3(PP_WPB * 64), 0, st, p);
    if (m.lane_finish)
        hipLaunchKernelGGL(pp_k_cover_finish, dim3((unsigned)((p.n_edges + PP_FINISH_THREADS - 1) / PP_FINISH_THREADS)), dim3(PP_FINISH_THREADS), 0, st, p);
    if (c->timing) HIP_TRY(hipEventRecord(ev[EV_COVERED], st));
    return PPGPU_OK;
}

static int tsp_table_pass(ppgpu_ctx* c, const PPParams& p) {
    const bool point = p.heuristic == PPGPU_H_TSP_POINT_ALL || p.heuristic == PPGPU_H_TSP_POINT_K;
    const bool dubins = p.heuristic == PPGPU_H_TSP_DUBINS_ALL || p.heuristic == PPGPU_H_TSP_DUBINS_K;
    if (!point && !dubins) return PPGPU_OK;
    const int range_min = dubins ? c->tsp_dubins_min : c->tsp_table_min, range_max = dubins ? c->tsp_dubins_max : c->tsp_table_max;
    if (range_max <= 0 || !p.child || p.stride <= 0 || p.n_edges <= 0) return PPGPU_OK;
    hipStream_t st = c->stream;
    PPTspTableArgs q;
    q.out = p.out; q.child = p.child; q.stride = p.stride; q.n_edges = p.n_edges;
    q.heuristic = p.heuristic; q.tsp_k = p.tsp_k; q.ribw = p.ribw; q.max_speed = p.max_speed; q.tpf = p.tpf; q.h_rho = p.h_rho;
    q.min_ribbons = range_min; q.max_ribbons = range_max;
    q.list = c->tsp_list.p; q.list_cap = (unsigned)c->tsp_list.cap; q.count = (unsigned*)(c->tsp_words.p + 2); q.stats = c->tsp_words.p;
    q.slots = c->tsp_slots.p; q.bytes = c->tsp_slots.cap;
    q.T = dubins ? c->tsp_T.p : nullptr;
    if (dubins && q.list_cap > PP_TT_TCAP) q.list_cap = PP_TT_TCAP;
    if (c->timing) HIP_TRY(hipEventRecord(c->t_tsp.ev[0], st));
    HIP_TRY(hipMemsetAsync(c->tsp_words.p + 2, 0, sizeof(unsigned long long), st));
    hipLaunchKernelGGL(pp_k_tsp_table_list, dim3((unsigned)((p.n_edges + 255) / 256)), dim3(256), 0, st, q);
    const long long grid = p.n_edges < PP_TT_GRID ? p.n_edges : PP_TT_GRID;
    if (dubins) hipLaunchKernelGGL(pp_k_tsp_table_dubins_T, dim3((unsigned)grid), dim3(256), 0, st, q);
    hipLaunchKernelGGL(dubins ? pp_k_tsp_table_dubins : pp_k_tsp_table, dim3((unsigned)grid), dim3(PP_TT_THREADS), 0, st, q);
    if (c->timing) { HIP_TRY(hipEventRecord(c->t_tsp.ev[1], st)); c->t_tsp.ms_earlier = 0; c->t_tsp.timed = true; }
    return PPGPU_OK;
}

static int cost_heuristic_tail(ppgpu_ctx* c, const CostLaunch& m) {
    const PPParams& p = m.p;
    const long long total = p.n_edges;
    hipStream_t st = c->stream;
    const dim3 per_wave((unsigned)((total + PP_H_WPB - 1) / PP_H_WPB));
    if (p.heuristic == PPGPU_H_TSP_DUBINS_ALL || p.heuristic == PPGPU_H_TSP_DUBINS_K)
        hipLaunchKernelGGL(pp_k_heuristic_dubins, per_wave, dim3(PP_H_WPB * 64), 0, st, p);
    else if (!m.fuse_h)
        hipLaunchKernelGGL(pp_k_heuristic, per_wave, dim3(PP_H_WPB * 64), 0, st, p);
    if (m.forked) {
        HIP_TRY(hipEventRecord(c->ev_fork, st));
        HIP_TRY(hipStreamWaitEvent(c->side_stream, c->ev_fork, 0));
        hipLaunchKernelGGL(pp_k_heuristic_listed, per_wave, dim3(PP_H_WPB * 64), 0, c->side_stream, p);
        HIP_TRY(hipEventRecord(c->ev_join, c->side_stream));
    }
    if (m.defer_h) {
        hipLaunchKernelGGL(pp_k_deferred_list, dim3((unsigned)((total + 256 * PP_DL_PER - 1) / (256 * PP_DL_PER))), dim3(256), 0, st, p);
        hipLaunchKernelGGL(pp_k_heuristic_lanes, dim3((unsigned)((total * PP_HL_SPLIT + PP_HL_THREADS - 1) / PP_HL_THREADS) + PP_HL_MAX_N), dim3(PP_HL_THREADS), 0, st, p);
    }
    if (p.heuristic == PPGPU_H_TSP_POINT_K)
        hipLaunchKernelGGL(pp_k_heuristic_big, dim3((unsigned)(total < PP_BIG_GRID ? total : PP_BIG_GRID)), dim3(PP_BIG_WPB * 64), 0, st, p);
    if (m.forked) HIP_TRY(hipStreamWaitEvent(st, c->ev_join, 0));
    int rc = tsp_table_pass(c, p);
    if (rc) return rc;
    if (m.share) hipLaunchKernelGGL(pp_k_share_fanout, dim3((unsigned)((total + 15) / 16)), dim3(256), 0, st, p, m.share_child ? 1 : 0);
    return PPGPU_OK;
}

static int launch_cost(ppgpu_ctx* c, const PPParams& asked, CostLaunch* done = nullptr) {
    CostLaunch local;
    CostLaunch& m = done ? *done : local;
    m.p = asked;
    PPParams& p = m.p;
    const long long total = p.n_edges;
    if (total <= 0) return PPGPU_OK;
    p.total_edges = total;
    if ((total + PP_WPB - 1) / PP_WPB > 0x3fffffffll) return fail(PPGPU_ECAPACITY, "cost_edges: too many edges for one launch");
    cost_modes(c, m);
    int rc = cost_workspace(c, m);
    if (rc) return rc;
    if (c->timing) c->ev_slot = (int)(c->ev_launches % PP_TIMING_RING);
    for (double& ms : c->ms_ring[c->ev_slot]) ms = 0;
    c->live_earlier_slices = 0;
    c->last_launch_shared = false;
    if (m.share) HIP_TRY(hipMemsetAsync(p.share_head, 0xff, (size_t)p.nverts * PP_SHARE_KEYS * sizeof(unsigned), c->stream));
    for (long long e0 = 0; e0 < total; e0 += m.slice) {
        p.e_base = e0; p.ws_base = 0; p.n_edges = (total - e0 < m.slice) ? (total - e0) : m.slice;
        if (c->timing && e0 > 0 && (rc = bank_slice_timing(c, m.packed))) return rc;
        if ((rc = cost_slice(c, m))) return rc;
    }
    p.e_base = 0;
    p.n_edges = total;
    if ((rc = cost_heuristic_tail(c, m))) return rc;
    c->last_launch_edges = total; c->last_launch_packed = m.packed; c->last_launch_shared = m.share;
    if (c->timing) { HIP_TRY(hipEventRecord(c->ev_ring[c->ev_slot][EV_END], c->stream)); c->ev_launches++; }
    HIP_TRY(hipGetLastError());
    return PPGPU_OK;
}

int ppgpu_cost_edges_dense(ppgpu_ctx* c, int32_t v0, int32_t nv, int64_t s0, int64_t ns, uint32_t cfg_mask,
                           ppgpu_edge_result* d_results, double* d_child, int32_t stride) {
    int rc = require_world(c);
    if (rc) return rc;
    HIP_TRY(hipSetDevice(c->device));
    cfg_mask &= 0xFu;
    if (v0 < 0 || nv <= 0 || v0 + nv > c->nverts) return fail(PPGPU_EINVAL, "cost_edges_dense: vertex range");
    if (s0 < 0 || ns <= 0 || s0 + ns > c->n_samples) return fail(PPGPU_EINVAL, "cost_edges_dense: sample range");
    if (!cfg_mask || !d_results) return fail(PPGPU_EINVAL, "cost_edges_dense: empty configuration mask or null results");
    if (d_child && stride <= 0) return fail(PPGPU_EINVAL, "cost_edges_dense: ribbon_stride must be positive");
    PPParams p;
    fill_params(c, p);
    p.edges = nullptr; p.wedges = nullptr;
    p.v0 = v0; p.nv = nv; p.s0 = s0; p.ns = ns; p.cfg_mask = cfg_mask; p.per = __builtin_popcount(cfg_mask);
    p.n_edges = (long long)nv * ns * p.per;
    p.out = d_results; p.child = d_child; p.stride = stride;
    return launch_cost(c, p);
}

int ppgpu_cost_edges_list(ppgpu_ctx* c, int64_t n, const uint64_t* d_edges, ppgpu_edge_result* d_results, double* d_child,
                          int32_t stride) {
    int rc = require_world(c);
    if (rc) return rc;
    HIP_TRY(hipSetDevice(c->device));
    if (n < 0 || (n > 0 && (!d_edges || !d_results))) return fail(PPGPU_EINVAL, "cost_edges_list: bad arguments");
    if (d_child && stride <= 0) return fail(PPGPU_EINVAL, "cost_edges_list: ribbon_stride must be positive");
    return launch_cost(c, list_params(c, n, (const unsigned long long*)d_edges, nullptr, d_results, d_child, stride));
}

enum TraceKind { TRACE_STEPS, TRACE_COVER, TRACE_CONTACTS, TRACE_CLEARANCE };
struct TraceRequest {
    TraceKind kind;
    int32_t stride;
    int32_t* counts;
    void* records;
    size_t rec_bytes;
    ppgpu_cover_summary* summaries;
    double* child;
    int32_t ribbon_stride;
    uint32_t limit2;
};
static TraceRequest steps_request(int32_t stride, int32_t* counts, ppgpu_step_record* steps) {
    return TraceRequest{TRACE_STEPS, stride, counts, steps, sizeof(ppgpu_step_record), nullptr, nullptr, 0, 0};
}
static TraceRequest cover_request(int32_t stride, int32_t* counts, ppgpu_cover_record* cover, ppgpu_cover_summary* summaries, double* child, int32_t ribbon_stride) {
    return TraceRequest{TRACE_COVER, stride, counts, cover, sizeof(ppgpu_cover_record), summaries, child, ribbon_stride, 0};
}
static TraceRequest contacts_request(int32_t* counts, ppgpu_contact_record* contacts) {
    return TraceRequest{TRACE_CONTACTS, 0, counts, contacts, sizeof(ppgpu_contact_record), nullptr, nullptr, 0, 0};
}
static TraceRequest clearance_request(int32_t* counts, ppgpu_clearance_record* clearance, uint32_t limit2) {
    return TraceRequest{TRACE_CLEARANCE, 1, counts, clearance, sizeof(ppgpu_clearance_record), nullptr, nullptr, 0, limit2};
}
static int clearance_limit2(const ppgpu_ctx* c, const char* who, double margin, uint32_t* limit2) {
    *limit2 = 0;
    if (c->rows == 0 || !(margin > 0)) return PPGPU_OK;
    if (ppgpu_keepout_limit2(c->res, margin, limit2)) return fail(PPGPU_EINVAL, std::string(who) + ": margin above 255 cells");
    return PPGPU_OK;
}

static int trace_request_args(const ppgpu_ctx* c, const char* who, bool device, int64_t n, const void* edges, const void* results, const TraceRequest& r) {
    static const char* const records_name[] = {"d_steps", "d_cover", "d_contacts", "d_clearance"};
    const bool cover = r.kind == TRACE_COVER, contacts = r.kind == TRACE_CONTACTS;
    if (n < 0 || (n > 0 && (!edges || !r.counts || ((!contacts || c->n_obst > 0) && !r.records)))) return fail(PPGPU_EINVAL, std::string(who) + ": bad arguments");
    if (!contacts && (r.stride <= 0 || r.stride > 65535)) return fail(PPGPU_EINVAL, std::string(who) + ": step_stride must be in 1 .. 65535");
    if (device) {
        if (n > 0 && (!results || (cover && !r.summaries))) return fail(PPGPU_EINVAL, std::string(who) + (cover ? ": null results or summaries" : ": null results"));
    } else if (cover && n > 0 && !r.summaries) {
        return fail(PPGPU_EINVAL, std::string(who) + ": null summaries");
    }
    if (cover && r.child && r.ribbon_stride <= 0) return fail(PPGPU_EINVAL, std::string(who) + ": ribbon_stride must be positive");
    if (device && ((unsigned long long)r.records & 15ull) != 0ull)
        return fail(PPGPU_EINVAL, std::string(who) + ": " + records_name[r.kind] + " must be 16-byte aligned");
    return PPGPU_OK;
}

static void trace_kernel(ppgpu_ctx* c, const CostLaunch& L, const PPParams& q, const TraceRequest& r, void* dst, long long rec_base) {
    const dim3 grid((unsigned)((q.n_edges + PP_TRACE_WPB - 1) / PP_TRACE_WPB)), block(PP_TRACE_WPB * 64);
    switch (r.kind) {
    case TRACE_STEPS:
        hipLaunchKernelGGL(L.gaussian ? pp_k_trace_steps_gaussian : pp_k_trace_steps, grid, block, 0, c->stream, q, (ppgpu_step_record*)dst, rec_base, r.stride, r.counts);
        break;
    case TRACE_COVER:
        hipLaunchKernelGGL(pp_k_trace_cover, grid, block, 0, c->stream, q, (ppgpu_cover_record*)dst, rec_base, r.stride, r.counts, r.summaries, r.child,
                           r.child ? r.ribbon_stride : 0);
        break;
    case TRACE_CONTACTS:
        hipLaunchKernelGGL(L.gaussian ? pp_k_trace_contacts_gaussian : pp_k_trace_contacts, grid, block, 0, c->stream, q, (ppgpu_contact_record*)dst, rec_base, r.counts);
        break;
    case TRACE_CLEARANCE:
        hipLaunchKernelGGL(pp_k_trace_clearance, grid, block, 0, c->stream, q, c->grid_dist.p, r.limit2, (ppgpu_clearance_record*)dst, rec_base, r.counts);
        break;
    }
}

static int trace_passes(ppgpu_ctx* c, const CostLaunch& L, const TraceRequest& r, TraceTimer& tm, int stride, unsigned char* recs, bool host) {
    const PPParams& p = L.p;
    const long long total = p.n_edges;
    const bool reuse = L.slice >= total;
    const size_t edge_bytes = (size_t)stride * r.rec_bytes;
    long long pass = reuse ? total : L.slice;
    if (host) {
        long long cap = (long long)(c->slice_bytes / edge_bytes);
        if (cap < 1) cap = 1;
        if (pass > cap) pass = cap;
        int rc = c->tmp_trace.reserve((size_t)pass * edge_bytes, false, c->stream);
        if (rc) return rc;
    }
    tm.ms_earlier = 0;
    tm.timed = false;
    for (long long e0 = 0; e0 < total; e0 += pass) {
        PPParams q = p;
        q.e_base = e0; q.n_edges = (total - e0 < pass) ? (total - e0) : pass;
        q.ws_base = reuse ? e0 : 0;
        if (!reuse) {
            q.reset_words = 0;
            q.share_head = nullptr;
            hipLaunchKernelGGL(c->solve_all_words ? pp_k_solve_edges_all_words : pp_k_solve_edges, dim3((unsigned)((q.n_edges + 255) / 256)), dim3(256), 0, c->stream, q);
        }
        unsigned char* dst = host ? c->tmp_trace.p : recs;
        const size_t bytes = (size_t)q.n_edges * edge_bytes;
        if (host) HIP_TRY(hipMemcpyAsync(dst, recs + (size_t)e0 * edge_bytes, bytes, hipMemcpyHostToDevice, c->stream));
        if (c->timing && tm.timed) {
            float ms = 0;
            HIP_TRY(hipEventSynchronize(tm.ev[1]));
            HIP_TRY(hipEventElapsedTime(&ms, tm.ev[0], tm.ev[1]));
            tm.ms_earlier += ms;
        }
        if (c->timing) HIP_TRY(hipEventRecord(tm.ev[0], c->stream));
        trace_kernel(c, L, q, r, dst, host ? e0 : 0ll);
        if (c->timing) { HIP_TRY(hipEventRecord(tm.ev[1], c->stream)); tm.timed = true; }
        HIP_TRY(hipGetLastError());
        if (host) {
            HIP_TRY(hipMemcpyAsync(recs + (size_t)e0 * edge_bytes, dst, bytes, hipMemcpyDeviceToHost, c->stream));
            HIP_TRY(hipStreamSynchronize(c->stream));
        }
    }
    return PPGPU_OK;
}

static int trace_timing(ppgpu_ctx* c, TraceTimer& tm, double* ms_out) {
    if (!c || !ms_out) return fail(PPGPU_EINVAL, "null argument");
    if (!c->timing || !tm.timed) return fail(PPGPU_ESTATE, "no timed trace launch (ppgpu_enable_timing, then trace edges)");
    HIP_TRY(hipSetDevice(c->device));
    float ms = 0;
    HIP_TRY(hipEventSynchronize(tm.ev[1]));
    HIP_TRY(hipEventElapsedTime(&ms, tm.ev[0], tm.ev[1]));
    *ms_out = ms + tm.ms_earlier;
// ... 710 lines not shown
```

Baseline: 181.9 million edges/s.

## Compact swept edges into a list so plan, pose and approach kernels skip shared edges

The share-mark kernel now compacts every edge that actually needs a sweep into a device list with a block-level ballot/prefix and one 64-bit atomic. The plan-skips, pose-sweep and approach-events kernels read edge indices from that list and exit early past its count, instead of working on every edge and skipping shared or malformed ones. Edges left off the list have their track summary zeroed, and an optional approach list adds the unshared ones straight to the live list. The cost is an extra indirection and gathered, uncoalesced setup loads, plus a larger mark kernel with atomics. Grids are still sized for all edges, so the surplus blocks launch and exit.

```diff
diff --git a/include/ppgpu.h b/include/ppgpu.h
--- a/include/ppgpu.h
+++ b/include/ppgpu.h
@@ -110,6 +110,8 @@
 int ppgpu_past_timing(ppgpu_ctx* ctx, int32_t back, double* ms_solve, double* ms_pose, double* ms_cover, double* ms_heuristic);
 int ppgpu_last_cover_edges(ppgpu_ctx* ctx, int64_t* n_edges);
 int ppgpu_last_shared_edges(ppgpu_ctx* ctx, int64_t* n_edges);
+int ppgpu_last_swept_edges(ppgpu_ctx* ctx, int64_t* n_edges);
+int ppgpu_last_slices(ppgpu_ctx* ctx, int64_t* n_slices, int64_t* last_slice_edges);
 
 int ppgpu_device_alloc(ppgpu_ctx* ctx, uint64_t bytes, void** d_out);
 int ppgpu_device_free(ppgpu_ctx* ctx, void* d_ptr);
diff --git a/path_planner_amd/api.py b/path_planner_amd/api.py
--- a/path_planner_amd/api.py
+++ b/path_planner_amd/api.py
@@ -49,6 +49,8 @@
         "ppgpu_past_timing": (C.c_int, [vp, i32, C.POINTER(dbl), C.POINTER(dbl), C.POINTER(dbl), C.POINTER(dbl)]),
         "ppgpu_last_cover_edges": (C.c_int, [vp, C.POINTER(i64)]),
         "ppgpu_last_shared_edges": (C.c_int, [vp, C.POINTER(i64)]),
+        "ppgpu_last_swept_edges": (C.c_int, [vp, C.POINTER(i64)]),
+        "ppgpu_last_slices": (C.c_int, [vp, C.POINTER(i64), C.POINTER(i64)]),
         "ppgpu_set_config": (C.c_int, [vp, C.POINTER(PpgpuConfig)]),
         "ppgpu_set_grid": (C.c_int, [vp, vp, i32, i32, dbl]),
         "ppgpu_get_grid_clearance": (C.c_int, [vp, vp, i64]),
@@ -112,7 +114,10 @@
         "ppgpu_comm_destroy": (C.c_int, [vp]),
         "ppgpu_comm_abort": (C.c_int, [vp]),
     }
+    optional = {"ppgpu_last_swept_edges", "ppgpu_last_slices"}
     for name, (res, args) in sig.items():
+        if name in optional and not hasattr(lib, name):
+            continue
         fn = getattr(lib, name)
         fn.restype = res
         fn.argtypes = args
@@ -188,6 +193,16 @@
         n = C.c_int64()
         self._ck(LIB.ppgpu_last_shared_edges(self._h, C.byref(n)), "ppgpu_last_shared_edges")
         return n.value
+
+    def last_swept_edges(self):
+        n = C.c_int64()
+        self._ck(LIB.ppgpu_last_swept_edges(self._h, C.byref(n)), "ppgpu_last_swept_edges")
+        return n.value
+
+    def last_slices(self):
+        n, last = C.c_int64(), C.c_int64()
+        self._ck(LIB.ppgpu_last_slices(self._h, C.byref(n), C.byref(last)), "ppgpu_last_slices")
+        return n.value, last.value
 
     def reserve_samples(self, max_samples, max_vertices=16):
         self._ck(LIB.ppgpu_reserve_samples(self._h, max_samples, max_vertices), "ppgpu_reserve_samples")
diff --git a/path_planner_amd/csrc/pp_k_common.h b/path_planner_amd/csrc/pp_k_common.h
--- a/path_planner_amd/csrc/pp_k_common.h
+++ b/path_planner_amd/csrc/pp_k_common.h
@@ -7,8 +7,13 @@
     unsigned live_count;
     unsigned hw_count;
     unsigned defer_count[PP_HL_MAX_N + 1];
+    unsigned sweep_count;
+    unsigned swept_total;
 };
 static_assert(sizeof(PPLaunchWords) == 128, "the launch counters share one 128-byte line");
+static_assert(offsetof(PPLaunchWords, sweep_count) % 8 == 0 && offsetof(PPLaunchWords, swept_total) == offsetof(PPLaunchWords, sweep_count) + 4,
+              "pp_k_mark_sweeps adds to sweep_count (low half) and swept_total (high half) with one 64-bit atomic");
+__device__ __forceinline__ unsigned long long* pp_sweep_counters(PPLaunchWords* w) { return reinterpret_cast<unsigned long long*>(&w->sweep_count); }
 
 struct PPParams {
     double max_speed, slow_speed, rho, rho_cov, horizon, tmin, inc_d, sst, ribw, cpf, tpf;
@@ -48,6 +53,8 @@
     int ngp, nch;
     unsigned* share_head;
     unsigned* share_of;
+    int approach_list;
+    unsigned* sweep_list;
 };
 
 #define PP_SETUP_MALFORMED 1u
@@ -56,6 +63,8 @@
 #define PP_SETUP_NO_SWEEP (PP_SETUP_MALFORMED | PP_SETUP_COLOCATED | PP_SETUP_SHARED)
 #define PP_SHARE_KEYS 8
 #define PP_SHARE_NONE 0xffffffffu
+#define PP_FAR_DONE (-2)
+#define PP_SHARE_UNSWEPT 0xfffffffeu
 struct PPEdgeSetupBody {
     PPSegBase seg[3];
     double p0, p1, p2, hi1;
@@ -222,5 +231,9 @@
 __device__ __forceinline__ void pp_launch_reset(const PPParams& p, long long e) {
     if (!p.reset_words) return;
     if (e < PP_NQ) p.work[(size_t)e * PP_QSTRIDE] = 0ull;
-    if (e == 0) { if (p.e_base == 0) *p.words = PPLaunchWords{}; else p.words->live_count = 0u; }
-}
+    if (p.e_base == 0) {
+        if (e < (long long)(sizeof(PPLaunchWords) / sizeof(unsigned))) reinterpret_cast<unsigned*>(p.words)[e] = 0u;
+    } else if (e == 0) {
+        p.words->live_count = 0u; p.words->sweep_count = 0u;
+    }
+}
diff --git a/path_planner_amd/csrc/pp_k_cover.h b/path_planner_amd/csrc/pp_k_cover.h
--- a/path_planner_amd/csrc/pp_k_cover.h
+++ b/path_planner_amd/csrc/pp_k_cover.h
@@ -20,7 +20,6 @@
     return m;
 }
 
-#define PP_FAR_DONE (-2)
 #define PP_FAR_SHARED (-3)
 #define PP_FAR_LAST_MASK 0xfffff
 #define PP_FAR_SPLIT (1 << 30)
@@ -56,11 +55,20 @@
 #ifndef PP_LANE_NEAR_MAX
 #define PP_LANE_NEAR_MAX 8
 #endif
-__global__ __launch_bounds__(PP_APPROACH_THREADS, PP_APPROACH_MIN_WAVES) void pp_k_approach_events(PPParams p) {
+template <bool LISTED>
+__device__ __forceinline__ void pp_approach_events_body(const PPParams& p) {
     __shared__ double s_rec[PP_APPROACH_THREADS * PP_REC_STRIDE];
     const long long e0 = (long long)blockIdx.x * PP_APPROACH_THREADS;
-    const long long e = e0 + threadIdx.x;
-    const bool valid = e < p.n_edges;
+    long long eIdx = e0 + threadIdx.x;
+    bool inRange = eIdx < p.n_edges;
+    if (LISTED) {
+        const long long count = (long long)(unsigned)pp_const_i32(&p.words->sweep_count)[0];
+        if (e0 >= count) return;
+        inRange = eIdx < count;
+        eIdx = inRange ? (long long)p.sweep_list[eIdx] : 0;
+    }
+    const long long e = eIdx;
+    const bool valid = inRange;
     const PPEdgeSetupBody* S = p.setup + p.ws_base + (valid ? e : 0);
     int2 out; out.x = 0; out.y = 0;
     int splitInfo = 0;
@@ -206,6 +214,9 @@
         }
     }
 }
+
+__global__ __launch_bounds__(PP_APPROACH_THREADS, PP_APPROACH_MIN_WAVES) void pp_k_approach_events(PPParams p) { pp_approach_events_body<true>(p); }
+__global__ __launch_bounds__(PP_APPROACH_THREADS, PP_APPROACH_MIN_WAVES) void pp_k_approach_events_direct(PPParams p) { pp_approach_events_body<false>(p); }
 
 #ifndef PP_FUSE_HEUR
 #define PP_FUSE_HEUR 1
diff --git a/path_planner_amd/csrc/pp_k_solve.h b/path_planner_amd/csrc/pp_k_solve.h
--- a/path_planner_amd/csrc/pp_k_solve.h
+++ b/path_planner_amd/csrc/pp_k_solve.h
@@ -94,8 +94,8 @@
             if (!(bound < 9.0e4)) dub.type = -1;
         }
     }
-    bool member[2] = {false, false};
-    unsigned key[2] = {0u, 0u}, pos[2] = {0u, 0u};
+    bool member0 = false, member1 = false;
+    unsigned key0 = 0u, key1 = 0u, pos0 = 0u, pos1 = 0u;
     for (int k = 0; k < (e2 >= 0 ? 2 : 1); k++) {
         PPEdgeSetup* __restrict__ O = p.setup + p.ws_base + (k ? e2 : e);
         struct { double approx, wStart, wEnd, speed; int type; unsigned vi, cbits, sflags; } S;
@@ -116,10 +116,11 @@
         }
         if (p.share_head) {
             const long long egk = k ? pp_edge_position(p, p.e_base + e2) : eg;
-            member[k] = pp_edge_shareable(p, cv, S.type, S.sflags, S.cbits, S.wStart, S.wEnd, S.speed);
-            key[k] = member[k] ? pp_share_key(S.vi, S.cbits, S.type) : PP_SHARE_NONE;
-            pos[k] = (unsigned)egk;
-            p.share_of[egk] = key[k];
+            const bool member = pp_edge_shareable(p, cv, S.type, S.sflags, S.cbits, S.wStart, S.wEnd, S.speed);
+            const bool unswept = S.type < 0 || (S.sflags & (PP_SETUP_MALFORMED | PP_SETUP_COLOCATED)) != 0u;
+            const unsigned key = member ? pp_share_key(S.vi, S.cbits, S.type) : PP_SHARE_NONE;
+            if (k) { member1 = member; key1 = key; pos1 = (unsigned)egk; } else { member0 = member; key0 = key; pos0 = (unsigned)egk; }
+            p.share_of[egk] = unswept ? PP_SHARE_UNSWEPT : key;
         }
         pp_curve_segments(cv, O->seg);
         O->qx = cv.qx; O->qy = cv.qy; O->rho = cv.rho; O->rho_inv = cv.rho_inv; O->length = cv.length;
@@ -147,27 +148,67 @@
         O->omask = omask;
     }
     if (p.share_head) {
-        pp_share_elect(p, member[0], key[0], pos[0]);
-        if (__ballot(e2 >= 0) != 0ull) pp_share_elect(p, member[1], key[1], pos[1]);
-    }
-}
-__global__ __launch_bounds__(256) void pp_k_share_mark(PPParams p) {
-    const long long e = (long long)blockIdx.x * 256 + threadIdx.x;
-    if (e >= p.n_edges) return;
-    const long long eg = pp_edge_position(p, p.e_base + e);
-    const unsigned key = p.share_of[eg];
-    if (key == PP_SHARE_NONE) return;
-    const unsigned head = p.share_head[key];
-    if (head == (unsigned)eg) { p.share_of[eg] = PP_SHARE_NONE; return; }
-    p.share_of[eg] = head;
-    PPEdgeSetup* S = p.setup + p.ws_base + e;
-    S->sflags |= PP_SETUP_SHARED;
-    double* r = reinterpret_cast<double*>(p.out + eg);
-    const unsigned info = (unsigned)(S->type & 0xff);
-    r[0] = __hiloint2double((int)info, 0);
-    r[1] = 0.0; r[2] = 0.0; r[3] = S->approx;
-    for (int i = 4; i < 13; i++) r[i] = 0.0;
-    r[13] = S->p0; r[14] = S->p1; r[15] = S->p2;
+        pp_share_elect(p, member0, key0, pos0);
+        if (__ballot(e2 >= 0) != 0ull) pp_share_elect(p, member1, key1, pos1);
+    }
+}
+#define PP_MARK_THREADS 1024
+#define PP_MARK_THREADS_PLAIN 256
+__global__ __launch_bounds__(PP_MARK_THREADS) void pp_k_mark_sweeps(PPParams p) {
+    const long long e = (long long)blockIdx.x * blockDim.x + threadIdx.x;
+    const bool valid = e < p.n_edges;
+    const long long eg = valid ? pp_edge_position(p, p.e_base + e) : 0;
+    const unsigned key = valid ? p.share_of[eg] : PP_SHARE_UNSWEPT;
+    unsigned head = PP_SHARE_NONE;
+    if (key != PP_SHARE_UNSWEPT && key != PP_SHARE_NONE) {
+        head = p.share_head[key];
+        if (head == (unsigned)eg) head = PP_SHARE_NONE;
+    }
+    const bool swept = key != PP_SHARE_UNSWEPT && head == PP_SHARE_NONE;
+    unsigned at = 0u;
+    if (p.sweep_list) {
+        __shared__ unsigned s_cnt[PP_MARK_THREADS / 64];
+        __shared__ unsigned s_base;
+        const int lane = threadIdx.x & 63, wave = threadIdx.x >> 6;
+        const unsigned long long m = __ballot(swept);
+        if (lane == 0) s_cnt[wave] = (unsigned)__popcll(m);
+        __syncthreads();
+        if (threadIdx.x == 0) {
+            unsigned tot = 0;
+            for (int w = 0; w < (int)(blockDim.x >> 6); w++) tot += s_cnt[w];
+            s_base = tot ? (unsigned)atomicAdd(pp_sweep_counters(p.words), ((unsigned long long)tot << 32) | tot) : 0u;
+        }
+        __syncthreads();
+        at = s_base + (unsigned)__popcll(m & ((1ull << lane) - 1ull));
+        for (int w = 0; w < wave; w++) at += s_cnt[w];
+    }
+    if (!valid) return;
+    if (key != PP_SHARE_NONE) p.share_of[eg] = head;
+    if (head != PP_SHARE_NONE) {
+        PPEdgeSetup* S = p.setup + p.ws_base + e;
+        S->sflags |= PP_SETUP_SHARED;
+        double* r = reinterpret_cast<double*>(p.out + eg);
+        const unsigned info = (unsigned)(S->type & 0xff);
+        r[0] = __hiloint2double((int)info, 0);
+        r[1] = 0.0; r[2] = 0.0; r[3] = S->approx;
+        for (int i = 4; i < 13; i++) r[i] = 0.0;
+        r[13] = S->p0; r[14] = S->p1; r[15] = S->p2;
+    }
+    if (!p.sweep_list) return;
+    if (swept) p.sweep_list[at] = (unsigned)e;
+    else {
+        reinterpret_cast<int4*>(p.track_summary)[p.ws_base + e] = make_int4(0, 0, 0, 0);
+        if (p.approach_list) {
+            if (head != PP_SHARE_NONE) {
+                p.track_far[p.ws_base + e] = make_int2(PP_FAR_DONE, 0);
+            } else {
+                p.track_far[p.ws_base + e] = make_int2(0, 0);
+                const unsigned li = atomicAdd(&p.words->live_count, 1u);
+                p.live_list[2 * (size_t)li] = (unsigned)e;
+                p.live_list[2 * (size_t)li + 1] = (unsigned)eg;
+            }
+        }
+    }
 }
 __global__ __launch_bounds__(256) void pp_k_share_fanout(PPParams p, int copy_child) {
     const long long eg = (long long)blockIdx.x * 16 + (threadIdx.x >> 4);
diff --git a/path_planner_amd/csrc/pp_k_sweep.h b/path_planner_amd/csrc/pp_k_sweep.h
--- a/path_planner_amd/csrc/pp_k_sweep.h
+++ b/path_planner_amd/csrc/pp_k_sweep.h
@@ -14,6 +14,7 @@
     int dub_err;
     int pad;
 };
+static_assert(sizeof(PPTrackSummary) == sizeof(int4), "pp_k_mark_sweeps zeroes the summary of an edge off the sweep list with one 16-byte store");
 
 #define PP_FINISH_MAX 8
 struct PPCoverState {
@@ -226,13 +227,27 @@
                 for (int j = 0; j < p.n_obst && decided; j++) against(OB[j]);
         });
 }
-template <bool OBST_LDS>
-__device__ __forceinline__ void pp_plan_stage(const PPParams& p, const long long el0, const int ne, double* s_setup, PPObst* s_obst) {
+template <bool LISTED>
+__device__ __forceinline__ long long pp_plan_count(const PPParams& p) {
+    return LISTED ? (long long)(unsigned)pp_const_i32(&p.words->sweep_count)[0] : p.n_edges;
+}
+template <bool OBST_LDS, bool LISTED>
+__device__ __forceinline__ void pp_plan_stage(const PPParams& p, const long long el0, const int ne, double* s_setup, PPObst* s_obst, unsigned* s_slot) {
     const int tid = (int)threadIdx.x;
-    const double* src = reinterpret_cast<const double*>(p.setup + p.ws_base + el0);
-    for (int i = tid; i < ne * PP_SETUP_GLOBAL_WORDS; i += 256) {
-        const int ed = i / PP_SETUP_GLOBAL_WORDS, w = i - ed * PP_SETUP_GLOBAL_WORDS;
-        if (w < PP_SETUP_WORDS) s_setup[ed * PP_SETUP_LDS_STRIDE + w] = src[i];
+    if (LISTED) {
+        if (tid < ne) s_slot[tid] = p.sweep_list[el0 + tid];
+        __syncthreads();
+        for (int i = tid; i < ne * PP_SETUP_GLOBAL_WORDS; i += 256) {
+            const int ed = i / PP_SETUP_GLOBAL_WORDS, w = i - ed * PP_SETUP_GLOBAL_WORDS;
+            const double* src = reinterpret_cast<const double*>(p.setup + p.ws_base + (long long)s_slot[ed]);
+            if (w < PP_SETUP_WORDS) s_setup[ed * PP_SETUP_LDS_STRIDE + w] = src[w];
+        }
+    } else {
+        const double* src = reinterpret_cast<const double*>(p.setup + p.ws_base + el0);
+        for (int i = tid; i < ne * PP_SETUP_GLOBAL_WORDS; i += 256) {
+            const int ed = i / PP_SETUP_GLOBAL_WORDS, w = i - ed * PP_SETUP_GLOBAL_WORDS;
+            if (w < PP_SETUP_WORDS) s_setup[ed * PP_SETUP_LDS_STRIDE + w] = src[i];
+        }
     }
     if (OBST_LDS) {
         const double* os = reinterpret_cast<const double*>(p.obst);
@@ -240,46 +255,54 @@
         for (int i = tid; i < p.n_obst * (int)(sizeof(PPObst) / sizeof(double)); i += 256) od[i] = os[i];
     }
 }
-template <bool GAUSSIAN, bool OBST_LDS>
+template <bool GAUSSIAN, bool OBST_LDS, bool LISTED>
 __device__ __forceinline__ void pp_plan_skips_thread(const PPParams& p, int epw) {
     __shared__ double s_setup[PP_PLAN_EDGES_MAX * PP_SETUP_LDS_STRIDE];
     __shared__ PPObst s_obst[OBST_LDS ? PP_WAVE : 1];
+    __shared__ unsigned s_slot[LISTED ? PP_PLAN_EDGES_MAX : 1];
     const int tid = (int)threadIdx.x;
-    const long long el0 = (long long)blockIdx.x * epw;
-    const int ne = (int)((p.n_edges - el0 < (long long)epw) ? (p.n_edges - el0) : (long long)epw);
-    pp_plan_stage<OBST_LDS>(p, el0, ne, s_setup, s_obst);
+    const long long el0 = (long long)blockIdx.x * epw, n = pp_plan_count<LISTED>(p);
+    if (LISTED && el0 >= n) return;
+    const int ne = (int)((n - el0 < (long long)epw) ? (n - el0) : (long long)epw);
+    pp_plan_stage<OBST_LDS, LISTED>(p, el0, ne, s_setup, s_obst, s_slot);
     __syncthreads();
     const int t = (int)blockIdx.y * 256 + tid;
     if (t >= ne * p.nch) return;
     const int el = (int)((unsigned)t / (unsigned)p.nch);
     const int chunk = t - el * p.nch;
     const PPEdgeSetupBody* S = reinterpret_cast<const PPEdgeSetupBody*>(&s_setup[el * PP_SETUP_LDS_STRIDE]);
-    pp_plan_skips_chunk<GAUSSIAN>(p, S, OBST_LDS ? s_obst : p.obst, p.ws_base + el0 + el, chunk);
+    pp_plan_skips_chunk<GAUSSIAN>(p, S, OBST_LDS ? s_obst : p.obst, p.ws_base + (LISTED ? (long long)s_slot[el] : el0 + el), chunk);
 }
 #ifndef PP_PLAN_MIN_WAVES
 #define PP_PLAN_MIN_WAVES 8
 #endif
-__global__ __launch_bounds__(256, PP_PLAN_MIN_WAVES) void pp_k_plan_skips_chunkwise(PPParams p, int epw) { pp_plan_skips_thread<false, true>(p, epw); }
-__global__ __launch_bounds__(256) void pp_k_plan_skips_many(PPParams p, int epw) { pp_plan_skips_thread<false, false>(p, epw); }
-__global__ __launch_bounds__(256) void pp_k_plan_skips_gaussian_chunkwise(PPParams p, int epw) { pp_plan_skips_thread<true, true>(p, epw); }
-__global__ __launch_bounds__(256) void pp_k_plan_skips_gaussian_many(PPParams p, int epw) { pp_plan_skips_thread<true, false>(p, epw); }
+__global__ __launch_bounds__(256, PP_PLAN_MIN_WAVES) void pp_k_plan_skips_chunkwise(PPParams p, int epw) { pp_plan_skips_thread<false, true, true>(p, epw); }
+__global__ __launch_bounds__(256) void pp_k_plan_skips_many(PPParams p, int epw) { pp_plan_skips_thread<false, false, true>(p, epw); }
+__global__ __launch_bounds__(256) void pp_k_plan_skips_gaussian_chunkwise(PPParams p, int epw) { pp_plan_skips_thread<true, true, true>(p, epw); }
+__global__ __launch_bounds__(256) void pp_k_plan_skips_gaussian_many(PPParams p, int epw) { pp_plan_skips_thread<true, false, true>(p, epw); }
+__global__ __launch_bounds__(256, PP_PLAN_MIN_WAVES) void pp_k_plan_skips_chunkwise_direct(PPParams p, int epw) { pp_plan_skips_thread<false, true, false>(p, epw); }
+__global__ __launch_bounds__(256) void pp_k_plan_skips_many_direct(PPParams p, int epw) { pp_plan_skips_thread<false, false, false>(p, epw); }
+__global__ __launch_bounds__(256) void pp_k_plan_skips_gaussian_chunkwise_direct(PPParams p, int epw) { pp_plan_skips_thread<true, true, false>(p, epw); }
+__global__ __launch_bounds__(256) void pp_k_plan_skips_gaussian_many_direct(PPParams p, int epw) { pp_plan_skips_thread<true, false, false>(p, epw); }
 
 #ifndef PP_PLAN_SPAN
 #define PP_PLAN_SPAN 4
 #endif
 static_assert(PP_PLAN_SPAN >= 2 && PP_PLAN_SPAN <= 32 && 256 % PP_PLAN_SPAN == 0, "a span may not straddle a 256-chunk tile of a long edge (and 256 threads clear the span words)");
 #define PP_PLAN_SPANS_MAX (256 / PP_PLAN_SPAN + PP_PLAN_EDGES_MAX)
-template <bool GAUSSIAN>
+template <bool GAUSSIAN, bool LISTED>
 __device__ __forceinline__ void pp_plan_skips_spans(const PPParams& p, int epw) {
     constexpr int LOG = __builtin_ctz(PP_PLAN_SPAN);
     __shared__ double s_setup[PP_PLAN_EDGES_MAX * PP_SETUP_LDS_STRIDE];
     __shared__ PPObst s_obst[PP_WAVE];
     __shared__ double s_bx[256], s_by[256];
     __shared__ unsigned long long s_span[PP_PLAN_SPANS_MAX];
+    __shared__ unsigned s_slot[LISTED ? PP_PLAN_EDGES_MAX : 1];
     const int tid = (int)threadIdx.x;
-    const long long el0 = (long long)blockIdx.x * epw;
-    const int ne = (int)((p.n_edges - el0 < (long long)epw) ? (p.n_edges - el0) : (long long)epw);
-    pp_plan_stage<true>(p, el0, ne, s_setup, s_obst);
+    const long long el0 = (long long)blockIdx.x * epw, n = pp_plan_count<LISTED>(p);
+    if (LISTED && el0 >= n) return;
+    const int ne = (int)((n - el0 < (long long)epw) ? (n - el0) : (long long)epw);
+    pp_plan_stage<true, LISTED>(p, el0, ne, s_setup, s_obst, s_slot);
     if (tid < PP_PLAN_SPANS_MAX) s_span[tid] = 0ull;
     __syncthreads();
     const int t = (int)blockIdx.y * 256 + tid;
@@ -340,7 +363,7 @@
     }
     __syncthreads();
     if (!live) return;
-    pp_plan_chunk<GAUSSIAN>(p, S, p.ws_base + el0 + el, chunk, tg, endTime, tF,
+    pp_plan_chunk<GAUSSIAN>(p, S, p.ws_base + (LISTED ? (long long)s_slot[el] : el0 + el), chunk, tg, endTime, tF,
         [&](double, double dL, double& xF, double& yF, double& xE, double& yE, double& tE, double& dE) {
             xF = s_bx[tid]; yF = s_by[tid];
             xE = NAN; yE = 0.0;
@@ -360,8 +383,10 @@
             }
         });
 }
-__global__ __launch_bounds__(256, PP_PLAN_MIN_WAVES) void pp_k_plan_skips(PPParams p, int epw) { pp_plan_skips_spans<false>(p, epw); }
-__global__ __launch_bounds__(256, PP_PLAN_MIN_WAVES) void pp_k_plan_skips_gaussian(PPParams p, int epw) { pp_plan_skips_spans<true>(p, epw); }
+__global__ __launch_bounds__(256, PP_PLAN_MIN_WAVES) void pp_k_plan_skips(PPParams p, int epw) { pp_plan_skips_spans<false, true>(p, epw); }
+__global__ __launch_bounds__(256, PP_PLAN_MIN_WAVES) void pp_k_plan_skips_gaussian(PPParams p, int epw) { pp_plan_skips_spans<true, true>(p, epw); }
+__global__ __launch_bounds__(256, PP_PLAN_MIN_WAVES) void pp_k_plan_skips_direct(PPParams p, int epw) { pp_plan_skips_spans<false, false>(p, epw); }
+__global__ __launch_bounds__(256, PP_PLAN_MIN_WAVES) void pp_k_plan_skips_gaussian_direct(PPParams p, int epw) { pp_plan_skips_spans<true, false>(p, epw); }
 
 template <bool GAUSSIAN>
 __device__ __forceinline__ void pp_pose_sweep_edge(const PPParams& p, const long long e) {
@@ -562,12 +587,32 @@
 #ifndef PP_POSE_MIN_WAVES
 #define PP_POSE_MIN_WAVES 6
 #endif
+__device__ __forceinline__ void pp_pose_sweep_listed(const PPParams& p, bool& mine, long long& idx) {
+    const unsigned count = (unsigned)pp_const_i32(&p.words->sweep_count)[0];
+    const unsigned entry = (unsigned)pp_const_i32(p.sweep_list + idx)[0];
+    mine = idx < (long long)count;
+    idx = (long long)entry;
+}
 __global__ __launch_bounds__(PP_WPB * 64, PP_POSE_MIN_WAVES) void pp_k_pose_sweep(PPParams p) {
+    int wave;
+    long long idx = pp_wave_edge<PP_WPB>(wave);
+    bool mine;
+    pp_pose_sweep_listed(p, mine, idx);
+    if (mine) pp_pose_sweep_edge<false>(p, p.ws_base + idx);
+}
+__global__ __launch_bounds__(PP_WPB * 64, 4) void pp_k_pose_sweep_gaussian(PPParams p) {
+    int wave;
+    long long idx = pp_wave_edge<PP_WPB>(wave);
+    bool mine;
+    pp_pose_sweep_listed(p, mine, idx);
+    if (mine) pp_pose_sweep_edge<true>(p, p.ws_base + idx);
+}
+__global__ __launch_bounds__(PP_WPB * 64, PP_POSE_MIN_WAVES) void pp_k_pose_sweep_direct(PPParams p) {
     int wave;
     const long long idx = pp_wave_edge<PP_WPB>(wave);
     if (idx < p.n_edges) pp_pose_sweep_edge<false>(p, p.ws_base + idx);
 }
-__global__ __launch_bounds__(PP_WPB * 64, 4) void pp_k_pose_sweep_gaussian(PPParams p) {
+__global__ __launch_bounds__(PP_WPB * 64, 4) void pp_k_pose_sweep_gaussian_direct(PPParams p) {
     int wave;
     const long long idx = pp_wave_edge<PP_WPB>(wave);
     if (idx < p.n_edges) pp_pose_sweep_edge<true>(p, p.ws_base + idx);
diff --git a/path_planner_amd/csrc/ppgpu.hip b/path_planner_amd/csrc/ppgpu.hip
--- a/path_planner_amd/csrc/ppgpu.hip
+++ b/path_planner_amd/csrc/ppgpu.hip
@@ -172,6 +172,8 @@
     bool lane_heuristic = true;
     long long prepass_min_edges = PP_PREPASS_MIN_EDGES;
     bool share_sweeps = true;
+    bool use_sweep_list = true;
+    bool approach_list = true;
     size_t slice_bytes = PP_SLICE_BYTES;
     DevBuf<PPEdgeSetup> setup;
     DevBuf<unsigned short> track_hits;
@@ -184,6 +186,9 @@
     DevBuf<unsigned> defer_list, live_list, hw_list;
     DevBuf<unsigned> share_head, share_of;
     bool last_launch_shared = false;
+    DevBuf<unsigned> sweep_list;
+    long long last_launch_slices = 0, last_slice_edges = 0;
+    bool last_launch_listed = false;
     DevBuf<PPCoverState> cover_state;
     DevBuf<unsigned long long> work;
     int n_cu = 0;
@@ -301,6 +306,8 @@
     if (const char* aw = std::getenv("PPGPU_SOLVE_ALL_WORDS")) c->solve_all_words = std::atoi(aw) != 0;
     if (const char* ps = std::getenv("PPGPU_PLAN_SPANS")) c->plan_spans = std::atoi(ps) != 0;
     if (const char* ss = std::getenv("PPGPU_SHARE_SWEEPS")) c->share_sweeps = std::atoi(ss) != 0;
+    if (const char* sl = std::getenv("PPGPU_SWEEP_LIST")) c->use_sweep_list = std::atoi(sl) != 0;
+    if (const char* al = std::getenv("PPGPU_APPROACH_LIST")) c->approach_list = std::atoi(al) != 0;
     if (const char* sb = std::getenv("PPGPU_SLICE_BYTES")) {
         const long long v = std::atoll(sb);
         if (v > 0) c->slice_bytes = (size_t)v;
@@ -395,6 +402,25 @@
     int64_t n = 0;
     for (unsigned h : of) n += (h != PP_SHARE_NONE);
     *n_edges = n;
+    return PPGPU_OK;
+}
+
+int ppgpu_last_slices(ppgpu_ctx* c, int64_t* n_slices, int64_t* last_slice_edges) {
+    if (!c || !n_slices || !last_slice_edges) return fail(PPGPU_EINVAL, "null argument");
+    *n_slices = c->last_launch_slices; *last_slice_edges = c->last_slice_edges;
+    return PPGPU_OK;
+}
+
+int ppgpu_last_swept_edges(ppgpu_ctx* c, int64_t* n_edges) {
+    if (!c || !n_edges) return fail(PPGPU_EINVAL, "null argument");
+    HIP_TRY(hipSetDevice(c->device));
+    *n_edges = c->last_launch_edges;
+    if (c->last_launch_listed) {
+        unsigned swept = 0;
+        HIP_TRY(hipStreamSynchronize(c->stream));
+        HIP_TRY(hipMemcpy(&swept, &c->words.p->swept_total, sizeof(unsigned), hipMemcpyDeviceToHost));
+        *n_edges = (int64_t)swept;
+    }
     return PPGPU_OK;
 }
 
@@ -1216,7 +1242,7 @@
     p.heuristic = g.heuristic; p.tsp_k = g.tsp_k; p.h_rho = g.heuristic_turning_radius;
     p.fuse_h = 0;
     p.lane_split = 0; p.defer_h = 0; p.defer_list = nullptr; p.quiet_finish = 0; p.live_list = nullptr; p.cover_state = nullptr; p.hw_list = nullptr; p.words = nullptr; p.reset_words = 0;
-    p.share_head = nullptr; p.share_of = nullptr;
+    p.share_head = nullptr; p.share_of = nullptr; p.sweep_list = nullptr; p.approach_list = 0;
     p.grid = PPGrid{grid_bits(c), c->rows, c->cols, c->wpr, c->res, c->res > 0 ? 1.0 / c->res : 0.0, c->rows > 0 ? c->grid_clear.p : nullptr};
     p.obst = c->obst.p; p.n_obst = c->n_obst; p.obst_model = c->obst_model;
     p.verts = c->verts.p; p.ribbons = c->ribbons.p; p.tgrid = c->tgrid.p; p.ng = c->ng; p.nverts = c->nverts;
@@ -1352,6 +1378,7 @@
     bool forked;
     bool share;
     bool share_child;
+    bool sweep_list;
     int nch, ngp;
     long long slice;
 };
@@ -1387,6 +1414,7 @@
     m.forked = m.lane_finish && m.fuse_h && p.heuristic != PPGPU_H_MAX_DISTANCE;
     m.share = m.prepasses && m.packed && !p.wedges && c->share_sweeps && (long long)p.nverts * PP_SHARE_KEYS < (1ll << 32);
     m.share_child = m.share && p.child != nullptr;
+    m.sweep_list = m.share && c->use_sweep_list;
 }
 
 static int cost_workspace(ppgpu_ctx* c, CostLaunch& m) {
@@ -1434,6 +1462,11 @@
         if ((rc = c->share_head.reserve((size_t)p.nverts * PP_SHARE_KEYS, false, st)) || (rc = c->share_of.reserve(total, false, st))) return rc;
         p.share_head = c->share_head.p; p.share_of = c->share_of.p;
     }
+    if (m.sweep_list) {
+        if ((rc = c->sweep_list.reserve(ws + PP_WPB, false, st))) return rc;
+        p.sweep_list = c->sweep_list.p;
+        p.approach_list = c->approach_list ? 1 : 0;
+    }
     return PPGPU_OK;
 }
 
@@ -1454,7 +1487,10 @@
     hipEvent_t* ev = c->ev_ring[c->ev_slot];
     if (c->timing) HIP_TRY(hipEventRecord(ev[EV_BEGIN], st));
     hipLaunchKernelGGL(c->solve_all_words ? pp_k_solve_edges_all_words : pp_k_solve_edges, dim3((unsigned)((p.n_edges + 255) / 256)), dim3(256), 0, st, p);
-    if (m.share) hipLaunchKernelGGL(pp_k_share_mark, dim3((unsigned)((p.n_edges + 255) / 256)), dim3(256), 0, st, p);
+    if (m.share) {
+        const unsigned mark_threads = m.sweep_list ? PP_MARK_THREADS : PP_MARK_THREADS_PLAIN;
+        hipLaunchKernelGGL(pp_k_mark_sweeps, dim3((unsigned)((p.n_edges + mark_threads - 1) / mark_threads)), dim3(mark_threads), 0, st, p);
+    }
     if (c->timing) HIP_TRY(hipEventRecord(ev[EV_SOLVED], st));
     if (m.skip_chunks) {
         int epw = 256 / p.nch;
@@ -1462,13 +1498,17 @@
         if (epw > PP_PLAN_EDGES_MAX) epw = PP_PLAN_EDGES_MAX;
         const unsigned blocks = (unsigned)((p.n_edges + epw - 1) / epw);
         const bool many = p.n_obst > PP_WAVE;
-        void (*planner)(PPParams, int) = m.gaussian ? (many ? pp_k_plan_skips_gaussian_many : (c->plan_spans ? pp_k_plan_skips_gaussian : pp_k_plan_skips_gaussian_chunkwise))
-                                                    : (many ? pp_k_plan_skips_many : (c->plan_spans ? pp_k_plan_skips : pp_k_plan_skips_chunkwise));
+        void (*planner)(PPParams, int);
+        if (m.sweep_list) planner = m.gaussian ? (many ? pp_k_plan_skips_gaussian_many : (c->plan_spans ? pp_k_plan_skips_gaussian : pp_k_plan_skips_gaussian_chunkwise))
+                                               : (many ? pp_k_plan_skips_many : (c->plan_spans ? pp_k_plan_skips : pp_k_plan_skips_chunkwise));
+        else planner = m.gaussian ? (many ? pp_k_plan_skips_gaussian_many_direct : (c->plan_spans ? pp_k_plan_skips_gaussian_direct : pp_k_plan_skips_gaussian_chunkwise_direct))
+                                  : (many ? pp_k_plan_skips_many_direct : (c->plan_spans ? pp_k_plan_skips_direct : pp_k_plan_skips_chunkwise_direct));
         hipLaunchKernelGGL(planner, dim3(blocks, (unsigned)((epw * p.nch + 255) / 256)), dim3(256), 0, st, p, epw);
     }
-    hipLaunchKernelGGL(m.gaussian ? pp_k_pose_sweep_gaussian : pp_k_pose_sweep, dim3((unsigned)((p.n_edges + PP_WPB - 1) / PP_WPB)), dim3(PP_WPB * 64), 0, st, p);
+    void (*pose)(PPParams) = m.sweep_list ? (m.gaussian ? pp_k_pose_sweep_gaussian : pp_k_pose_sweep) : (m.gaussian ? pp_k_pose_sweep_gaussian_direct : pp_k_pose_sweep_direct);
+    hipLaunchKernelGGL(pose, dim3((unsigned)((p.n_edges + PP_WPB - 1) / PP_WPB)), dim3(PP_WPB * 64), 0, st, p);
     if (c->timing) HIP_TRY(hipEventRecord(ev[EV_POSED], st));
-    if (m.prepasses) hipLaunchKernelGGL(pp_k_approach_events, dim3((unsigned)((p.n_edges + PP_APPROACH_THREADS - 1) / PP_APPROACH_THREADS)), dim3(PP_APPROACH_THREADS), 0, st, p);
+    if (m.prepasses) hipLaunchKernelGGL(p.approach_list ? pp_k_approach_events : pp_k_approach_events_direct, dim3((unsigned)((p.n_edges + PP_APPROACH_THREADS - 1) / PP_APPROACH_THREADS)), dim3(PP_APPROACH_THREADS), 0, st, p);
     if (c->timing) HIP_TRY(hipEventRecord(ev[EV_APPROACHED], st));
     hipLaunchKernelGGL(m.gaussian ? pp_k_cover_sweep_gaussian : pp_k_cover_sweep, dim3(resident_grid(c, m.gaussian, p.n_edges)), dim3(PP_WPB * 64), 0, st, p);
     if (m.lane_finish)
@@ -1545,17 +1585,19 @@
     if (c->timing) c->ev_slot = (int)(c->ev_launches % PP_TIMING_RING);
     for (double& ms : c->ms_ring[c->ev_slot]) ms = 0;
     c->live_earlier_slices = 0;
-    c->last_launch_shared = false;
+    c->last_launch_shared = false; c->last_launch_listed = false;
     if (m.share) HIP_TRY(hipMemsetAsync(p.share_head, 0xff, (size_t)p.nverts * PP_SHARE_KEYS * sizeof(unsigned), c->stream));
+    c->last_launch_slices = 0;
     for (long long e0 = 0; e0 < total; e0 += m.slice) {
         p.e_base = e0; p.ws_base = 0; p.n_edges = (total - e0 < m.slice) ? (total - e0) : m.slice;
+        c->last_launch_slices++; c->last_slice_edges = p.n_edges;
         if (c->timing && e0 > 0 && (rc = bank_slice_timing(c, m.packed))) return rc;
         if ((rc = cost_slice(c, m))) return rc;
     }
     p.e_base = 0;
     p.n_edges = total;
     if ((rc = cost_heuristic_tail(c, m))) return rc;
-    c->last_launch_edges = total; c->last_launch_packed = m.packed; c->last_launch_shared = m.share;
+    c->last_launch_edges = total; c->last_launch_packed = m.packed; c->last_launch_shared = m.share; c->last_launch_listed = m.sweep_list;
     if (c->timing) { HIP_TRY(hipEventRecord(c->ev_ring[c->ev_slot][EV_END], c->stream)); c->ev_launches++; }
     HIP_TRY(hipGetLastError());
     return PPGPU_OK;
```

New measurement: 191.4 million edges/s (median of 6 runs). 1.05x the previous value.
